# ivargr/kmer_mapper

Hardware: AMD Instinct MI355X
Metric: M k-mers mapped/sec (whole node), k=31 150bp reads (higher is better)
Workload: dtype u64

## Files before the change

### kmer_mapper_amd/csrc/kmm.hip

```cpp
#include <hip/hip_runtime.h>

#include <climits>
#include <cstdarg>
#include <cstdint>
#include <cstdio>
#include <cstdlib>
#include <chrono>
#include <cstring>
#include <memory>
#include <mutex>
#include <string>
#include <thread>
#include <type_traits>
#include <utility>
#include <vector>

#include "kmm.h"
#include "kmm_radix_plan.hpp"

namespace {

thread_local std::string g_err;

int fail(int code, const char *fmt, ...)
// ... 188 lines not shown
constexpr size_t RING_SLOT = (size_t)16 << 20;
#ifndef KMM_RING_SLOTS
#define KMM_RING_SLOTS 8
#endif
constexpr int RING_SLOTS = KMM_RING_SLOTS;


struct TimedEvent {
    Event start, stop;
    int kernel_id = 0;
};

struct BgzfStaged {
    std::vector<unsigned long long> m_off, o_rel;
    uint64_t p = 0;
    int chain_err = 0;
    uint32_t bad_isize = 0, bad_ms = 0;
    bool hit_cap = false;
    bool staged = false;
    double ms_scan_inside = 0;
};

struct IndexStreams {
    Stream stream;
    Stream copy_stream;
};

struct RxDir16 {
    DevPtr<uint16_t> rx_pstart16;
    DevPtr<uint32_t> rx_slice_e0;
    DevPtr<uint16_t> rx_slice_fmax;
};
struct RxSlotFilter {
    DevPtr<uint32_t> rx_slots;
};
struct RxArrays : RxDir16, RxSlotFilter {
    uint64_t rx_S = 0;
    DevPtr<uint32_t> rx_pstart;
    DevPtr<uint64_t> rx_pkeys;
    DevPtr<uint64_t> rx_pkeys_raw;
    DevPtr<uint16_t> rx_pfreq;
    DevPtr<uint32_t> rx_pnodes, rx_porig, rx_ecnt, rx_ecnt_acc;
    DevPtr<uint32_t> rx_norder, rx_nnode;
    DevPtr<uint32_t> rx_occ;
};

struct kmm_index : IndexStreams, RxArrays {
    int device = 0;
    Event copied;
    DevPtr<uint4> buckets;
    DevPtr<uint4> entries;
    DevPtr<uint32_t> occ;
    bool use_occ = true;
    int occ_shift = 0;
    uint32_t bloom_words = 0;
    bool wide = false;
    bool direct_deferred = false;
    size_t direct_bytes = 0;
    size_t occ_bytes_plan = 0;
    int rx_why_not = 0;
    uint32_t *counts = nullptr;
    DevPtr<uint32_t> own_counts_buf;
    DevPtr<uint8_t> lut_default;
    DevPtr<uint8_t> lut_codes;
    DevPtr<unsigned long long> first_bad;
    DevPtr<unsigned long long> stats;
    DevPtr<unsigned long long> queue;
    bool dynamic_schedule = true;
    int dyn_chunk = 16;
    uint64_t modulo = 0, magic = 0;
    int64_t n_entries = 0, max_node_id = 0;
    Stage stage[2];
    int cur = 0;
    int n_cu = 256;
    int path = 0;
    int grid_per_cu = 64;
    bool rx_ok = false;
    RxGeometry rx_geo;
    bool rx_no_mid = false;
    bool rx_flush_sorted = true;
    uint32_t rx_max_slice = 0;
    bool rx_fits_small = false, rx_fits_mid = false;
    int rx_grid_per_cu = 2;
    int64_t rx_min_units = 0;
    int64_t rx_sub_cap = RX_SUB_CAP_MAX;
    int64_t rx_sub_cap_eff = 0;
    int rx_sub_cap_eff_age = 0;
    int64_t rx_sub_cap_last = 0;
    const uint32_t *dbg_T1 = nullptr, *dbg_item_base = nullptr;
    const uint16_t *dbg_start1 = nullptr;
    uint32_t dbg_F1 = 0, dbg_NB = 0;
    int host_pack_threads = 0;
    std::unique_ptr<kmm_hostpack::Workers> pack_pool;
    PinnedBuf pack_pinned;
    PinnedBuf ring[RING_SLOTS];
    PinnedBuf pack_bits_pinned;
    int64_t host_packed_calls = 0, host_packed_record_calls = 0;
    int64_t host_pack_slice_kb = 0;
    DevBuf bgzf_comp[2], bgzf_raw[2], bgzf_meta[2], bgzf_tabs, bgzf_err, bgzf_carry, bgzf_crc, bgzf_status;
    Event bgzf_done[2];
    Event bgzf_slot_ev[RING_SLOTS];
    bool bgzf_used[2] = {false, false};
    int bgzf_cur = 0;
    int64_t bgzf_carry_len = 0;
    BgzfStaged bgzf_pre;
    bool bgzf_pre_valid = false;
    const uint8_t *bgzf_pre_from = nullptr, *bgzf_hint_ptr = nullptr;
    int64_t bgzf_pre_n = 0, bgzf_hint_n = 0;
    int bgzf_pre_buf = 0;
    int64_t bgzf_prestaged_calls = 0;
    int64_t bgzf_head_skip = 0;
    int64_t bgzf_tail_stop = -1;
    int64_t bgzf_calls = 0, bgzf_members = 0;
    DevBuf gz_comp, gz_raw, gz_carry, gz_window, gz_tabs, gz_meta, gz_res, gz_win, gz_gmaps, gz_gwin, gz_err;
    std::vector<DevBuf> gz_arena;
    kmm_gunzip::StreamState gz_state;
    int64_t gz_carry_len = 0;
    double gz_ratio = 4.0;
    int64_t gzip_calls = 0, gzip_members = 0, gzip_chunks = 0, gzip_false_starts = 0, gzip_continuations = 0, gzip_inflated = 0;
    int dbg_gzip_chunk_kb = 0;
    DevBuf bam_tiles[2], bam_bad, bam_base, bam_ctl, bam_out;
    int32_t bam_n_ref = -1;
    uint32_t bam_excl = 0;
    int64_t bam_calls = 0, bam_records = 0, bam_excluded = 0, bam_header_bytes = 0, bam_false_starts = 0, bam_continuations = 0;
    DevBuf rs_comp, rs_raw, rs_meta, rs_err, rs_status;
    int64_t bam_n_ref_param = -1;
    int64_t dbg_bam_resync_kb = 0;
    int64_t dbg_bgzf_call_cap_kb = 0;
    int64_t flat_uniform_batches = 0;
    DevBuf sam_tiles, sam_base, sam_ctl;
    int64_t sam_calls = 0, sam_records = 0, sam_excluded = 0, sam_header_lines = 0;
    uint32_t bam_incl = 0, bam_min_mapq = 0;
    int sel_n_regions = 0, sel_keep_unplaced = 0;
    std::vector<kmm_sel::Interval> sel_iv_id, sel_iv_name;
    std::vector<std::string> sel_names;
    DevBuf sel_buf;
    size_t sel_off_name_iv = 0, sel_off_name_off = 0, sel_off_names = 0;
    int dbg_bgzf_slot_kb = 0;
    int64_t dbg_rx_buf_limit = 0;
    int dbg_rec_copy_stream = 0;
    int dbg_rec_skip = 0;
    int min_base_quality = 0;
    int use_record_qual = 0;
    int original_strand = 0;
    int64_t dbg_rec_piece_kb = 0;
    int dbg_rec_grid = 0;
    bool rx_filter = true;
    bool rx_filter_slots = true;
    bool rx_p3_fp = true;
    uint32_t dbg_p2f_cap = P2F_SLOTS;
    bool rx_packed = true;
    bool ecnt_dirty = false;
    bool rx_unchecked = false;
    DevBuf rx_buf1, rx_buf2, rx_meta, rx_probe;
    int sticky_rc = KMM_OK;
    std::string sticky_msg;
    uint64_t map_calls = 0;
    int64_t read_hits_calls = 0;
    int record_hits = 0, rhq_mode = 0;
    DevBuf rhq_hits, rhq_win;
    int64_t rhq_head = 0, rhq_pending = 0, rhq_cap = 0;
    int record_keep = 0, rk_invert = 0, rk_min_permille = 0;
    int64_t rk_min_hits = 1;
    DevBuf rkq, rk_ctl, rk_tile, rk_super;
    int64_t rkq_bound = 0, rkq_cap = 0;
    uint64_t n_radix_batches = 0, n_direct_batches = 0;
    ncclComm_t comm = nullptr;
    int comm_rank = -1, comm_size = 0;
    int comm_slices = 8;
    int64_t comm_sliced_reduces = 0;
    Stream comm_stream;
    std::vector<Event> comm_events;
    std::vector<uint64_t> flush_cuts;
    bool timing = false;
    std::vector<TimedEvent> ev_used;
    std::vector<TimedEvent> ev_free;
    double ms_total[KMM_N_KERNELS] = {0};
    int64_t launches[KMM_N_KERNELS] = {0};
};

namespace {

IndexView view_of(const kmm_index *ix)
{
    IndexView v;
    v.buckets = ix->buckets;
    v.entries = ix->entries;
    v.occ = ix->use_occ ? ix->occ : nullptr;
    v.occ_shift = ix->occ_shift;
    v.bloom_words = ix->bloom_words;
    v.wide = ix->wide ? 1 : 0;
    v.counts = ix->counts;
    v.stats = ix->stats;
    v.modulo = ix->modulo;
    v.magic = ix->magic;
    return v;
}

struct ScopedTimer {
    kmm_index *ix;
    TimedEvent ev{};
    bool active = false;
    int begin(kmm_index *ix_, int kernel_id)
    {
        ix = ix_;
        if (!ix->timing)
            return KMM_OK;
        if (!ix->ev_free.empty()) {
            ev = std::move(ix->ev_free.back());
            ix->ev_free.pop_back();
        } else {
            HIPCHK(hipEventCreate(ev.start.put()));
            HIPCHK(hipEventCreate(ev.stop.put()));
        }
        ev.kernel_id = kernel_id;
        HIPCHK(hipEventRecord(ev.start, ix->stream));
        active = true;
        return KMM_OK;
    }
    int end()
    {
        if (!active)
            return KMM_OK;
        HIPCHK(hipEventRecord(ev.stop, ix->stream));
        ix->ev_used.push_back(std::move(ev));
        active = false;
        return KMM_OK;
    }
};

int rx_flush(kmm_index *ix);
int rx_build_slots(kmm_index *ix);
bool rx_slots_active(const kmm_index *ix);
int rx_check_conservation(kmm_index *ix);
int ensure_direct(kmm_index *ix);
constexpr size_t KMM_STAT_BYTES = (size_t)KMM_STAT_SHARDS * KMM_STAT_STRIDE * 8;

int drain(kmm_index *ix)
{
    KMMCHK(rx_flush(ix));
    HIPCHK(hipStreamSynchronize(ix->copy_stream));
    HIPCHK(hipStreamSynchronize(ix->stream));
    if (ix->sticky_rc != KMM_OK)
        return fail(ix->sticky_rc, "%s", ix->sticky_msg.c_str());
    KMMCHK(rx_check_conservation(ix));
    unsigned long long bad[3] = {NO_BAD, NO_BAD, NO_BAD};
    HIPCHK(hipMemcpy(bad, ix->first_bad, sizeof bad, hipMemcpyDeviceToHost));
    if (bad[0] != NO_BAD || bad[1] != NO_BAD || bad[2] != NO_BAD) {
        unsigned long long reset[3] = {NO_BAD, NO_BAD, NO_BAD};
        HIPCHK(hipMemcpy(ix->first_bad, reset, sizeof reset, hipMemcpyHostToDevice));
        char where[160];
        snprintf(where, sizeof where, " [one of the map calls since the last synchronising call; the latest was call "
                 "#%llu on this handle; counts are invalid until kmm_reset_counts]", (unsigned long long)ix->map_calls);
        int rc;
        if (bad[2] != NO_BAD)
            rc = fail(KMM_ERR_INVALID_ARG, "read_offsets of a mapped chunk is not non-decreasing at read %llu%s",
                      bad[2], where);
        else if (bad[1] != NO_BAD)
            rc = fail(KMM_ERR_MALFORMED,
                      "record structure violated at byte offset %llu of a mapped chunk (a record line "
                      "does not start with '@' / '+' / '>'%s): multi-line FASTA/FASTQ is not supported by "
                      "the GPU reader%s", bad[1],
                      ix->min_base_quality > 0 ? ", or a quality line that ends there is not as long as its sequence line "
                                                 "(checked with min_base_quality set)" : "", where);
        else
            rc = fail(KMM_ERR_INVALID_BASE,
                      "read byte at offset %llu of a mapped chunk is not a nucleotide under the "
                      "lookup table (the reference's DNA encoder raises here)%s", bad[0], where);
        ix->sticky_rc = rc;
        ix->sticky_msg = g_err;
        return rc;
    }
    return KMM_OK;
}

int grid_for(const kmm_index *ix, int64_t work_items, int per_cu)
{
    int64_t cap = (int64_t)ix->n_cu * per_cu;
    int64_t g = work_items < cap ? work_items : cap;
    return (int)(g < 1 ? 1 : g);
}

int grid_for_tiles(const kmm_index *ix, int64_t n_tiles)
{
    const int64_t slots = (int64_t)ix->n_cu * 8;
    const int64_t cap = (int64_t)ix->n_cu * ix->grid_per_cu;
    int64_t g = n_tiles <= slots ? n_tiles : n_tiles / 4;
    if (n_tiles > slots && g < slots)
        g = slots;
    if (g > cap)
        g = cap;
    return (int)(g < 1 ? 1 : g);
}

struct DirectSchedule {
    dim3 grid;
    unsigned long long *queue;
};

int direct_schedule(kmm_index *ix, int64_t n_units, DirectSchedule *sched)
{
    const int64_t slots = (int64_t)ix->n_cu * 8;
    const bool dynamic = ix->dynamic_schedule && n_units >= slots * 4 * ix->dyn_chunk;
    if (dynamic)
        HIPCHK(hipMemsetAsync(ix->queue, 0, 3 * sizeof(unsigned long long), ix->stream));
    sched->grid = dim3(dynamic ? (unsigned)slots : (unsigned)grid_for_tiles(ix, n_units));
    sched->queue = dynamic ? ix->queue : nullptr;
    return KMM_OK;
}

template <typename F>
void with_probe_flavour(const IndexView &iv, F &&f)
{
    if (iv.occ && iv.wide)
        f(std::integral_constant<int, PROBE_WIDE_FILTER>{});
    else if (iv.occ)
        f(std::integral_constant<int, PROBE_BITMAP>{});
    else if (iv.wide)
        f(std::integral_constant<int, PROBE_WIDE>{});
    else
        f(std::integral_constant<int, PROBE_NARROW>{});
}

template <typename TT>
int stage_in(kmm_index *ix, DevBuf &buf, const TT *src, size_t count, const TT **dev, bool *staged)
{
    if (count == 0) {
        KMMCHK(ensure(buf, 256));
        *dev = static_cast<const TT *>(buf.p);
        return KMM_OK;
    }
    if (is_device_ptr(src)) {
        *dev = src;
        return KMM_OK;
    }
    KMMCHK(ensure(buf, count * sizeof(TT)));
    HIPCHK(hipMemcpyAsync(buf.p, src, count * sizeof(TT), hipMemcpyHostToDevice, ix->copy_stream));
    *dev = static_cast<const TT *>(buf.p);
    *staged = true;
    return KMM_OK;
}

Stage &next_stage(kmm_index *ix)
{
    Stage &s = ix->stage[ix->cur];
    ix->cur ^= 1;
    return s;
}

int stage_acquire(kmm_index *ix, Stage &s)
{
    if (s.used)
        HIPCHK(hipStreamWaitEvent(ix->copy_stream, s.done, 0));
    return KMM_OK;
}

int stage_copies_done(kmm_index *ix)
{
    HIPCHK(hipEventRecord(ix->copied, ix->copy_stream));
    HIPCHK(hipStreamWaitEvent(ix->stream, ix->copied, 0));
    return KMM_OK;
}

int stage_release(kmm_index *ix, Stage &s, bool staged)
{
    HIPCHK(hipEventRecord(s.done, ix->stream));
    s.used = true;
    if (staged)
        HIPCHK(hipEventSynchronize(ix->copied));
    return KMM_OK;
}

int lut_has_break(const uint8_t *lut, bool *has_break)
{
    *has_break = false;
    if (!lut)
        return KMM_OK;
    uint8_t copy[256];
    if (is_device_ptr(lut)) {
        HIPCHK(hipMemcpy(copy, lut, 256, hipMemcpyDeviceToHost));
        lut = copy;
    }
    *has_break = memchr(lut, KMM_LUT_BREAK, 256) != nullptr;
    return KMM_OK;
// ... 540 lines not shown
    if (with_occ && N <= bloom_max_entries) {
        size_t bb = (size_t)N * 2;
        const size_t cap = N <= 13000000 ? KMM_BLOOM_MAX_BYTES : KMM_BLOOM_MAX_BYTES * 3 / 2;
        if (bb > cap) bb = cap;
        if (bb < 64) bb = 64;
        if (const char *env = getenv("KMM_BLOOM_BYTES"))
            bb = (size_t)strtoull(env, nullptr, 10);
        if (bb >= 4) {
            ix->bloom_words = (uint32_t)(bb / 4);
            occ_bytes = (size_t)ix->bloom_words * 4;
        }
    }
    ix->occ_shift = occ_shift;
    ix->wide = !with_occ;
    if (const char *env = getenv("KMM_WIDE_BUCKETS"))
        ix->wide = atoi(env) != 0;
    HIPCHK(hipMalloc(ix->own_counts_buf.put(), sizeof(uint32_t) * (size_t)(ix->max_node_id + 1)));
    ix->counts = ix->own_counts_buf;
    HIPCHK(hipMemsetAsync(ix->counts, 0, sizeof(uint32_t) * (size_t)(ix->max_node_id + 1), ix->stream));
    HIPCHK(hipMalloc(ix->lut_default.put(), 256));
    HIPCHK(hipMalloc(ix->first_bad.put(), 3 * sizeof(unsigned long long)));
    HIPCHK(hipMalloc(ix->queue.put(), 4 * sizeof(unsigned long long)));
    HIPCHK(hipMalloc(ix->stats.put(), KMM_STAT_BYTES));
    HIPCHK(hipMemset(ix->stats, 0, KMM_STAT_BYTES));
    uint8_t lut[256];
    default_lut(lut);
    HIPCHK(hipMemcpy(ix->lut_default, lut, 256, hipMemcpyHostToDevice));
    HIPCHK(hipMalloc(ix->lut_codes.put(), 256));
    memset(lut, 0xFF, sizeof lut);
    lut[0] = 0; lut[1] = 1; lut[2] = 2; lut[3] = 3;
    HIPCHK(hipMemcpy(ix->lut_codes, lut, 256, hipMemcpyHostToDevice));
    unsigned long long nb[3] = {NO_BAD, NO_BAD, NO_BAD};
    HIPCHK(hipMemcpy(ix->first_bad, nb, sizeof nb, hipMemcpyHostToDevice));
    {
        const int budget = kmm_hostpack::cpu_budget();
        ix->host_pack_threads = budget >= 8 ? (budget < 16 ? budget : 16) : 0;
        if (const char *env = getenv("KMM_HOST_PACK_THREADS")) {
            const int v = atoi(env);
            ix->host_pack_threads = v < 0 ? 0 : (v > 256 ? 256 : v);
        }
    }

    if (ix->host_pack_threads > 0 && (size_t)(ix->max_node_id + 1) * 4 >= ((size_t)64 << 20))
        (void)ensure_ring(ix);

    DevBuf d_h2i, d_nk, d_km, d_nd, d_fr, d_err;
    bool staged = false;
    const int32_t *p_h2i = nullptr, *p_nk = nullptr, *p_nd = nullptr;
    const uint64_t *p_km = nullptr;
    const uint16_t *p_fr = nullptr;
    int rc = KMM_OK;
    do {
        if ((rc = stage_in<int32_t>(ix, d_h2i, h2i, (size_t)M, &p_h2i, &staged))) break;
        if ((rc = stage_in<int32_t>(ix, d_nk, nk, (size_t)M, &p_nk, &staged))) break;
        if ((rc = stage_in<uint64_t>(ix, d_km, kmers, (size_t)N, &p_km, &staged))) break;
        if ((rc = stage_in<int32_t>(ix, d_nd, nodes, (size_t)N, &p_nd, &staged))) break;
        if ((rc = stage_in<uint16_t>(ix, d_fr, freqs, (size_t)N, &p_fr, &staged))) break;
        if ((rc = ensure(d_err, 4))) break;
    } while (0);
    if (rc == KMM_OK) {
        hipError_t e = hipMemsetAsync(d_err.p, 0, 4, ix->copy_stream);
        if (e == hipSuccess) e = hipStreamSynchronize(ix->copy_stream);
        if (e != hipSuccess)
            rc = fail(KMM_ERR_HIP, "index upload: %s", hipGetErrorString(e));
    }
    uint32_t err = 0;
    if (rc == KMM_OK) {
        hipLaunchKernelGGL(k_validate_index, dim3(grid_for(ix, (int64_t)((M + 255) / 256), 16)), dim3(256), 0, ix->stream,
                           p_h2i, p_nk, p_nd, M, N, ix->max_node_id, (uint32_t *)d_err.p);
        hipError_t e = hipGetLastError();
        if (e == hipSuccess) e = hipStreamSynchronize(ix->stream);
        if (e == hipSuccess) e = hipMemcpy(&err, d_err.p, 4, hipMemcpyDeviceToHost);
        if (e != hipSuccess)
            rc = fail(KMM_ERR_HIP, "index validation: %s", hipGetErrorString(e));
    }
    if (rc == KMM_OK && !err)
        rc = rx_build(ix, p_h2i, p_nk, p_km, p_nd, p_fr);
    size_t eager_max = (size_t)16 << 30;
    if (const char *env = getenv("KMM_DIRECT_EAGER_BYTES"))
        eager_max = (size_t)strtoull(env, nullptr, 10);
    ix->direct_bytes = sizeof(uint4) * ((size_t)M * (ix->wide ? 2 : 1) + (size_t)(N > 0 ? N : 1));
    if (rc == KMM_OK && !err) {
        ix->occ_bytes_plan = with_occ ? occ_bytes : 0;
        if (ix->rx_ok && ix->direct_bytes > eager_max) {
            ix->direct_deferred = true;
        } else {
            IdxRaw src;
            src.h2i = p_h2i; src.nk = p_nk; src.kmers = p_km; src.nodes = p_nd; src.freqs = p_fr;
            rc = direct_build(ix, src, N, with_occ ? occ_bytes : 0, (uint32_t *)d_err.p);
        }
    }
    if (rc != KMM_OK)
        return rc;
    if (err & 1u)
        return fail(KMM_ERR_INDEX, "index inconsistent: a non-empty bucket "
                    "(hashes_to_index[h], n_kmers[h]) reaches outside [0, n_entries=%lld)",
                    (long long)N);
    if (err & 2u)
        return fail(KMM_ERR_INDEX, "index inconsistent: a node id lies outside [0, max_node_id=%lld]",
                    (long long)ix->max_node_id);
    return KMM_OK;
}

int kmm_index_create(const int32_t *hashes_to_index, const int32_t *n_kmers, uint64_t modulo,
                     const uint64_t *kmers, const int32_t *nodes, const uint16_t *frequencies,
                     int64_t n_entries, int64_t max_node_id, int device, kmm_index_t **out)
{
    if (!out)
        return fail(KMM_ERR_INVALID_ARG, "out is NULL");
    *out = nullptr;
    if (!hashes_to_index || !n_kmers)
        return fail(KMM_ERR_INVALID_ARG, "hashes_to_index / n_kmers is NULL");
    if (modulo < 1)
        return fail(KMM_ERR_INVALID_ARG, "modulo must be >= 1");
    if (n_entries < 0 || max_node_id < 0)
        return fail(KMM_ERR_INVALID_ARG, "n_entries=%lld / max_node_id=%lld negative",
                    (long long)n_entries, (long long)max_node_id);
    if (n_entries > 0 && (!kmers || !nodes || !frequencies))
        return fail(KMM_ERR_INVALID_ARG, "kmers / nodes / frequencies is NULL");
    if (n_entries > 0x7FFFFFFFll)
        return fail(KMM_ERR_INVALID_ARG, "n_entries exceeds the int32 bucket offsets of the index format");
    int ndev = 0;
    hipError_t e = hipGetDeviceCount(&ndev);
    if (e != hipSuccess || ndev < 1) {
        (void)hipGetLastError();
        return fail(KMM_ERR_HIP, "no HIP device available (%s): libkmm has no CPU fallback",
                    e != hipSuccess ? hipGetErrorString(e) : "0 devices");
    }
    if (device < 0 || device >= ndev)
        return fail(KMM_ERR_INVALID_ARG, "device %d outside [0, %d)", device, ndev);
    kmm_index *ix = new kmm_index();
    ix->device = device;
    ix->modulo = modulo;
    ix->magic = magic_for(modulo);
    ix->n_entries = n_entries;
    ix->max_node_id = max_node_id;
    int rc = index_create_impl(ix, hashes_to_index, n_kmers, kmers, nodes, frequencies);
    if (rc != KMM_OK) {
        std::string keep = g_err;
        kmm_index_destroy(ix);
        g_err = keep;
        return rc;
    }
    *out = ix;
    return KMM_OK;
}

int kmm_reset_counts(kmm_index_t *ix)
{
    if (!ix)
        return fail(KMM_ERR_INVALID_ARG, "idx is NULL");
    HIPCHK(hipSetDevice(ix->device));
    HIPCHK(hipMemsetAsync(ix->counts, 0, sizeof(uint32_t) * (size_t)(ix->max_node_id + 1), ix->stream));
    if (ix->rx_ecnt && ix->ecnt_dirty)
        HIPCHK(hipMemsetAsync(ix->rx_ecnt, 0, sizeof(uint32_t) * (size_t)(ix->rx_S ? ix->rx_S : 1), ix->stream));
    if (ix->rx_ecnt_acc)
        HIPCHK(hipMemsetAsync(ix->rx_ecnt_acc, 0, sizeof(uint32_t) * (size_t)(ix->rx_S ? ix->rx_S : 1), ix->stream));
    ix->ecnt_dirty = false;
    ix->rhq_head = ix->rhq_pending = 0;
    if (ix->rk_ctl.p)
        HIPCHK(hipMemsetAsync(ix->rk_ctl.p, 0, 16, ix->stream));
    ix->rkq_bound = 0;
    HIPCHK(hipMemsetAsync(ix->first_bad, 0xFF, 3 * sizeof(unsigned long long), ix->stream));
    if (ix->sticky_rc != KMM_OK) {
        unsigned long long nb[3] = {NO_BAD, NO_BAD, NO_BAD};
        HIPCHK(hipStreamSynchronize(ix->stream));
        HIPCHK(hipMemcpy(ix->first_bad, nb, sizeof nb, hipMemcpyHostToDevice));
        if (ix->sticky_rc == KMM_ERR_INTERNAL)
            HIPCHK(hipMemset(ix->stats, 0, KMM_STAT_BYTES));
        ix->sticky_rc = KMM_OK;
        ix->sticky_msg.clear();
    }
    return KMM_OK;
}

int kmm_bind_counts(kmm_index_t *ix, uint32_t *device_counts)
{
    if (!ix)
        return fail(KMM_ERR_INVALID_ARG, "idx is NULL");
    HIPCHK(hipSetDevice(ix->device));
    KMMCHK(rx_flush(ix));
    HIPCHK(hipStreamSynchronize(ix->stream));
    if (!device_counts) {
        ix->counts = ix->own_counts_buf;
        return KMM_OK;
    }
    if (!is_device_ptr(device_counts))
        return fail(KMM_ERR_INVALID_ARG, "kmm_bind_counts needs a device pointer");
    ix->counts = device_counts;
    return KMM_OK;
}

int kmm_counts_device_ptr(kmm_index_t *ix, uint32_t **out)
{
    if (!ix || !out)
        return fail(KMM_ERR_INVALID_ARG, "NULL argument");
    *out = ix->counts;
    return KMM_OK;
}

int kmm_synchronize(kmm_index_t *ix)
{
    if (!ix)
        return fail(KMM_ERR_INVALID_ARG, "idx is NULL");
    HIPCHK(hipSetDevice(ix->device));
    return drain(ix);
}

static bool ensure_pack_pool(kmm_index_t *ix);
static bool ensure_pinned(PinnedBuf &b, size_t want);

static bool ensure_ring(kmm_index_t *ix)
{
    for (int i = 0; i < RING_SLOTS; ++i) {
        if (ix->ring[i].p)
            continue;
        size_t got = 0;
        uint8_t *p = g_shelf.take(RING_SLOT, &got);
        if (p && got != RING_SLOT) {
            g_shelf.give(p, got);
            p = nullptr;
        }
        if (!p && hipHostMalloc(reinterpret_cast<void **>(&p), RING_SLOT, hipHostMallocDefault) != hipSuccess) {
            (void)hipGetLastError();
            return false;
        }
        ix->ring[i].p = p;
        ix->ring[i].bytes = RING_SLOT;
    }
    for (int i = 0; i < RING_SLOTS; ++i)
        if (!ix->bgzf_slot_ev[i] && hipEventCreateWithFlags(ix->bgzf_slot_ev[i].put(), hipEventDisableTiming) != hipSuccess) {
            (void)hipGetLastError();
            return false;
        }
    return true;
}

static int fetch_to_pageable(kmm_index_t *ix, uint8_t *dst, const uint8_t *src, size_t bytes, bool *done)
{
    *done = false;
    constexpr size_t SLOT = RING_SLOT;
    constexpr int SLOTS = RING_SLOTS;
    if (bytes < 4 * SLOT || !ensure_pack_pool(ix) || !ensure_ring(ix))
        return KMM_OK;
    const size_t n_slots = (bytes + SLOT - 1) / SLOT;
    auto issue = [&](size_t c) -> int {
        const size_t b0 = c * SLOT, len = bytes - b0 < SLOT ? bytes - b0 : SLOT;
        HIPCHK(hipMemcpyAsync(ix->ring[c % SLOTS].p, src + b0, len, hipMemcpyDeviceToHost, ix->copy_stream));
        HIPCHK(hipEventRecord(ix->bgzf_slot_ev[c % SLOTS], ix->copy_stream));
        return KMM_OK;
    };
    for (size_t c = 0; c < n_slots && c < (size_t)SLOTS; ++c)
        KMMCHK(issue(c));
    const int T = ix->pack_pool->size();
    for (size_t c = 0; c < n_slots; ++c) {
        HIPCHK(hipEventSynchronize(ix->bgzf_slot_ev[c % SLOTS]));
        const size_t b0 = c * SLOT, len = bytes - b0 < SLOT ? bytes - b0 : SLOT;
        const uint8_t *from = ix->ring[c % SLOTS].p;
        const size_t per = ((len + (size_t)T - 1) / (size_t)T + 63) & ~(size_t)63;
        ix->pack_pool->start([=](int w) {
            const size_t a = (size_t)w * per;
            if (a < len)
                memcpy(dst + b0 + a, from + a, len - a < per ? len - a : per);
        });
        ix->pack_pool->wait();
        if (c + SLOTS < n_slots)
            KMMCHK(issue(c + SLOTS));
    }
    *done = true;
    return KMM_OK;
}

int kmm_get_node_counts(kmm_index_t *ix, uint32_t *out)
{
    if (!ix || !out)
        return fail(KMM_ERR_INVALID_ARG, "NULL argument");
    HIPCHK(hipSetDevice(ix->device));
    KMMCHK(drain(ix));
    const size_t bytes = sizeof(uint32_t) * (size_t)(ix->max_node_id + 1);
    hipPointerAttribute_t a;
    memset(&a, 0, sizeof a);
    const bool known = hipPointerGetAttributes(&a, out) == hipSuccess;
    if (!known)
        (void)hipGetLastError();
    const bool on_device = known && (a.type == hipMemoryTypeDevice || a.type == hipMemoryTypeManaged);
    const bool page_locked = known && a.type == hipMemoryTypeHost;
    if (!on_device && !page_locked) {
        bool done = false;
        KMMCHK(guarded("kmm_get_node_counts", [&] {
            return fetch_to_pageable(ix, reinterpret_cast<uint8_t *>(out), reinterpret_cast<const uint8_t *>(ix->counts), bytes, &done);
        }));
        if (done)
            return KMM_OK;
    }
    HIPCHK(hipMemcpy(out, ix->counts, bytes, on_device ? hipMemcpyDeviceToDevice : hipMemcpyDeviceToHost));
    return KMM_OK;
}

int kmm_comm_get_unique_id(uint8_t id[KMM_COMM_ID_BYTES])
{
    if (!id)
        return fail(KMM_ERR_INVALID_ARG, "id is NULL");
    static_assert(KMM_COMM_ID_BYTES == NCCL_UNIQUE_ID_BYTES, "kmm.h and rccl.h disagree on the id size");
    KMMCHK(rccl_load());
    ncclUniqueId u;
    RCCLCHK(g_rccl.GetUniqueId(&u));
    memcpy(id, u.internal, KMM_COMM_ID_BYTES);
    return KMM_OK;
}

int kmm_comm_init_rank(kmm_index_t *ix, const uint8_t id[KMM_COMM_ID_BYTES], int n_ranks, int rank)
{
    if (!ix || !id)
        return fail(KMM_ERR_INVALID_ARG, "NULL argument");
    if (n_ranks < 1 || rank < 0 || rank >= n_ranks)
        return fail(KMM_ERR_INVALID_ARG, "rank %d outside [0, %d)", rank, n_ranks);
    KMMCHK(rccl_load());
    HIPCHK(hipSetDevice(ix->device));
    if (ix->comm) {
        RCCLCHK(g_rccl.CommDestroy(ix->comm));
        ix->comm = nullptr;
    }
    ncclUniqueId u;
    memcpy(u.internal, id, KMM_COMM_ID_BYTES);
    RCCLCHK(g_rccl.CommInitRank(&ix->comm, n_ranks, u, rank));
    ix->comm_rank = rank;
    ix->comm_size = n_ranks;
    return KMM_OK;
}

int kmm_comm_reduce_counts(kmm_index_t *ix, int root)
{
    if (!ix)
        return fail(KMM_ERR_INVALID_ARG, "idx is NULL");
    if (!ix->comm)
        return fail(KMM_ERR_INVALID_ARG, "kmm_comm_init_rank has not been called on this handle");
    if (root < -1 || root >= ix->comm_size)
        return fail(KMM_ERR_INVALID_ARG, "root %d outside [-1, %d)", root, ix->comm_size);
    HIPCHK(hipSetDevice(ix->device));
    const size_t n = (size_t)ix->max_node_id + 1;
    auto reduce = [&](size_t first, size_t count, hipStream_t st) {
        return root < 0 ? g_rccl.AllReduce(ix->counts + first, ix->counts + first, count, ncclUint32, ncclSum, ix->comm, st)
                        : g_rccl.Reduce(ix->counts + first, ix->counts + first, count, ncclUint32, ncclSum, root, ix->comm, st);
    };
    const int S = ix->comm_slices;
    if (S > 1 && n >= (size_t)S * 1024) {
        const bool by_range = ix->rx_norder && !ix->rx_ecnt_acc && ix->rx_flush_sorted;
        ix->comm_sliced_reduces++;
        if (!ix->comm_stream)
            HIPCHK(hipStreamCreateWithFlags(ix->comm_stream.put(), hipStreamNonBlocking));
        while ((int)ix->comm_events.size() < S + 1) {
            Event e;
            HIPCHK(hipEventCreateWithFlags(e.put(), hipEventDisableTiming));
            ix->comm_events.push_back(std::move(e));
        }
        if (!by_range)
            KMMCHK(rx_flush(ix));
        if (by_range && (int)ix->flush_cuts.size() != S + 1) {
            std::vector<uint32_t> bounds(S + 1);
            for (int t = 0; t <= S; ++t)
                bounds[t] = (uint32_t)(n * (size_t)t / (size_t)S);
            DevBuf d_b, d_c;
            KMMCHK(ensure(d_b, (S + 1) * 4));
            KMMCHK(ensure(d_c, (S + 1) * 8));
            HIPCHK(hipMemcpyAsync(d_b.p, bounds.data(), (S + 1) * 4, hipMemcpyHostToDevice, ix->stream));
            hipLaunchKernelGGL(k_rx_node_cuts, dim3(1), dim3(64), 0, ix->stream, ix->rx_nnode, ix->rx_S, (const uint32_t *)d_b.p, S + 1,
                               (unsigned long long *)d_c.p);
            HIPCHK(hipGetLastError());
            ix->flush_cuts.assign(S + 1, 0);
            HIPCHK(hipMemcpyAsync(ix->flush_cuts.data(), d_c.p, (S + 1) * 8, hipMemcpyDeviceToHost, ix->stream));
            HIPCHK(hipStreamSynchronize(ix->stream));
            ix->flush_cuts[0] = 0;
            ix->flush_cuts[S] = ix->rx_S;
        }
        ScopedTimer tm;
        KMMCHK(tm.begin(ix, KMM_KERNEL_RX_FLUSH));
        for (int t = 0; t < S; ++t) {
            if (by_range && ix->ecnt_dirty) {
                const uint64_t j0 = ix->flush_cuts[t], j1 = ix->flush_cuts[t + 1];
                if (j1 > j0)
                    hipLaunchKernelGGL(k_rx_flush_sorted, dim3(grid_for(ix, (int64_t)((j1 - j0 + 1023) / 1024), 8)), dim3(256), 0, ix->stream,
                                       view_of(ix), ix->rx_ecnt, ix->rx_norder + j0, ix->rx_nnode + j0, j1 - j0);
                HIPCHK(hipGetLastError());
            }
            HIPCHK(hipEventRecord(ix->comm_events[t], ix->stream));
            HIPCHK(hipStreamWaitEvent(ix->comm_stream, ix->comm_events[t], 0));
            const size_t first = n * (size_t)t / (size_t)S, end = n * (size_t)(t + 1) / (size_t)S;
            RCCLCHK(reduce(first, end - first, ix->comm_stream));
        }
        if (by_range && ix->ecnt_dirty)
            HIPCHK(hipMemsetAsync(ix->rx_ecnt, 0, (size_t)ix->rx_S * 4, ix->stream));
        KMMCHK(tm.end());
        ix->ecnt_dirty = false;
        HIPCHK(hipEventRecord(ix->comm_events[S], ix->comm_stream));
        HIPCHK(hipStreamWaitEvent(ix->stream, ix->comm_events[S], 0));
        return drain(ix);
    }
    KMMCHK(rx_flush(ix));
    RCCLCHK(reduce(0, n, ix->stream));
    return drain(ix);
}

int kmm_comm_destroy(kmm_index_t *ix)
{
    if (!ix)
        return fail(KMM_ERR_INVALID_ARG, "idx is NULL");
    if (ix->comm) {
        HIPCHK(hipSetDevice(ix->device));
        HIPCHK(hipStreamSynchronize(ix->stream));
        RCCLCHK(g_rccl.CommDestroy(ix->comm));
        ix->comm = nullptr;
        ix->comm_rank = -1;
        ix->comm_size = 0;
    }
    return KMM_OK;
}

int kmm_reduce_counts(kmm_index_t **per_gpu, int n_gpus, int root)
{
    if (!per_gpu || n_gpus < 1)
        return fail(KMM_ERR_INVALID_ARG, "per_gpu is NULL or n_gpus < 1");
    if (root < -1 || root >= n_gpus)
        return fail(KMM_ERR_INVALID_ARG, "root %d outside [-1, %d)", root, n_gpus);
    std::vector<int> devs(n_gpus);
    for (int i = 0; i < n_gpus; ++i) {
        if (!per_gpu[i])
            return fail(KMM_ERR_INVALID_ARG, "per_gpu[%d] is NULL", i);
        if (per_gpu[i]->max_node_id != per_gpu[0]->max_node_id)
            return fail(KMM_ERR_INVALID_ARG, "handles disagree on max_node_id");
        devs[i] = per_gpu[i]->device;
        for (int j = 0; j < i; ++j)
            if (devs[j] == devs[i])
                return fail(KMM_ERR_INVALID_ARG, "handles %d and %d share device %d: one handle per GPU", j, i, devs[i]);
    }
    if (n_gpus == 1) {
        HIPCHK(hipSetDevice(per_gpu[0]->device));
        return drain(per_gpu[0]);
    }
    KMMCHK(rccl_load());
    std::vector<ncclComm_t> comms(n_gpus);
    RCCLCHK(g_rccl.CommInitAll(comms.data(), n_gpus, devs.data()));
    int rc = KMM_OK;
    const size_t n = (size_t)per_gpu[0]->max_node_id + 1;
    for (int i = 0; i < n_gpus && rc == KMM_OK; ++i) {
        if (hipSetDevice(devs[i]) != hipSuccess)
            rc = fail(KMM_ERR_HIP, "hipSetDevice(%d) failed", devs[i]);
        else
            rc = rx_flush(per_gpu[i]);
    }
    if (rc == KMM_OK) {
        ncclResult_t r = g_rccl.GroupStart();
        for (int i = 0; i < n_gpus && r == ncclSuccess; ++i) {
            kmm_index *ix = per_gpu[i];
            r = root < 0 ? g_rccl.AllReduce(ix->counts, ix->counts, n, ncclUint32, ncclSum, comms[i], ix->stream)
                         : g_rccl.Reduce(ix->counts, ix->counts, n, ncclUint32, ncclSum, root, comms[i], ix->stream);
        }
        const ncclResult_t r2 = g_rccl.GroupEnd();
        if (r == ncclSuccess)
            r = r2;
        if (r != ncclSuccess)
            rc = fail(KMM_ERR_HIP, "RCCL reduce of the node counts: %s", g_rccl.GetErrorString(r));
    }
    for (int i = 0; i < n_gpus; ++i) {
        (void)hipSetDevice(devs[i]);
        const int d = drain(per_gpu[i]);
        if (rc == KMM_OK)
            rc = d;
        (void)g_rccl.CommDestroy(comms[i]);
    }
    return rc;
}

int kmm_get_kmer_counts(kmm_index_t *ix, uint32_t *out)
{
    if (!ix || !out)
        return fail(KMM_ERR_INVALID_ARG, "NULL argument");
    if (!ix->rx_ecnt_acc)
        return fail(KMM_ERR_INVALID_ARG, "per-k-mer counts are only kept in count_kmers mode "
                    "(kmm_set_param(idx, \"count_kmers\", 1) before mapping)");
    HIPCHK(hipSetDevice(ix->device));
    KMMCHK(drain(ix));
    const size_t n = (size_t)ix->n_entries;
    if (n == 0)
        return KMM_OK;
    const bool out_dev = is_device_ptr(out);
    DevBuf tmp;
    uint32_t *d_out = out;
    if (!out_dev) {
        KMMCHK(ensure(tmp, n * 4));
        d_out = (uint32_t *)tmp.p;
    }
    hipError_t e = hipMemsetAsync(d_out, 0, n * 4, ix->stream);
    if (e == hipSuccess && ix->rx_S) {
        hipLaunchKernelGGL(k_rx_entry_counts, dim3(grid_for(ix, (int64_t)((ix->rx_S + 255) / 256), 16)), dim3(256), 0,
                           ix->stream, ix->rx_ecnt_acc, ix->rx_porig, ix->rx_S, d_out);
        e = hipGetLastError();
    }
    if (e == hipSuccess && !out_dev)
        e = hipMemcpyAsync(out, d_out, n * 4, hipMemcpyDeviceToHost, ix->stream);
    if (e == hipSuccess)
        e = hipStreamSynchronize(ix->stream);
    if (e != hipSuccess)
        return fail(KMM_ERR_HIP, "kmm_get_kmer_counts: %s", hipGetErrorString(e));
    return KMM_OK;
}

int kmm_map_kmers(kmm_index_t *ix, const uint64_t *kmers, int64_t n, int max_freq, int also_revcomp,
                  int k)
// ... 2476 lines not shown
                    "lookup table (the reference's DNA encoder raises here)", bad[0]);
    return KMM_OK;
}

int kmm_build_index(int device, const uint64_t *kmers, const int32_t *nodes, int64_t n, uint64_t modulo,
                    int32_t *hashes_to_index, int32_t *n_kmers, uint64_t *kmers_out, int32_t *nodes_out,
                    uint16_t *frequencies_out)
{
    if (n < 0 || modulo < 1)
        return fail(KMM_ERR_INVALID_ARG, "n negative or modulo < 1");
    if (n > 0x7FFFFFFFll || modulo > 0x7FFFFFFFull)
        return fail(KMM_ERR_INVALID_ARG, "n / modulo exceed the int32 arrays of the index format");
    if (!hashes_to_index || !n_kmers || (n > 0 && (!kmers || !nodes || !kmers_out || !nodes_out || !frequencies_out)))
        return fail(KMM_ERR_INVALID_ARG, "NULL argument");
    int ndev = 0;
    hipError_t e0 = hipGetDeviceCount(&ndev);
    if (e0 != hipSuccess || ndev < 1) {
        (void)hipGetLastError();
        return fail(KMM_ERR_HIP, "no HIP device available: libkmm has no CPU fallback");
    }
    HIPCHK(hipSetDevice(device));
    const uint64_t M = modulo;
    const uint64_t magic = magic_for(M);
    Stream st;
    DevBuf d_km, d_nd, d_nk, d_h2i, d_cur, d_src, d_ko, d_no, d_fo, d_list, d_ksort;
    std::vector<DevBuf> scratch(2 * SCAN_MAX_LEVELS);
    int rc = KMM_OK;
    hipError_t e = hipSuccess;
    HIPCHK(hipStreamCreateWithFlags(st.put(), hipStreamNonBlocking));
    auto up = [&](DevBuf &b, const void *src, size_t bytes, const void **dev) -> bool {
        if (bytes == 0 || is_device_ptr(src)) {
            *dev = src;
            return true;
        }
        if ((rc = ensure(b, bytes)))
            return false;
        if ((e = hipMemcpyAsync(b.p, src, bytes, hipMemcpyHostToDevice, st)))
            return false;
        *dev = b.p;
        return true;
    };
    auto down = [&](void *dst, const void *dev, size_t bytes) -> bool {
        if (bytes == 0 || dst == dev)
            return true;
        e = hipMemcpyAsync(dst, dev, bytes, is_device_ptr(dst) ? hipMemcpyDeviceToDevice : hipMemcpyDeviceToHost, st);
        if (e == hipSuccess)
            e = hipStreamSynchronize(st);
        return e == hipSuccess;
    };
    do {
        const void *p_km = nullptr, *p_nd = nullptr;
        if (!up(d_km, kmers, (size_t)n * 8, &p_km)) break;
        if (!up(d_nd, nodes, (size_t)n * 4, &p_nd)) break;
        uint32_t *w_nk = is_device_ptr(n_kmers) ? (uint32_t *)n_kmers : nullptr;
        uint32_t *w_h2i = is_device_ptr(hashes_to_index) ? (uint32_t *)hashes_to_index : nullptr;
        if (!w_nk) { if ((rc = ensure(d_nk, (size_t)M * 4))) break; w_nk = (uint32_t *)d_nk.p; }
        if (!w_h2i) { if ((rc = ensure(d_h2i, (size_t)M * 4))) break; w_h2i = (uint32_t *)d_h2i.p; }
        if ((rc = ensure(d_cur, (size_t)M * 4))) break;
        if ((e = hipMemsetAsync(w_nk, 0, (size_t)M * 4, st))) break;
        if ((e = hipMemsetAsync(d_cur.p, 0, (size_t)M * 4, st))) break;
        int64_t g = (n + 255) / 256;
        if (g > 65536) g = 65536;
        if (g < 1) g = 1;
        if (n > 0)
            hipLaunchKernelGGL(k_bi_hist, dim3((unsigned)g), dim3(256), 0, st, (const uint64_t *)p_km, n, M, magic, w_nk);
        if ((rc = scan_exclusive(w_nk, w_h2i, M, scratch, 0, st))) break;
        if (n > 0) {
            uint64_t *w_ko = is_device_ptr(kmers_out) ? kmers_out : nullptr;
            int32_t *w_no = is_device_ptr(nodes_out) ? nodes_out : nullptr;
            uint16_t *w_fo = is_device_ptr(frequencies_out) ? frequencies_out : nullptr;
            if (!w_ko) { if ((rc = ensure(d_ko, (size_t)n * 8))) break; w_ko = (uint64_t *)d_ko.p; }
            if (!w_no) { if ((rc = ensure(d_no, (size_t)n * 4))) break; w_no = (int32_t *)d_no.p; }
            if (!w_fo) { if ((rc = ensure(d_fo, (size_t)n * 2))) break; w_fo = (uint16_t *)d_fo.p; }
            if ((rc = ensure(d_src, (size_t)n * 4))) break;
            hipLaunchKernelGGL(k_bi_scatter, dim3((unsigned)g), dim3(256), 0, st, (const uint64_t *)p_km, n, M, magic,
                               w_h2i, (uint32_t *)d_cur.p, (uint32_t *)d_src.p);
            hipLaunchKernelGGL(k_bi_place, dim3((unsigned)g), dim3(256), 0, st, (const uint64_t *)p_km,
                               (const int32_t *)p_nd, n, M, magic, w_h2i, w_nk, (const uint32_t *)d_src.p, w_ko,
                               w_no, w_fo);
            const size_t list_cap = (size_t)n / BI_BIG + 2;
            if ((rc = ensure(d_list, (list_cap + 1) * 4))) break;
            if ((rc = ensure(d_ksort, (size_t)n * 8))) break;
            uint32_t *d_count = (uint32_t *)d_list.p + list_cap;
            if ((e = hipMemsetAsync(d_count, 0, 4, st))) break;
            {
                uint64_t gm = (M + 255) / 256;
                if (gm > 65536) gm = 65536;
                hipLaunchKernelGGL(k_bi_list_big, dim3((unsigned)gm), dim3(256), 0, st, w_nk, M, (uint32_t *)d_list.p, d_count);
            }
            hipLaunchKernelGGL(k_bi_big, dim3(1024), dim3(1024), 0, st, (const uint64_t *)p_km, (const int32_t *)p_nd, w_h2i,
                               w_nk, (const uint32_t *)d_list.p, d_count, (uint32_t *)d_src.p, (uint64_t *)d_ksort.p, w_ko,
                               w_no, w_fo);
            if ((e = hipGetLastError())) break;
            if ((e = hipStreamSynchronize(st))) break;
            if (!down(kmers_out, w_ko, (size_t)n * 8)) break;
            if (!down(nodes_out, w_no, (size_t)n * 4)) break;
            if (!down(frequencies_out, w_fo, (size_t)n * 2)) break;
        }
        {
            uint64_t gm = (M + 255) / 256;
            if (gm > 65536) gm = 65536;
            hipLaunchKernelGGL(k_bi_zero_empty, dim3((unsigned)gm), dim3(256), 0, st, w_h2i, w_nk, M);
        }
        if ((e = hipGetLastError())) break;
        if ((e = hipStreamSynchronize(st))) break;
        if (!down(n_kmers, w_nk, (size_t)M * 4)) break;
        if (!down(hashes_to_index, w_h2i, (size_t)M * 4)) break;
    } while (0);
    (void)hipStreamSynchronize(st);
    if (rc != KMM_OK)
        return rc;
    if (e != hipSuccess)
        return fail(KMM_ERR_HIP, "kmm_build_index: %s", hipGetErrorString(e));
    return KMM_OK;
}

int kmm_get_stats(kmm_index_t *ix, int reset, uint64_t *n_lookups, uint64_t *n_hits)
{
    if (!ix)
        return fail(KMM_ERR_INVALID_ARG, "idx is NULL");
    HIPCHK(hipSetDevice(ix->device));
    KMMCHK(drain(ix));
    std::vector<unsigned long long> st(KMM_STAT_BYTES / 8);
    HIPCHK(hipMemcpy(st.data(), ix->stats, KMM_STAT_BYTES, hipMemcpyDeviceToHost));
    unsigned long long tot[2] = {0, 0};
    for (int i = 0; i < KMM_STAT_SHARDS; ++i) {
        tot[0] += st[(size_t)i * KMM_STAT_STRIDE];
        tot[1] += st[(size_t)i * KMM_STAT_STRIDE + 1];
    }
    if (n_lookups)
        *n_lookups = tot[0];
    if (n_hits)
        *n_hits = tot[1];
    if (reset)
        HIPCHK(hipMemset(ix->stats, 0, KMM_STAT_BYTES));
    return KMM_OK;
}

int kmm_set_timing(kmm_index_t *ix, int enabled)
{
    if (!ix)
        return fail(KMM_ERR_INVALID_ARG, "idx is NULL");
    ix->timing = enabled != 0;
    return KMM_OK;
}

int kmm_get_timing(kmm_index_t *ix, int kernel_id, double *kernel_ms, int64_t *n_launches)
{
    if (!ix)
        return fail(KMM_ERR_INVALID_ARG, "idx is NULL");
    if (kernel_id < 0 || kernel_id >= KMM_N_KERNELS)
        return fail(KMM_ERR_INVALID_ARG, "kernel_id %d outside [0, %d)", kernel_id, KMM_N_KERNELS);
    HIPCHK(hipSetDevice(ix->device));
    HIPCHK(hipStreamSynchronize(ix->stream));
    for (auto &ev : ix->ev_used) {
        float ms = 0.f;
        HIPCHK(hipEventElapsedTime(&ms, ev.start, ev.stop));
        ix->ms_total[ev.kernel_id] += ms;
        ix->launches[ev.kernel_id] += 1;
        ix->ev_free.push_back(std::move(ev));
    }
    ix->ev_used.clear();
    if (kernel_ms)
        *kernel_ms = ix->ms_total[kernel_id];
    if (n_launches)
        *n_launches = ix->launches[kernel_id];
    ix->ms_total[kernel_id] = 0.0;
    ix->launches[kernel_id] = 0;
    return KMM_OK;
}

int kmm_set_record_regions(kmm_index_t *ix, const kmm_region_t *regions, int n_regions, int keep_unplaced)
{
    return guarded("kmm_set_record_regions", [&]() -> int {
        if (!ix || n_regions < 0 || (n_regions > 0 && !regions))
            return fail(KMM_ERR_INVALID_ARG, "kmm_set_record_regions: NULL argument or n_regions negative");
        if (n_regions > KMM_MAX_RECORD_REGIONS)
            return fail(KMM_ERR_INVALID_ARG, "kmm_set_record_regions: %d regions, at most %d are taken", n_regions, KMM_MAX_RECORD_REGIONS);
        std::vector<kmm_sel::Interval> by_id, by_name;
        std::vector<std::string> names;
        bool ids = true, named = true;
        for (int i = 0; i < n_regions; ++i) {
            const kmm_region_t &r = regions[i];
            if (r.beg < 0 || r.end <= r.beg)
                return fail(KMM_ERR_INVALID_ARG, "kmm_set_record_regions: region %d is [%lld, %lld): beg < 0 or end <= beg", i,
                            (long long)r.beg, (long long)r.end);
            if (r.ref_name && (r.ref_name[0] == 0 || strlen(r.ref_name) > (size_t)KMM_MAX_REGION_NAME_BYTES || !strcmp(r.ref_name, "*")))
                return fail(KMM_ERR_INVALID_ARG, "kmm_set_record_regions: region %d: ref_name is empty, \"*\" or longer than %d bytes", i,
                            KMM_MAX_REGION_NAME_BYTES);
            ids = ids && r.ref_id >= 0;
            named = named && r.ref_name != nullptr;
            if (r.ref_name)
                names.push_back(r.ref_name);
        }
        if (n_regions > 0 && !ids && !named)
            return fail(KMM_ERR_INVALID_ARG, "kmm_set_record_regions: every region needs a ref_id (>= 0; BAM) or every region a ref_name (SAM)");
        std::sort(names.begin(), names.end());
        names.erase(std::unique(names.begin(), names.end()), names.end());
        if (!named)
            names.clear();
        for (int i = 0; i < n_regions; ++i) {
            const kmm_region_t &r = regions[i];
            if (ids)
                by_id.push_back(kmm_sel::Interval{(int64_t)r.ref_id, r.beg, r.end});
            if (named)
                by_name.push_back(kmm_sel::Interval{(int64_t)(std::lower_bound(names.begin(), names.end(), std::string(r.ref_name)) - names.begin()),
                                                    r.beg, r.end});
        }
        kmm_sel::merge_intervals(by_id);
        kmm_sel::merge_intervals(by_name);
        std::vector<int64_t> refs;
        for (const kmm_sel::Interval &v : by_id)
            if (refs.empty() || refs.back() != v.ref)
                refs.push_back(v.ref);
        if (refs.size() > (size_t)KMM_MAX_REGION_REFERENCES || names.size() > (size_t)KMM_MAX_REGION_REFERENCES)
            return fail(KMM_ERR_INVALID_ARG, "kmm_set_record_regions: regions on %zu distinct references, at most %d are taken",
                        std::max(refs.size(), names.size()), KMM_MAX_REGION_REFERENCES);
        const size_t off_name_iv = by_id.size() * sizeof(kmm_sel::Interval), off_name_off = off_name_iv + by_name.size() * sizeof(kmm_sel::Interval),
                     off_names = off_name_off + (names.size() + 1) * 4;
        std::vector<uint8_t> h(off_names);
        if (!by_id.empty())
            memcpy(h.data(), by_id.data(), off_name_iv);
        if (!by_name.empty())
            memcpy(h.data() + off_name_iv, by_name.data(), off_name_off - off_name_iv);
        uint32_t at = 0;
        for (size_t i = 0; i <= names.size(); ++i) {
            memcpy(h.data() + off_name_off + 4 * i, &at, 4);
            if (i < names.size()) {
                h.insert(h.end(), names[i].begin(), names[i].end());
                at += (uint32_t)names[i].size();
            }
        }
        HIPCHK(hipSetDevice(ix->device));
        HIPCHK(hipStreamSynchronize(ix->stream));
        if (n_regions > 0) {
            KMMCHK(ensure(ix->sel_buf, h.size() + 64));
            HIPCHK(hipMemcpy(ix->sel_buf.p, h.data(), h.size(), hipMemcpyHostToDevice));
        }
        ix->sel_n_regions = n_regions;
        ix->sel_keep_unplaced = n_regions > 0 && keep_unplaced ? 1 : 0;
        ix->sel_iv_id.swap(by_id);
        ix->sel_iv_name.swap(by_name);
        ix->sel_names.swap(names);
        ix->sel_off_name_iv = off_name_iv;
        ix->sel_off_name_off = off_name_off;
        ix->sel_off_names = off_names;
        return KMM_OK;
    });
}

int kmm_set_param(kmm_index_t *ix, const char *name, int64_t value)
{
    if (!ix || !name)
        return fail(KMM_ERR_INVALID_ARG, "NULL argument");
    HIPCHK(hipSetDevice(ix->device));
    if (strncmp(name, "debug_records_", 14) != 0)
        HIPCHK(hipStreamSynchronize(ix->stream));
    if (!strcmp(name, "path")) {
        if (value < 0 || value > 2)
            return fail(KMM_ERR_INVALID_ARG, "path must be 0 (auto), 1 (direct) or 2 (radix)");
        if (value == 2 && !ix->rx_ok)
            return fail(KMM_ERR_INVALID_ARG, "the radix path is not available for this index (modulo %llu: needs modulo < 2^31 "
                        "and slices whose entries fit LDS)", (unsigned long long)ix->modulo);
        ix->path = (int)value;
    } else if (!strcmp(name, "part_shift")) {
        const int rc = rx_reconfigure(ix, (int)value, -1, true);
        if (rc == RX_REFUSED)
            return fail(KMM_ERR_INVALID_ARG, "part_shift %lld: needs 0 <= shift <= 13, at most 512 x 512 fine partitions "
                        "and 2^shift small enough for the quotient of a 64-bit k-mer by the modulo to fit beside "
                        "the hash bits", (long long)value);
        KMMCHK(rc);
    } else if (!strcmp(name, "radix_packed_tiles")) {
        ix->rx_packed = value != 0;
    } else if (!strcmp(name, "radix_filter")) {
        ix->rx_filter = value != 0;
        if (ix->rx_pstart) {
            const int rc = rx_reconfigure(ix, ix->rx_geo.w, -1, false);
            if (rc != RX_REFUSED)
                KMMCHK(rc);
        }
    } else if (!strcmp(name, "radix_filter_slots")) {
        ix->rx_filter_slots = value != 0;
        if (ix->rx_pstart && ix->rx_ok)
            KMMCHK(rx_build_slots(ix));
    } else if (!strcmp(name, "radix_p3_fingerprints")) {
        ix->rx_p3_fp = value != 0;
    } else if (!strcmp(name, "debug_p2f_round_slots")) {
        if (value < 512 || value > P2F_SLOTS || (value & 1))
            return fail(KMM_ERR_INVALID_ARG, "debug_p2f_round_slots must be even and in [512, %d]", P2F_SLOTS);
        ix->dbg_p2f_cap = (uint32_t)value;
    } else if (!strcmp(name, "fine_bits")) {
        const int rc = value < 0 || value > 9 ? RX_REFUSED : rx_reconfigure(ix, ix->rx_geo.w, (int)value, true);
        if (rc == RX_REFUSED)
            return fail(KMM_ERR_INVALID_ARG, "fine_bits %lld: both fan-outs must stay within 512", (long long)value);
        KMMCHK(rc);
    } else if (!strcmp(name, "radix_min_units")) {
        ix->rx_min_units = value;
    } else if (!strcmp(name, "radix_sub_batch_kmers")) {
        if (value < 4 * RX_B || value > ((int64_t)1 << 32) - 2 * RX_B)
            return fail(KMM_ERR_INVALID_ARG, "radix_sub_batch_kmers outside [%d, 2^32 - %d]", 4 * RX_B, 2 * RX_B);
        ix->rx_sub_cap = value;
        ix->rx_sub_cap_eff = 0;
    } else if (!strcmp(name, "comm_overlap_slices")) {
        if (value < 1 || value > 64)
            return fail(KMM_ERR_INVALID_ARG, "comm_overlap_slices outside [1, 64]");
        ix->comm_slices = (int)value;
        ix->flush_cuts.clear();
    } else if (!strcmp(name, "radix_sorted_flush")) {
        ix->rx_flush_sorted = value != 0;
    } else if (!strcmp(name, "radix_grid_per_cu")) {
        if (value < 1 || value > 2)
            return fail(KMM_ERR_INVALID_ARG, "radix_grid_per_cu must be 1 or 2");
        ix->rx_grid_per_cu = (int)value;
    } else if (!strcmp(name, "count_kmers")) {
        if (value && !ix->rx_ok)
            return fail(KMM_ERR_INVALID_ARG, "count_kmers needs the radix path, which is not available for this index");
        KMMCHK(rx_flush(ix));
        HIPCHK(hipStreamSynchronize(ix->stream));
        if (value && !ix->rx_ecnt_acc) {
            const size_t S = ix->rx_S ? ix->rx_S : 1;
            HIPCHK(hipMalloc(ix->rx_ecnt_acc.put(), S * 4));
            HIPCHK(hipMemset(ix->rx_ecnt_acc, 0, S * 4));
        } else if (!value && ix->rx_ecnt_acc) {
            HIPCHK(ix->rx_ecnt_acc.reset());
        }
    } else if (!strcmp(name, "grid_per_cu")) {
        if (value < 1 || value > 1024)
            return fail(KMM_ERR_INVALID_ARG, "grid_per_cu outside [1, 1024]");
        ix->grid_per_cu = (int)value;
    } else if (!strcmp(name, "dynamic_schedule")) {
        ix->dynamic_schedule = value != 0;
    } else if (!strcmp(name, "dyn_chunk")) {
        if (value < 1 || value > 4096)
            return fail(KMM_ERR_INVALID_ARG, "dyn_chunk outside [1, 4096]");
        ix->dyn_chunk = (int)value;
    } else if (!strcmp(name, "occupancy_filter")) {
        ix->use_occ = value != 0;
    } else if (!strcmp(name, "debug_records_copy_stream")) {
        ix->dbg_rec_copy_stream = value != 0;
    } else if (!strcmp(name, "host_pack_threads")) {
        if (value < 0 || value > 256)
            return fail(KMM_ERR_INVALID_ARG, "host_pack_threads outside [0, 256]");
        ix->host_pack_threads = (int)value;
    } else if (!strcmp(name, "host_pack_slice_kb")) {
        if (value < 0 || value > 65536)
            return fail(KMM_ERR_INVALID_ARG, "host_pack_slice_kb outside [0, 65536]");
        ix->host_pack_slice_kb = value;
    } else if (!strcmp(name, "bgzf_head_skip")) {
        if (value < 0)
            return fail(KMM_ERR_INVALID_ARG, "bgzf_head_skip negative");
        ix->bgzf_head_skip = value;
    } else if (!strcmp(name, "bgzf_tail_stop")) {
        ix->bgzf_tail_stop = value < 0 ? -1 : value;
    } else if (!strcmp(name, "debug_bgzf_ring_slot_kb") || !strcmp(name, "debug_ring_slot_kb")) {
        if (value != 0 && (value < 4 || value > (1 << 20) || (value & (value - 1))))
            return fail(KMM_ERR_INVALID_ARG, "debug_ring_slot_kb: 0 or a power of two in [4, 2^20]");
        ix->dbg_bgzf_slot_kb = (int)value;
    } else if (!strcmp(name, "bam_exclude_flags")) {
        if (value < 0 || value > 0xFFFF)
            return fail(KMM_ERR_INVALID_ARG, "bam_exclude_flags outside [0, 0xFFFF]");
        ix->bam_excl = (uint32_t)value;
    } else if (!strcmp(name, "bam_include_flags")) {
        if (value < 0 || value > 0xFFFF)
            return fail(KMM_ERR_INVALID_ARG, "bam_include_flags outside [0, 0xFFFF]");
        ix->bam_incl = (uint32_t)value;
    } else if (!strcmp(name, "bam_min_mapq")) {
        if (value < 0 || value > 255)
            return fail(KMM_ERR_INVALID_ARG, "bam_min_mapq outside [0, 255]");
        ix->bam_min_mapq = (uint32_t)value;
    } else if (!strcmp(name, "bam_n_ref")) {
        if (value < -1 || value > 0x7FFFFFFFll)
            return fail(KMM_ERR_INVALID_ARG, "bam_n_ref outside [-1, 2^31)");
        ix->bam_n_ref_param = value;
    } else if (!strcmp(name, "debug_bam_resync_kb")) {
        if (value < 0 || value > (1ll << 32))
            return fail(KMM_ERR_INVALID_ARG, "debug_bam_resync_kb outside [0, 2^32]");
        ix->dbg_bam_resync_kb = value;
    } else if (!strcmp(name, "debug_bgzf_call_cap_kb")) {
        if (value < 0 || value > (7ll << 19))
            return fail(KMM_ERR_INVALID_ARG, "debug_bgzf_call_cap_kb outside [0, 3.5 GiB / 1 KiB]");
        ix->dbg_bgzf_call_cap_kb = value;
    } else if (!strcmp(name, "debug_gzip_chunk_kb")) {
        if (value < 0 || value > (1 << 20))
            return fail(KMM_ERR_INVALID_ARG, "debug_gzip_chunk_kb outside [0, 2^20]");
        ix->dbg_gzip_chunk_kb = (int)value;
    } else if (!strcmp(name, "debug_rx_buffer_limit")) {
        ix->dbg_rx_buf_limit = value;
    } else if (!strcmp(name, "debug_records_skip")) {
        ix->dbg_rec_skip = (int)value;
    } else if (!strcmp(name, "min_base_quality")) {
        if (value < 0 || value > 93)
            return fail(KMM_ERR_INVALID_ARG, "min_base_quality outside [0, 93]");
        ix->min_base_quality = (int)value;
    } else if (!strcmp(name, "record_hits")) {
        if (value < 0 || value > 2)
            return fail(KMM_ERR_INVALID_ARG, "record_hits takes 0 (off), 1 (hits) or 2 (hits and windows)");
        if (value != 0 && ix->rhq_pending > 0 && ix->rhq_mode != (int)value)
            return fail(KMM_ERR_INVALID_ARG, "record_hits %lld with %lld entries of mode %d pending: take them (kmm_take_record_hits) "
                        "or empty the queue (kmm_reset_counts) first", (long long)value, (long long)ix->rhq_pending, ix->rhq_mode);
        ix->record_hits = (int)value;
        if (value != 0)
            ix->rhq_mode = (int)value;
    } else if (!strcmp(name, "record_keep")) {
        if (value != 0 && value != 1)
            return fail(KMM_ERR_INVALID_ARG, "record_keep takes 0 or 1");
        ix->record_keep = (int)value;
    } else if (!strcmp(name, "record_keep_min_hits")) {
        if (value < 0 || value > 0xFFFFFFFFll)
            return fail(KMM_ERR_INVALID_ARG, "record_keep_min_hits outside [0, 2^32 - 1]");
        ix->rk_min_hits = value;
    } else if (!strcmp(name, "record_keep_min_permille")) {
        if (value < 0 || value > 1000)
            return fail(KMM_ERR_INVALID_ARG, "record_keep_min_permille outside [0, 1000]");
        ix->rk_min_permille = (int)value;
    } else if (!strcmp(name, "record_keep_invert")) {
        if (value != 0 && value != 1)
            return fail(KMM_ERR_INVALID_ARG, "record_keep_invert takes 0 or 1");
        ix->rk_invert = (int)value;
    } else if (!strcmp(name, "record_keep_pending_bytes") || !strcmp(name, "record_keep_pending_records")) {
        return fail(KMM_ERR_INVALID_ARG, "%s is read-only", name);
    } else if (!strcmp(name, "use_record_qual")) {
        if (value != 0 && value != 1)
            return fail(KMM_ERR_INVALID_ARG, "use_record_qual takes 0 or 1");
        ix->use_record_qual = (int)value;
    } else if (!strcmp(name, "original_strand")) {
        if (value != 0 && value != 1)
            return fail(KMM_ERR_INVALID_ARG, "original_strand takes 0 or 1");
        ix->original_strand = (int)value;
    } else if (!strcmp(name, "debug_records_piece_kb")) {
        if (value < 0 || value > (1 << 20))
            return fail(KMM_ERR_INVALID_ARG, "debug_records_piece_kb outside [0, 2^20]");
        ix->dbg_rec_piece_kb = value;
    } else if (!strcmp(name, "debug_records_grid")) {
        if (value < 0 || value > 65536)
            return fail(KMM_ERR_INVALID_ARG, "debug_records_grid outside [0, 65536]");
        ix->dbg_rec_grid = (int)value;
    } else if (!strcmp(name, "debug_skew_p2_counter")) {
        unsigned long long v = 0;
        HIPCHK(hipMemcpy(&v, ix->stats + 2, 8, hipMemcpyDeviceToHost));
// ... 32 lines not shown
    else if (!strcmp(name, "gzip_calls"))
        *value = ix->gzip_calls;
    else if (!strcmp(name, "gzip_members"))
        *value = ix->gzip_members;
    else if (!strcmp(name, "gzip_chunks"))
        *value = ix->gzip_chunks;
    else if (!strcmp(name, "gzip_false_starts"))
        *value = ix->gzip_false_starts;
    else if (!strcmp(name, "gzip_continuations"))
        *value = ix->gzip_continuations;
    else if (!strcmp(name, "gzip_inflated_bytes"))
        *value = ix->gzip_inflated;
    else if (!strcmp(name, "debug_gzip_chunk_kb"))
        *value = ix->dbg_gzip_chunk_kb;
    else if (!strcmp(name, "min_base_quality"))
        *value = ix->min_base_quality;
    else if (!strcmp(name, "use_record_qual"))
        *value = ix->use_record_qual;
    else if (!strcmp(name, "original_strand"))
        *value = ix->original_strand;
    else if (!strcmp(name, "debug_records_piece_kb"))
        *value = ix->dbg_rec_piece_kb;
    else if (!strcmp(name, "debug_records_grid"))
        *value = ix->dbg_rec_grid;
    else if (!strcmp(name, "record_hits"))
        *value = ix->record_hits;
    else if (!strcmp(name, "record_hits_pending"))
        *value = ix->rhq_pending;
    else if (!strcmp(name, "record_hits_pending_mode"))
        *value = ix->rhq_mode;
    else if (!strcmp(name, "record_keep"))
        *value = ix->record_keep;
    else if (!strcmp(name, "record_keep_min_hits"))
        *value = ix->rk_min_hits;
    else if (!strcmp(name, "record_keep_min_permille"))
        *value = ix->rk_min_permille;
    else if (!strcmp(name, "record_keep_invert"))
        *value = ix->rk_invert;
    else if (!strcmp(name, "record_keep_pending_bytes") || !strcmp(name, "record_keep_pending_records")) {
        HIPCHK(hipSetDevice(ix->device));
        KMMCHK(drain(ix));
        unsigned long long tail[2];
        KMMCHK(rkq_tail(ix, tail));
        *value = (int64_t)tail[name[20] == 'b' ? 0 : 1];
    } else if (!strcmp(name, "read_hits_calls"))
        *value = ix->read_hits_calls;
    else if (!strcmp(name, "bam_calls"))
        *value = ix->bam_calls;
    else if (!strcmp(name, "bam_records"))
        *value = ix->bam_records;
    else if (!strcmp(name, "bam_records_excluded"))
        *value = ix->bam_excluded;
    else if (!strcmp(name, "bam_header_bytes"))
        *value = ix->bam_header_bytes;
    else if (!strcmp(name, "bam_false_starts"))
        *value = ix->bam_false_starts;
    else if (!strcmp(name, "bam_continuations"))
        *value = ix->bam_continuations;
    else if (!strcmp(name, "bam_exclude_flags"))
        *value = ix->bam_excl;
    else if (!strcmp(name, "bam_include_flags"))
        *value = ix->bam_incl;
    else if (!strcmp(name, "bam_min_mapq"))
        *value = ix->bam_min_mapq;
    else if (!strcmp(name, "record_regions"))
        *value = (int64_t)(ix->sel_iv_id.empty() ? ix->sel_iv_name.size() : ix->sel_iv_id.size());
    else if (!strcmp(name, "sam_calls"))
        *value = ix->sam_calls;
    else if (!strcmp(name, "sam_records"))
        *value = ix->sam_records;
    else if (!strcmp(name, "sam_records_excluded"))
        *value = ix->sam_excluded;
    else if (!strcmp(name, "sam_header_lines"))
        *value = ix->sam_header_lines;
    else if (!strcmp(name, "debug_bgzf_call_cap_kb"))
        *value = ix->dbg_bgzf_call_cap_kb;
    else if (!strcmp(name, "bam_n_ref"))
        *value = ix->bam_n_ref_param;
    else if (!strcmp(name, "debug_bam_resync_kb"))
        *value = ix->dbg_bam_resync_kb;
    else if (!strcmp(name, "flat_uniform_batches"))
        *value = ix->flat_uniform_batches;
    else if (!strcmp(name, "bgzf_members"))
        *value = ix->bgzf_members;
    else if (!strcmp(name, "bgzf_carry_bytes"))
        *value = ix->bgzf_carry_len;
    else if (!strcmp(name, "host_cpu_budget"))
        *value = kmm_hostpack::cpu_budget();
    else if (!strcmp(name, "radix_sub_batch_kmers"))
        *value = ix->rx_sub_cap;
    else if (!strcmp(name, "radix_sub_batch_kmers_effective"))
        *value = ix->rx_sub_cap_last;
    else if (!strcmp(name, "comm_overlap_slices"))
        *value = ix->comm_slices;
    else if (!strcmp(name, "comm_sliced_reduces"))
        *value = ix->comm_sliced_reduces;
    else if (!strcmp(name, "debug_rx_t1_sum") || !strcmp(name, "debug_rx_start1_sum") || !strcmp(name, "debug_rx_items")) {
        HIPCHK(hipSetDevice(ix->device));
        HIPCHK(hipStreamSynchronize(ix->copy_stream));
        HIPCHK(hipStreamSynchronize(ix->stream));
        if (!ix->dbg_T1)
            return fail(KMM_ERR_INVALID_ARG, "no radix batch has run on this handle");
        uint64_t sum = 0;
        if (name[9] == 't') {
            std::vector<uint32_t> t(ix->dbg_F1);
            HIPCHK(hipMemcpy(t.data(), ix->dbg_T1, t.size() * 4, hipMemcpyDeviceToHost));
            for (uint32_t v : t)
                sum += v;
        } else if (name[9] == 'i') {
            uint32_t v = 0;
            HIPCHK(hipMemcpy(&v, ix->dbg_item_base + ix->dbg_F1, 4, hipMemcpyDeviceToHost));
            sum = v;
        } else {
            const size_t ld = (size_t)ix->dbg_F1 + 1;
            std::vector<uint16_t> r((size_t)ix->dbg_NB * ld);
            HIPCHK(hipMemcpy(r.data(), ix->dbg_start1, r.size() * 2, hipMemcpyDeviceToHost));
            for (size_t b = 0; b < ix->dbg_NB; ++b)
                sum += r[b * ld + ld - 1];
        }
        *value = (int64_t)sum;
    }
    else if (!strcmp(name, "radix_sorted_flush"))
        *value = (ix->rx_flush_sorted && ix->rx_norder) ? 1 : 0;
    else if (!strcmp(name, "radix_available"))
        *value = ix->rx_ok ? 1 : 0;
    else if (!strcmp(name, "radix_batches"))
        *value = (int64_t)ix->n_radix_batches;
    else if (!strcmp(name, "direct_batches"))
        *value = (int64_t)ix->n_direct_batches;
    else if (!strcmp(name, "radix_unavailable_reason"))
        *value = ix->rx_ok ? 0 : ix->rx_why_not;
    else if (!strcmp(name, "direct_view_resident"))
        *value = ix->buckets ? 1 : 0;
    else if (!strcmp(name, "direct_view_bytes"))
        *value = (int64_t)ix->direct_bytes;
    else if (!strcmp(name, "radix_view_bytes"))
        *value = ix->rx_pstart ? (int64_t)rx_view_bytes(ix->modulo, ix->rx_S, ix->rx_norder != nullptr) : 0;
    else if (!strcmp(name, "radix_filter"))
        *value = (ix->rx_ok && rx_filter_active(ix)) ? 1 : 0;
    else if (!strcmp(name, "radix_p3_keys_in_lds"))
        *value = ix->rx_ok ? rx_p3_shape(rx_p3_variant(ix)).keys_in_lds : 0;
    else if (!strcmp(name, "radix_filter_buckets_per_bit"))
        *value = (ix->rx_ok && rx_filter_active(ix)) ? (1 << ix->rx_geo.occ_shift) : 0;
    else if (!strcmp(name, "radix_filter_slots"))
        *value = (ix->rx_ok && rx_slots_active(ix)) ? 1 : 0;
    else if (!strcmp(name, "radix_p3_fingerprints"))
        *value = (ix->rx_ok && rx_p3_fp_active(ix)) ? 1 : 0;
    else if (!strcmp(name, "radix_filter_bits_per_partition"))
        *value = !(ix->rx_ok && rx_filter_active(ix)) ? 0
                 : rx_slots_active(ix)                ? (int64_t)P2F_SLOT_WORDS * 32
                                                      : (int64_t)1 << (ix->rx_geo.w + ix->rx_geo.f2 - ix->rx_geo.occ_shift);
    else if (!strcmp(name, "debug_p2f_round_slots"))
        *value = ix->dbg_p2f_cap;
    else if (!strcmp(name, "radix_packed_tiles"))
        *value = ix->rx_packed ? 1 : 0;
    else if (!strcmp(name, "n_fine_per_coarse"))
        *value = ix->rx_ok ? ix->rx_geo.F2 : 0;
    else if (!strcmp(name, "count_kmers"))
        *value = ix->rx_ecnt_acc ? 1 : 0;
    else if (!strcmp(name, "n_coarse_partitions"))
        *value = ix->rx_ok ? ix->rx_geo.F1 : 0;
    else if (!strcmp(name, "radix_p2_kmers") || !strcmp(name, "radix_p3_kmers") || !strcmp(name, "radix_p2_dropped") ||
             !strcmp(name, "radix_p2_multi_round_items") || !strcmp(name, "quality_masked_bases") ||
             !strcmp(name, "records_without_qual") || !strcmp(name, "records_reversed") ||
             !strcmp(name, "debug_p3_key_reads") || !strncmp(name, "stats_slot_", 11)) {
        HIPCHK(hipSetDevice(ix->device));
        KMMCHK(drain(ix));
        std::vector<unsigned long long> st(KMM_STAT_BYTES / 8);
        HIPCHK(hipMemcpy(st.data(), ix->stats, KMM_STAT_BYTES, hipMemcpyDeviceToHost));
        const int slot = name[0] == 's' ? atoi(name + 11) : name[0] == 'q' ? KMM_STAT_QUAL_MASKED
                                                          : !strcmp(name, "records_without_qual") ? KMM_STAT_REC_NO_QUAL
                                                          : !strcmp(name, "records_reversed") ? KMM_STAT_REC_REVERSED
                                                          : name[0] == 'd' ? KMM_STAT_RX_P3_KEYS
                                                          : !strcmp(name, "radix_p2_dropped") ? KMM_STAT_RX_DROPPED
                                                          : !strcmp(name, "radix_p2_multi_round_items") ? KMM_STAT_RX_MULTI
                                                          : name[7] == '2' ? 2 : 3;
        if (slot < 0 || slot >= KMM_STAT_STRIDE)
            return fail(KMM_ERR_INVALID_ARG, "unknown parameter '%s'", name);
        unsigned long long t = 0;
        for (int i = 0; i < KMM_STAT_SHARDS; ++i)
            t += st[(size_t)i * KMM_STAT_STRIDE + slot];
        *value = (int64_t)t;
    }
    else if (!strcmp(name, "grid_per_cu"))
        *value = ix->grid_per_cu;
    else if (!strcmp(name, "dynamic_schedule"))
        *value = ix->dynamic_schedule ? 1 : 0;
    else if (!strcmp(name, "occupancy_filter"))
        *value = (ix->use_occ && ix->occ) ? 1 : 0;
    else if (!strcmp(name, "bloom_filter_bytes"))
        *value = (ix->use_occ && ix->occ) ? (int64_t)ix->bloom_words * 4 : 0;
    else if (!strcmp(name, "occupancy_bits_per_bucket"))
        *value = (ix->use_occ && ix->occ && !ix->bloom_words) ? (1 << ix->occ_shift) : 0;
    else if (!strcmp(name, "wide_buckets"))
        *value = ix->wide ? 1 : 0;
    else if (!strcmp(name, "n_partitions"))
        *value = ix->rx_ok ? ix->rx_geo.PF : 0;
    else
        return fail(KMM_ERR_INVALID_ARG, "unknown parameter '%s'", name);
    return KMM_OK;
}

}
```

### kmer_mapper_amd/csrc/kmm_radix.hpp

```cpp
#pragma once
#include <type_traits>
#include "kmm_radix_plan.hpp"

constexpr int RX_NT = 512;
constexpr int RX_KPT = RX_B / RX_NT;
#ifndef RX_LPR2V
#define RX_LPR2V 16
#endif
constexpr int RX_LPR = RX_LPR2V;
constexpr int RX_NG = RX_NT / RX_LPR;
#ifndef RX_RB1
#define RX_RB1 4
#endif
#ifndef RX_RB2
#define RX_RB2 8
#endif
constexpr int RX_SUBCAP = 1024;
#ifndef RX_SUBCAP3V
#define RX_SUBCAP3V 3072
#endif
constexpr int RX_SUBCAP3 = RX_SUBCAP3V;
#ifndef RX_LPR3
#define RX_LPR3 16
#endif
constexpr bool RX_P3_LINECUT = false;
constexpr int RX_LPR_P3 = RX_LPR3;
constexpr int RX_NG3 = RX_NT / RX_LPR_P3;
#ifndef RX_U3
#define RX_U3 8
#endif
constexpr int RX_U = RX_U3;
#ifndef RX_P3_GROUP
#define RX_P3_GROUP 4
#endif
constexpr int RX_G3 = RX_P3_GROUP;
#ifndef RX_U2V
#define RX_U2V 8
#endif
constexpr int RX_U2 = RX_U2V;
#ifdef RX_NT_LOADS
#define RX_LOAD2(p) __builtin_nontemporal_load(p)
#define RX_LOAD3(p) __builtin_nontemporal_load(p)
#else
#define RX_LOAD2(p) (*(p))
#define RX_LOAD3(p) (*(p))
#endif
constexpr int RX_WMAX = 4096;
constexpr int RX_WMAX_BIG = 8192;
constexpr uint32_t RX_FILTERED = 0x80000000u;
enum { MODE_KMERS = 3 };

struct RxView {
    const uint16_t *pstart16;
    const uint32_t *slice_e0;
    const uint16_t *slice_fmax;
    const uint32_t *pstart;
    const uint64_t *pkeys;
    const uint16_t *pfreq;
    uint32_t *ecnt;
    const uint32_t *occ;
    const uint32_t *slots;
    uint32_t p2f_cap;
    uint32_t p2f_k;
    int w, f2;
    int occ_shift;
    uint32_t PF, F1, F2;
    uint32_t NB;
    uint32_t max_items;
    uint64_t *buf1, *buf2;
    uint16_t *start1;
    uint32_t *P1T;
    uint16_t *S1T;
    uint32_t *csum;
    uint32_t *T1;
    uint32_t *item_base;
    uint32_t *work_base;
    uint2 *item_desc;
    uint16_t *start2;
    uint16_t *start2T;
    uint32_t *ctrl;
    unsigned long long *queue;
    uint64_t *probe;
};

#ifndef RX_PROBE_P1W
#define RX_PROBE_P1W 0
#endif
#ifndef RX_PROBE_P2R
#define RX_PROBE_P2R 0
#endif
#ifndef RX_PROBE_P2W
#define RX_PROBE_P2W 0
#endif
#ifndef RX_PROBE_P3R
#define RX_PROBE_P3R 0
#endif
#define RX_PROBE_ANY (RX_PROBE_P1W || RX_PROBE_P2R || RX_PROBE_P2W || RX_PROBE_P3R)

__device__ __forceinline__ uint64_t rx_pack(const IndexView &iv, int sh, uint64_t q, uint32_t *coarse)
{
    uint32_t h;
    const uint64_t quo = fastdiv_m31(q, (uint32_t)iv.modulo, iv.magic, &h);
    *coarse = h >> sh;
    return (quo << sh) | (uint64_t)(h & ((1u << sh) - 1u));
}

__device__ __forceinline__ uint2 rx_pair(const uint32_t *s_in, int c0, int n)
{
    const uint2 p = *reinterpret_cast<const uint2 *>(s_in + c0);
    return make_uint2(c0 < n ? p.x : 0u, c0 + 1 < n ? p.y : 0u);
}

template <bool ONEBAR>
__device__ __forceinline__ uint32_t rx_scan256(const uint32_t *s_in, uint32_t *s_out, int n, uint32_t *s_wave, const int tid)
{
    if (ONEBAR) {
    (void)s_wave;
    const int lane = tid & 63;
    const int wave = __builtin_amdgcn_readfirstlane(tid >> 6);
    if (wave < 4) {
        const uint32_t v = tid < n ? s_in[tid] : 0u;
        const uint32_t inc = wave_scan_incl(v);
        uint32_t before = 0;
        for (int x = 0; x < wave; ++x) {
            const uint32_t t = x * 64 + lane < n ? s_in[x * 64 + lane] : 0u;
            before += (uint32_t)__builtin_amdgcn_readlane((int)wave_scan_incl(t), 63);
        }
        if (tid < n)
            s_out[tid] = before + inc - v;
        if (tid == 255)
            s_out[n] = before + inc;
    }
    __syncthreads();
    return s_out[n];
    }
    const int lane = tid & 63, wave = tid >> 6;
    const uint32_t v = tid < n ? s_in[tid] : 0u;
    const uint32_t inc = wave_scan_incl(v);
    if (wave < 4 && lane == 63)
        s_wave[wave] = inc;
    __syncthreads();
    const uint32_t total = s_wave[0] + s_wave[1] + s_wave[2] + s_wave[3];
    if (tid < n) {
        uint32_t base = 0;
        for (int x = 0; x < wave; ++x)
            base += s_wave[x];
        s_out[tid] = base + inc - v;
    }
    if (tid == 0)
        s_out[n] = total;
    __syncthreads();
    return total;
}

template <bool ONEBAR>
__device__ __forceinline__ uint32_t rx_scan512(const uint32_t *s_in, uint32_t *s_out, int n, uint32_t *s_wave, const int tid)
{
    const int lane = tid & 63;
    const int wave = __builtin_amdgcn_readfirstlane(tid >> 6);
    if (ONEBAR) {
    (void)s_wave;
    if (wave < 4) {
        const int c0 = wave * 128 + lane * 2;
        const uint2 p = rx_pair(s_in, c0, n);
        const uint32_t v = p.x + p.y;
        const uint32_t inc = wave_scan_incl(v);
        uint32_t before = 0;
        for (int x = 0; x < wave; ++x) {
            const uint2 t = rx_pair(s_in, x * 128 + lane * 2, n);
            before += (uint32_t)__builtin_amdgcn_readlane((int)wave_scan_incl(t.x + t.y), 63);
        }
        const uint32_t ex = before + inc - v;
        if (c0 < n)
            s_out[c0] = ex;
        if (c0 + 1 < n)
            s_out[c0 + 1] = ex + p.x;
        if (tid == 255)
            s_out[n] = before + inc;
    }
    __syncthreads();
    return s_out[n];
    }
    uint2 p = make_uint2(0u, 0u);
    uint32_t v = 0, inc = 0;
    const int c0 = wave * 128 + lane * 2;
    if (wave < 4) {
        p = rx_pair(s_in, c0, n);
        v = p.x + p.y;
        inc = wave_scan_incl(v);
        if (lane == 63)
            s_wave[wave] = inc;
    }
    __syncthreads();
    const uint32_t total = s_wave[0] + s_wave[1] + s_wave[2] + s_wave[3];
    if (wave < 4) {
        uint32_t base = 0;
        for (int x = 0; x < wave; ++x)
            base += s_wave[x];
        const uint32_t ex = base + inc - v;
// ... 473 lines not shown
                            "v_addc_co_u32 %0, vcc, %0, %4, vcc\n\t"
                            "v_addc_co_u32 %1, vcc, %1, %5, vcc"
                            : "=&v"(nlo), "=&v"(nhi)
                            : "v"(qlo), "v"(qhi), "v"(e.y), "v"(e.z), "s"(M32), "v"(r2)
                            : "vcc");
                        qlo = nlo;
                        qhi = nhi;
                        rem = r2 - M32 < r2 ? r2 - M32 : r2;
                    }
                    q[i] = ((((uint64_t)qhi << 32) | qlo) << sh) | (uint64_t)(rem & ((1u << sh) - 1u));
                    return ((valid >> i) & 1u) ? rem >> sh : spare;
                } else {
                    uint32_t c;
                    q[i] = rx_pack(iv, sh, q[i], &c);
                    return ((valid >> i) & 1u) ? c : spare;
                }
            };
            auto post = [&]() {
                if constexpr (STAGE_EARLY) {
                    if (sb + sb_step < sb_end)
                        tile_packed_stage<C2>(rv, tile_begin + ((int64_t)(sb + sb_step) * 2 + half), sm[half], ltid, pw[0]);
                }
            };
            rx_sort_emit<RX_RB1, MODE == MODE_KMERS, true, RX_NT, true, decltype(fwd), RxNoHook, 0, true, decltype(post)>(
                q, fwd, F1, sbuf, s_cnt, s_base, s_wave, rx.buf1 + (size_t)sb * RX_B,
                rx.start1 + (size_t)sb * (size_t)(F1 + 1) RX_PT_ARG2, RxNoHook(), RX_KPT, wave_s, post,
                RX_PROBE_P1W ? rx.probe + (size_t)sb * RX_B : nullptr, RX_PROBE_P1W);
        }
    }
#ifdef RX_PT_P1
    RX_PT_END(iv, 10);
#endif
    rx_stat_add(iv, 0, lookups);
    rx_stat_add(iv, KMM_STAT_RX_P1, lookups);
}

__global__ void __launch_bounds__(256) k_rx_colsum(RxView rx)
{
    const uint32_t F1 = rx.F1;
    const uint32_t b0 = blockIdx.x * RX_CH;
    const uint32_t b1 = b0 + RX_CH < rx.NB ? b0 + RX_CH : rx.NB;
    const size_t ld = F1 + 1;
    for (uint32_t c = threadIdx.x; c < F1; c += 256) {
        const uint16_t *p = rx.start1 + (size_t)b0 * ld + c;
        uint32_t sum = 0, b = b0;
        for (; b + 8 <= b1; b += 8, p += 8 * ld) {
            uint32_t lo[8], hi[8];
#pragma unroll
            for (int u = 0; u < 8; ++u) {
                lo[u] = p[u * ld];
                hi[u] = p[u * ld + 1];
            }
#pragma unroll
            for (int u = 0; u < 8; ++u)
                sum += hi[u] - lo[u];
        }
        for (; b < b1; ++b, p += ld)
            sum += (uint32_t)p[1] - (uint32_t)p[0];
        rx.csum[(size_t)blockIdx.x * F1 + c] = sum;
    }
}

__device__ __forceinline__ uint32_t scan256_excl(uint32_t v, uint32_t *s_wave4, uint32_t *total)
{
    const int lane = threadIdx.x & 63, wave = threadIdx.x >> 6;
    const uint32_t inc = wave_scan_incl(v);
    __syncthreads();
    if (lane == 63)
        s_wave4[wave] = inc;
    __syncthreads();
    uint32_t base = 0;
    for (int x = 0; x < wave; ++x)
        base += s_wave4[x];
    *total = s_wave4[0] + s_wave4[1] + s_wave4[2] + s_wave4[3];
    return base + inc - v;
}

template <bool WITH_P>
__global__ void __launch_bounds__(256) k_rx_chunkscan(RxView rx, uint32_t n_chunks)
{
    __shared__ uint32_t s_wave4[4];
    const uint32_t c = blockIdx.x, F1 = rx.F1;
    uint32_t carry = 0;
    for (uint32_t base = 0; base < n_chunks; base += 256) {
        const uint32_t ch = base + threadIdx.x;
        const uint32_t v = ch < n_chunks ? rx.csum[(size_t)ch * F1 + c] : 0u;
        uint32_t tot;
        const uint32_t ex = scan256_excl(v, s_wave4, &tot);
        if (ch < n_chunks)
            rx.csum[(size_t)ch * F1 + c] = carry + ex;
        carry += tot;
    }
    if (threadIdx.x == 0) {
        rx.T1[c] = carry;
        if constexpr (WITH_P)
            rx.P1T[(size_t)c * (rx.NB + 1) + rx.NB] = carry;
    }
}

__device__ __forceinline__ uint32_t scan512_excl(uint32_t v, uint32_t *s_wave8, uint32_t *total)
{
    const int lane = threadIdx.x & 63, wave = threadIdx.x >> 6;
    const uint32_t inc = wave_scan_incl(v);
    __syncthreads();
    if (lane == 63)
        s_wave8[wave] = inc;
    __syncthreads();
    uint32_t base = 0, tot = 0;
    for (int x = 0; x < 8; ++x) {
        base += x < wave ? s_wave8[x] : 0u;
        tot += s_wave8[x];
    }
    *total = tot;
    return base + inc - v;
}

__global__ void __launch_bounds__(512) k_rx_tables(RxView rx)
{
    static_assert(RX_MAXF <= 512, "one thread per coarse partition");
    __shared__ uint32_t s_wave8[8];
    const uint32_t c = threadIdx.x, F1 = rx.F1;
    const uint32_t run = c < F1 ? rx.T1[c] : 0u;
    const uint32_t n_items = c < F1 ? (run + RX_B - 1) / RX_B : 0u;
    const uint32_t rows = (n_items + RX_IC - 1) / RX_IC;
    uint32_t tot_items, tot_rows;
    const uint32_t ib = scan512_excl(n_items, s_wave8, &tot_items);
    const uint32_t wb = scan512_excl(rows, s_wave8, &tot_rows);
    uint32_t jmax = n_items;
#pragma unroll
    for (int d = 32; d > 0; d >>= 1) {
        const uint32_t o = __shfl_xor(jmax, d);
        jmax = o > jmax ? o : jmax;
    }
    __syncthreads();
    if ((threadIdx.x & 63) == 0)
        s_wave8[threadIdx.x >> 6] = jmax;
    __syncthreads();
    if (c < F1) {
        rx.item_base[c] = ib;
        rx.work_base[c] = wb;
    }
    if (c == 0) {
        uint32_t m = s_wave8[0];
        for (int x = 1; x < 8; ++x)
            m = s_wave8[x] > m ? s_wave8[x] : m;
        rx.item_base[F1] = tot_items;
        rx.work_base[F1] = tot_rows;
        rx.ctrl[0] = tot_items;
        rx.ctrl[1] = tot_rows;
        rx.ctrl[2] = m;
    }
}

template <bool WITH_P>
__global__ void __launch_bounds__(256) k_rx_colscan(RxView rx)
{
    constexpr int RB = 32;
    constexpr int TB = WITH_P ? 32 : 64, CW = 256;
    static_assert(RX_CH % TB == 0 && TB % RB == 0, "a chunk is whole tiles, a tile whole register rounds");
    __shared__ uint32_t tP[WITH_P ? CW : 1][TB + 1];
    __shared__ uint16_t tS[CW][TB + 2];
    const uint32_t F1 = rx.F1, NB = rx.NB;
    const uint32_t b0 = blockIdx.x * RX_CH;
    const uint32_t b1 = b0 + RX_CH < NB ? b0 + RX_CH : NB;
    const size_t ld = F1 + 1;
    const uint32_t lane = threadIdx.x & 63, wave = threadIdx.x >> 6;
    {
    const uint32_t cb = blockIdx.y * CW;
    const uint32_t c = cb + threadIdx.x;
    const uint32_t nc = F1 - cb < (uint32_t)CW ? F1 - cb : (uint32_t)CW;
    uint32_t run = c < F1 ? rx.csum[(size_t)blockIdx.x * F1 + c] : 0u;
    const uint32_t ib = c < F1 ? rx.item_base[c] : 0u;
    for (uint32_t t0 = b0; t0 < b1; t0 += TB) {
        const uint32_t nb = b1 - t0 < (uint32_t)TB ? b1 - t0 : (uint32_t)TB;
        if (c < F1) {
#pragma unroll 1
            for (uint32_t r0 = 0; r0 < (uint32_t)TB; r0 += RB) {
                const uint16_t *p = rx.start1 + (size_t)(t0 + r0) * ld + c;
                uint32_t lo[RB], hi[RB];
#pragma unroll
                for (int u = 0; u < RB; ++u) {
                    lo[u] = r0 + (uint32_t)u < nb ? p[u * ld] : 0u;
                    hi[u] = r0 + (uint32_t)u < nb ? p[u * ld + 1] : 0u;
                }
#pragma unroll
                for (int u = 0; u < RB; ++u) {
                    const uint32_t cnt = hi[u] - lo[u];
                    if constexpr (WITH_P)
                        tP[threadIdx.x][r0 + u] = run;
                    tS[threadIdx.x][r0 + u] = (uint16_t)lo[u];
                    if (cnt) {
                        uint32_t m = (run + RX_B - 1) / RX_B;
                        while ((uint64_t)m * RX_B < (uint64_t)run + cnt) {
                            rx.item_desc[ib + m] = make_uint2(t0 + r0 + u, WITH_P ? c : run);
                            ++m;
                        }
                    }
                    run += cnt;
                }
            }
        }
        __syncthreads();
        if constexpr (WITH_P) {
            const uint32_t bi = lane & 31;
            for (uint32_t cc = wave * 2 + (lane >> 5); cc < nc; cc += 8) {
                if (bi < nb) {
                    rx.P1T[(size_t)(cb + cc) * (NB + 1) + t0 + bi] = tP[cc][bi];
                    rx.S1T[(size_t)(cb + cc) * NB + t0 + bi] = tS[cc][bi];
                }
            }
        } else {
            for (uint32_t cc = wave; cc < nc; cc += 4) {
                if (lane < nb)
                    rx.S1T[(size_t)(cb + cc) * NB + t0 + lane] = tS[cc][lane];
            }
        }
        __syncthreads();
    }
    }
}

constexpr int RX_TR2 = 32;
__global__ void __launch_bounds__(256) k_rx_tr2(RxView rx)
{
    __shared__ uint16_t tile[RX_TR2][RX_MAXF + 2];
    const uint32_t n_items = rx.ctrl[0], cols = rx.F2 + 1;
    const uint32_t i0 = blockIdx.x * RX_TR2;
    if (i0 >= n_items)
        return;
    const uint32_t ni = n_items - i0 < (uint32_t)RX_TR2 ? n_items - i0 : (uint32_t)RX_TR2;
    for (uint32_t e = threadIdx.x; e < ni * cols; e += 256)
        tile[e / cols][e % cols] = rx.start2[(size_t)i0 * cols + e];
    __syncthreads();
    const uint32_t it = threadIdx.x % RX_TR2, c0 = threadIdx.x / RX_TR2;
    if (it < ni)
        for (uint32_t col = c0; col < cols; col += 256 / RX_TR2)
            rx.start2T[(size_t)col * rx.max_items + i0 + it] = tile[it][col];
}

__global__ void __launch_bounds__(RX_NT, 4) k_rx_p2(IndexView iv, RxView rx)
{
    __shared__ uint64_t sbuf[RX_B];
    __shared__ uint32_t sub_src[RX_SUBCAP];
    __shared__ uint32_t sub_meta[RX_SUBCAP], s_wave8[2][RX_NT / 64];
    __shared__ __attribute__((aligned(8))) uint32_t s_cnt[RX_MAXF + 2 + 64];
    __shared__ uint32_t s_base[RX_MAXF + 1], s_wave[4];
    __shared__ uint32_t s_idx;
    const int tid = threadIdx.x, grp = tid / RX_LPR, lg = tid % RX_LPR;
    const uint32_t NB = rx.NB;
    uint32_t gathered = 0;
    uint32_t scan_flip = 0;
    const uint32_t spare = rx_spare_key();
    const int F2 = (int)rx.F2;
    const uint32_t cs = (rx.F1 + 7u) / 8u, limit = rx.ctrl[2] * cs;
    const uint32_t home = rx_xcc_id();
    if (tid <= F2)
        s_cnt[tid] = 0;
    if (tid == 0)
        s_cnt[RX_NT] = 0;
    struct Item {
        uint32_t valid, c, item, b0, lo, hi;
    };
    struct RunDesc {
        uint32_t vs, ve, st;
    };
    auto describe = [&](uint32_t sub, uint32_t idx) {
        Item d;
        d.valid = 0; d.c = 0; d.item = 0; d.b0 = 0; d.lo = 0; d.hi = 0;
        if (idx >= limit)
            return d;
        const uint32_t cj = idx / cs, cc = sub * cs + idx % cs;
        if (cc >= rx.F1)
            return d;
        const uint32_t ib = rx.item_base[cc];
        if (cj >= rx.item_base[cc + 1] - ib)
            return d;
        d.valid = 1;
        d.c = cc;
        d.item = ib + cj;
        d.b0 = rx.item_desc[d.item].x;
        d.lo = cj * RX_B;
        const uint32_t Tc = rx.T1[cc];
        d.hi = Tc - d.lo < (uint32_t)RX_B ? Tc : d.lo + RX_B;
        return d;
    };
    auto run_desc = [&](const Item &d, uint32_t bb) {
        RunDesc r;
        r.vs = 0xFFFFFFFFu; r.ve = 0xFFFFFFFFu; r.st = 0;
        const uint32_t b = bb + tid;
        if (d.valid && b < NB) {
            const uint32_t *P = rx.P1T + (size_t)d.c * (NB + 1);
            r.vs = P[b];
            r.ve = P[b + 1];
            r.st = rx.S1T[(size_t)d.c * NB + b];
        }
        return r;
    };
    RX_PT_DECL;
    for (uint32_t turn = 0; turn < 8u; ++turn) {
    const uint32_t sub = (home + turn) & 7u;
    uint32_t nxt = limit;
    if (tid == 0)
        nxt = rx_pop(rx.queue, sub, limit);
    if (tid == 0)
        s_idx = nxt;
    __syncthreads();
// ... 327 lines not shown
                len_max = 0;
            }
            }
            for (uint32_t stp = len_max ? 1u << (31 - __builtin_clz(len_max)) : 0u; stp >= 1u; stp >>= 1) {
#pragma unroll
                for (int u = 0; u < P2F_KPT; ++u) {
                    const uint32_t cand = pos[u] + stp;
                    const uint32_t t = t_vs[cand <= A[u + 1] ? cand : A[u + 1]];
                    pos[u] = (cand <= A[u + 1] && t <= v[u]) ? cand : pos[u];
                }
            }
            const uint32_t bbs = (uint32_t)__builtin_amdgcn_readfirstlane((int)bb);
            const char *base = reinterpret_cast<const char *>(rx.buf1 + (size_t)bbs * RX_B);
            const size_t left = (size_t)NB * RX_B - (size_t)bbs * RX_B;
            const uint32_t lim = left > 0x1FFFFFFFull ? 0x1FFFFFFFu : (uint32_t)left - 1u;
#pragma unroll
            for (int u = 0; u < P2F_KPT; ++u) {
                uint32_t el = t_off[pos[u]] + v[u];
                el = el < lim ? el : lim;
                const uint64_t y = RX_LOAD2(reinterpret_cast<const uint64_t *>(base + (el << 3)));
                x[u] = (!MERGE || ((vmask >> u) & 1u)) ? y : x[u];
#if RX_PROBE_P2R
                if (u % RX_PROBE_P2R == 0) {
                    const size_t all = (size_t)NB * RX_B, far = ((size_t)bbs * RX_B + el + all / 2) % all;
                    const uint64_t z = RX_LOAD2(rx.buf1 + far);
                    asm volatile("" ::"v"(z));
                }
#endif
            }
            return vmask;
        };

        uint32_t cover = 0, b0 = 0;
        RunDesc rd;
        rd.a = 0; rd.b = 0;
        auto more_rounds = [&](uint32_t j, uint64_t (&x)[P2F_KPT], uint32_t &vm) {
            const uint32_t lo = item_lo(j), n = item_n(j), hi = lo + n;
            uint32_t bb = b0 + P2F_NT;
            while (cover < hi && bb < NB) {
                RunDesc r2 = load_desc(bb);
                prescan(r2, 2u);
                __syncthreads();
                put_table(r2, cover, 2u, lo, hi);
                __syncthreads();
                const uint32_t cover2 = t_vs[P2F_NT];
                vm |= fill(std::true_type(), bb, lo, n, cover, cover2, x);
                cover = cover2;
                bb += P2F_NT;
            }
            __syncthreads();
        };
        auto process = [&](uint32_t j, uint64_t (&xa)[P2F_KPT], uint32_t vma, uint64_t (&xb)[P2F_KPT], uint32_t &vmb) {
            const uint32_t item = ib + j0 + j;
            RX_PT(0);
            uint32_t keys[P2F_KPT], n_ok = 0;
            if (nofilt) {
#pragma unroll
                for (int u = 0; u < P2F_KPT; ++u) {
                    const uint32_t ok = (vma >> u) & 1u;
                    n_ok += ok;
                    keys[u] = ok ? __builtin_amdgcn_ubfe((uint32_t)xa[u], (uint32_t)w, (uint32_t)rx.f2) : spare;
                }
            } else {
#pragma unroll
                for (int u = 0; u < P2F_KPT; ++u) {
                    const uint32_t xl = (uint32_t)xa[u];
                    const uint32_t bit = SLOT ? rx_filter_slot(xl & bmask, xa[u] >> P2F_LOGBITS)
                                              : (xl & bmask) >> gs;
                    const uint32_t ok = (s_bits[bit >> 5] >> (bit & 31u)) & (vma >> u) & 1u;
                    n_ok += ok;
                    keys[u] = ok ? __builtin_amdgcn_ubfe(xl, (uint32_t)w, (uint32_t)rx.f2) : spare;
                }
            }
            gathered += (uint32_t)__popc(vma);
            dropped += (uint32_t)__popc(vma) - n_ok;
            RX_PT(5);
            if (j + 2u < n_it)
                prescan(rd, j & 1u);
            if (j + 1u < n_it) {
                const uint32_t lo1 = item_lo(j + 1u), n1 = item_n(j + 1u);
                b0 = s_b0[j + 1u];
                cover = t_vs[P2F_NT];
                vmb = fill(std::false_type(), b0, lo1, n1, lo1, cover, xb, (int)((j + 1u) & 1u));
                if (cover < lo1 + n1)
                    more_rounds(j + 1u, xb, vmb);
            }
            RX_PT(1);
            auto fine = [&](int i) { return keys[i]; };
            auto mid = [&]() {
                if (j + 2u < n_it) {
                    put_table(rd, s_v0[j + 2u], j & 1u, item_lo(j + 2u), item_lo(j + 2u) + item_n(j + 2u), (int)(j & 1u));
                    if (j + 3u < n_it)
                        rd = load_desc(s_b0[j + 3u]);
                }
            };
            rx_sort_emit<P2F_KPT, false, true, P2F_NT, false, decltype(fine), decltype(mid), (FSMALL ? 2 : 1), false, RxNoHook, CAPMAX>(
                xa, fine, F2, sbuf, s_cnt2[j & 1u], s_base, s_wave, rx.buf2 + (size_t)item * RX_B,
                rx.start2 + (size_t)item * (F2 + 1) RX_PT_ARG2, mid, P2F_KPT, -1, RxNoHook(),
                RX_PROBE_P2W ? rx.probe + (size_t)item * RX_B : nullptr, RX_PROBE_P2W, SLOT ? rx.p2f_cap : (uint32_t)RX_B,
                SLOT ? multi_stat : nullptr);
            if (tid < RX_B / 32)
                t_sbits[(j + 1u) & 1u][tid] = 0u;
            if (tid == 0)
                t_empty[(j + 1u) & 1u] = 0u;
        };

        uint64_t x0[P2F_KPT], x1[P2F_KPT];
        uint32_t vm0 = 0, vm1 = 0;
        b0 = s_b0[0];
        rd = load_desc(b0);
        prescan(rd, 0u);
        __syncthreads();
        put_table(rd, s_v0[0], 0u, item_lo(0), item_lo(0) + item_n(0), 0);
        if (n_it > 1u) {
            rd = load_desc(s_b0[1]);
            prescan(rd, 1u);
        }
        __syncthreads();
        cover = t_vs[P2F_NT];
        vm0 = fill(std::false_type(), b0, item_lo(0), item_n(0), item_lo(0), cover, x0, 0);
        __syncthreads();
        if (cover < item_lo(0) + item_n(0))
            more_rounds(0, x0, vm0);
        if (tid < RX_B / 32)
            t_sbits[0][tid] = 0u;
        if (tid == 0)
            t_empty[0] = 0u;
        if (n_it > 1u) {
            put_table(rd, s_v0[1], 1u, item_lo(1), item_lo(1) + item_n(1), 1);
            if (n_it > 2u)
                rd = load_desc(s_b0[2]);
        }
        __syncthreads();
        for (uint32_t j = 0; j < n_it; j += 2u) {
            process(j, x0, vm0, x1, vm1);
            if (j + 1u < n_it)
                process(j + 1u, x1, vm1, x0, vm0);
        }
    }
    }
#ifndef RX_PT_P1
    RX_PT_END(iv, 10);
#endif
    rx_stat_add(iv, 2, gathered);
    rx_stat_add(iv, KMM_STAT_RX_DROPPED, dropped);
}

#ifdef RX_P3_FP_STATS
#define RX_P3_KEY_READ(cond) key_reads += (cond) ? 1u : 0u
#else
#define RX_P3_KEY_READ(cond)
#endif
template <int WMAX, int ECAP, int WPS, typename DirT, int SUBCAP = RX_SUBCAP3, bool P16 = false, bool FP = false>
__global__ void __launch_bounds__(RX_NT, WPS) k_rx_p3(IndexView iv, RxView rx, int max_freq)
{
    static_assert(!P16 || sizeof(DirT) == 2, "the 16-bit directory is copied as it is");
    __shared__ uint32_t sfp[FP ? (ECAP + 8) / 4 : 1];
    __shared__ __attribute__((aligned(4))) DirT sdir[WMAX + 2];
    __shared__ uint64_t skeys[ECAP];
    __shared__ uint32_t scnt[ECAP];
    __shared__ uint32_t sub_list[SUBCAP];
    __shared__ uint32_t s_wb[RX_MAXF + 1], s_wave8[2][RX_NT / 64];
    __shared__ uint32_t s_idx;
    const int tid = threadIdx.x, grp = tid / RX_LPR_P3, lg = tid % RX_LPR_P3;
    const uint32_t n_rows = rx.ctrl[1], F1 = rx.F1, F2 = rx.F2;
    const uint32_t W = 1u << rx.w;
    const uint64_t M = iv.modulo;
    for (uint32_t i = tid; i <= F1; i += RX_NT)
        s_wb[i] = rx.work_base[i];
    const uint32_t gs = (F2 + 7u) / 8u, limit = n_rows * gs;
    unsigned long long *counters = rx.queue + 128;
    const uint32_t home = rx_xcc_id();
    uint32_t hits = 0, probed = 0, scan_flip = 0;
#ifdef RX_P3_FP_STATS
    uint32_t key_reads = 0;
#endif
    const int sh = rx.w + rx.f2;
    __syncthreads();
    struct Slice {
        uint32_t valid, g, e0, ne, it0, n_it, over, tot, fmax;
        uint64_t h0;
    };
    auto describe = [&](uint32_t sub, uint32_t idx) {
        Slice d;
        d.valid = 0; d.g = 0; d.e0 = 0; d.ne = 0; d.it0 = 0; d.n_it = 0; d.h0 = 0; d.over = 0; d.tot = 0; d.fmax = 0xFFFFu;
        if (idx >= limit)
            return d;
        const uint32_t row = idx / gs, g = sub * gs + idx % gs;
        uint32_t c_lo = 0, c_hi = F1;
        while (c_hi - c_lo > 1) {
            const uint32_t mid = (c_lo + c_hi) >> 1;
            if (s_wb[mid] <= row)
                c_lo = mid;
            else
                c_hi = mid;
        }
        const uint32_t c = c_lo;
        const uint32_t f2c = rx.PF - c * F2 < F2 ? rx.PF - c * F2 : F2;
        if (g >= f2c)
            return d;
        const uint32_t chunk = row - s_wb[c];
        d.valid = 1;
        d.g = g;
        d.h0 = (uint64_t)(c * F2 + g) << rx.w;
        uint32_t e1;
        if (P16) {
            d.e0 = rx.slice_e0[c * F2 + g];
            e1 = rx.slice_e0[c * F2 + g + 1u];
            d.fmax = rx.slice_fmax ? (uint32_t)rx.slice_fmax[c * F2 + g] : 0xFFFFu;
        } else {
            d.e0 = rx.pstart[d.h0];
            e1 = rx.pstart[d.h0 + W < M ? d.h0 + W : M];
        }
        d.tot = e1 - d.e0;
        d.ne = e1 - d.e0 < (uint32_t)ECAP ? e1 - d.e0 : (uint32_t)ECAP;
        d.over = e1 - d.e0 > (uint32_t)ECAP ? 1u : 0u;
        d.it0 = rx.item_base[c] + chunk * RX_IC;
        const uint32_t it_end = rx.item_base[c + 1];
        d.n_it = it_end - d.it0 < (uint32_t)RX_IC ? it_end - d.it0 : (uint32_t)RX_IC;
        return d;
    };
    RX_PT_DECL;
    for (uint32_t turn = 0; turn < 8u; ++turn) {
    const uint32_t sub = (home + turn) & 7u;
    uint32_t nxt = limit;
    if (tid == 0)
        nxt = rx_pop(counters, sub, limit);
    if (tid == 0)
        s_idx = nxt;
    __syncthreads();
    const uint32_t idx_first = s_idx;
    __syncthreads();
    if (idx_first >= limit)
        continue;
    if (tid == 0)
        nxt = rx_pop(counters, sub, limit);
    Slice sl = describe(sub, idx_first);
    for (;;) {
        RX_PT(0);
        const uint32_t g = sl.g, e0 = sl.e0, ne = sl.ne, it0 = sl.it0, n_it = sl.n_it;
        const uint64_t h0 = sl.h0;
        uint32_t rf[RX_IC / RX_NT], rt[RX_IC / RX_NT];
#pragma unroll
        for (int j = 0; j < RX_IC / RX_NT; ++j)
            rf[j] = rt[j] = 0;
        if (sl.valid) {
        uint32_t dv[WMAX / RX_NT + 1];
        uint64_t kv[ECAP / RX_NT];
        uint32_t fv[ECAP / RX_NT];
#ifndef RX_P3_FMAX
#define RX_P3_FMAX 1
#endif
        const bool need_f = RX_P3_FMAX == 0 || (int)sl.fmax > max_freq;
        if (P16) {
            const uint32_t *p32 = reinterpret_cast<const uint32_t *>(rx.pstart16 + h0);
#pragma unroll
            for (int j = 0; j < WMAX / 2 / RX_NT; ++j) {
                const uint32_t i = tid + j * RX_NT;
                dv[j] = i < W / 2u ? p32[i] : 0u;
            }
            if (W < 2u)
                dv[0] = tid == 0 ? (uint32_t)rx.pstart16[h0] : 0u;
        } else {
#pragma unroll
            for (int j = 0; j <= WMAX / RX_NT; ++j) {
                const uint32_t i = tid + j * RX_NT;
                dv[j] = i <= W ? rx.pstart[h0 + i < M ? h0 + i : M] : 0u;
            }
        }
#pragma unroll
        for (int j = 0; j < ECAP / RX_NT; ++j) {
            const uint32_t i = tid + j * RX_NT;
            kv[j] = i < ne ? rx.pkeys[(size_t)e0 + i] : 0ull;
            fv[j] = i < ne && need_f ? rx.pfreq[(size_t)e0 + i] : 0u;
        }
        const uint16_t *rfp = rx.start2T + (size_t)g * rx.max_items + it0;
        const uint16_t *rtp = rfp + rx.max_items;
#pragma unroll
        for (int j = 0; j < RX_IC / RX_NT; ++j) {
            const uint32_t i = tid + j * RX_NT;
            rf[j] = i < n_it ? rfp[i] : 0u;
            rt[j] = i < n_it ? rtp[i] : 0u;
        }
        if (P16) {
            uint32_t *sd32 = reinterpret_cast<uint32_t *>(sdir);
#pragma unroll
            for (int j = 0; j < WMAX / 2 / RX_NT; ++j) {
                const uint32_t i = tid + j * RX_NT;
                if (i < W / 2u)
                    sd32[i] = dv[j];
            }
            if (W < 2u && tid == 0)
                sdir[0] = (DirT)dv[0];
            if (tid == 0)
                sdir[W] = (DirT)sl.tot;
        } else {
#pragma unroll
            for (int j = 0; j <= WMAX / RX_NT; ++j) {
                const uint32_t i = tid + j * RX_NT;
                if (i <= W)
                    sdir[i] = (DirT)(dv[j] - e0);
            }
        }
#pragma unroll
        for (int j = 0; j < ECAP / RX_NT; ++j) {
            const uint32_t i = tid + j * RX_NT;
            if (i < ne) {
                skeys[i] = kv[j];
                if constexpr (FP)
                    reinterpret_cast<uint8_t *>(sfp)[i] = (uint8_t)rx_p3_fp(kv[j] >> sh);
                scnt[i] = (int)fv[j] <= max_freq ? 0u : RX_FILTERED;
            }
        }
        }
        RX_PT(1);
        if (tid == 0)
            s_idx = nxt;
        __syncthreads();
        const uint32_t idx_n = s_idx;
        if (tid == 0 && idx_n < limit)
            nxt = rx_pop(counters, sub, limit);
        const Slice sl_n = describe(sub, idx_n);
        auto probe_bucket_hbm = [&](uint64_t q, uint32_t st, uint32_t cn) {
            for (uint32_t j = 0; j < cn; ++j) {
                const size_t e = (size_t)e0 + st + j;
                if (rx.pkeys[e] == q && (int)rx.pfreq[e] <= max_freq) {
                    atomicAdd(&rx.ecnt[e], 1u);
                    ++hits;
                }
            }
        };
        if (sl.valid) {
        {
            constexpr int NR = RX_IC / RX_NT;
            uint32_t len[NR], np[NR], np_sum = 0, src[NR];
#pragma unroll
            for (int j = 0; j < NR; ++j) {
                len[j] = rt[j] - rf[j];
                src[j] = (uint32_t)(tid + j * RX_NT) * (uint32_t)RX_B + rf[j];
                np[j] = (len[j] + (uint32_t)RX_LPR_P3 - 1u) / (uint32_t)RX_LPR_P3;
                np_sum += np[j];
            }
            const char *wbase = reinterpret_cast<const char *>(rx.buf2 + (size_t)__builtin_amdgcn_readfirstlane((int)it0) * RX_B);
            uint32_t n_sub;
            const uint32_t pre = rx_scan_threads(np_sum, s_wave8, scan_flip, &n_sub);
            for (uint32_t win = 0; win < n_sub; win += SUBCAP) {
                uint32_t first = pre;
#pragma unroll
                for (int j = 0; j < NR; ++j) {
                    const uint32_t j0 = first > win ? first : win;
                    const uint32_t j1 = first + np[j] < win + (uint32_t)SUBCAP ? first + np[j] : win + (uint32_t)SUBCAP;
                    for (uint32_t q = j0; q < j1; ++q) {
                        const uint32_t done = (q - first) * (uint32_t)RX_LPR_P3;
                        const uint32_t n = len[j] - done < (uint32_t)RX_LPR_P3 ? len[j] - done : (uint32_t)RX_LPR_P3;
                        sub_list[q - win] = ((src[j] + done) << 5) | n;
                    }
                    first += np[j];
                }
                const uint32_t nw = n_sub - win < (uint32_t)SUBCAP ? n_sub - win : (uint32_t)SUBCAP;
                constexpr uint32_t STEP = RX_NG3 * RX_U;
                static_assert(SUBCAP % STEP == 0, "a padded list must fit the window");
                const uint32_t n_bat = (nw + STEP - 1u) / STEP;
                for (uint32_t i = nw + tid; i < n_bat * STEP; i += RX_NT)
                    sub_list[i] = 0u;
                __syncthreads();
                RX_PT(2);
                auto request = [&](uint32_t j0, uint64_t (&x)[RX_U]) {
                    uint32_t e[RX_U], act = 0;
#pragma unroll
                    for (int u = 0; u < RX_U; ++u)
                        e[u] = sub_list[j0 + u * RX_NG3];
#pragma unroll
                    for (int u = 0; u < RX_U; ++u) {
                        const bool in = (uint32_t)lg < (e[u] & 31u);
                        x[u] = RX_LOAD3(reinterpret_cast<const uint64_t *>(wbase + (((e[u] >> 5) + (in ? (uint32_t)lg : 0u)) << 3)));
                        act |= (in ? 1u : 0u) << u;
#if RX_PROBE_P3R
                        if (u % RX_PROBE_P3R == 0) {
                            const size_t far = ((size_t)it0 * RX_B + (e[u] >> 5) + (uint32_t)lg) % ((size_t)rx.NB * RX_B);
                            const uint64_t z = RX_LOAD3(rx.buf1 + far);
                            asm volatile("" ::"v"(z));
                        }
#endif
                    }
                    return act;
                };
                auto probe = [&](auto over_tag, const uint64_t (&x)[RX_U], uint32_t actm) {
                    constexpr bool OVER = decltype(over_tag)::value;
#pragma unroll
                    for (int g0 = 0; g0 < RX_U; g0 += RX_G3) {
                        uint32_t st[RX_G3], cn[RX_G3];
#pragma unroll
                        for (int i = 0; i < RX_G3; ++i) {
                            const uint32_t hb = (uint32_t)x[g0 + i] & (W - 1u);
                            st[i] = sdir[hb];
                            cn[i] = sdir[hb + 1];
                        }
                        uint32_t mx = 0;
#pragma unroll
                        for (int i = 0; i < RX_G3; ++i) {
                            const bool act = (actm >> (g0 + i)) & 1u;
                            probed += act ? 1u : 0u;
                            cn[i] = act ? cn[i] - st[i] : 0u;
                            if constexpr (OVER) {
                                if (cn[i] && st[i] + cn[i] > ne) {
                                    probe_bucket_hbm(x[g0 + i], st[i], cn[i]);
                                    cn[i] = 0;
                                }
                            }
                            mx = cn[i] > mx ? cn[i] : mx;
                        }
                        if constexpr (FP) {
                            uint32_t f0[RX_G3], f1[RX_G3], fp4[RX_G3], cm[RX_G3], any = 0;
#pragma unroll
                            for (int i = 0; i < RX_G3; ++i) {
                                const uint32_t wi = (OVER && !cn[i] ? 0u : st[i]) >> 2;
                                f0[i] = sfp[wi];
                                f1[i] = sfp[wi + 1u];
                            }
#pragma unroll
                            for (int i = 0; i < RX_G3; ++i) {
                                fp4[i] = rx_p3_fp4(x[g0 + i] >> sh);
                                const uint32_t lo = __builtin_amdgcn_alignbit(f1[i], f0[i], 8u * st[i]);
                                cm[i] = rx_p3_match4(lo, fp4[i], cn[i]);
                                any |= cm[i];
                            }
                            while (any) {
                                uint64_t key[RX_G3];
                                uint32_t e8[RX_G3];
#pragma unroll
                                for (int i = 0; i < RX_G3; ++i) {
                                    e8[i] = cm[i] ? 8u * st[i] + (uint32_t)__builtin_ctz(cm[i]) : 0u;
                                    key[i] = *reinterpret_cast<const uint64_t *>(reinterpret_cast<const char *>(skeys) + e8[i]);
                                    RX_P3_KEY_READ(cm[i] != 0u);
                                }
                                any = 0;
#pragma unroll
                                for (int i = 0; i < RX_G3; ++i) {
                                    if (cm[i] && key[i] == x[g0 + i])
                                        atomicAdd(reinterpret_cast<uint32_t *>(reinterpret_cast<char *>(scnt) + (e8[i] >> 1)), 1u);
                                    cm[i] &= cm[i] - 1u;
                                    any |= cm[i];
                                }
                            }
                            if (mx >= (uint32_t)RX_P3_FP_ENTRIES) {
#pragma unroll
                                for (int i = 0; i < RX_G3; ++i) {
                                    if (rx_p3_match_entry4(f1[i] >> (8u * (st[i] & 3u)), fp4[i], cn[i])) {
                                        RX_P3_KEY_READ(true);
                                        if (skeys[st[i] + 4u] == x[g0 + i])
                                            atomicAdd(&scnt[st[i] + 4u], 1u);
                                    }
                                }
                            }
                        }
                        for (uint32_t j = FP ? RX_P3_FP_ENTRIES : 0; j < mx; ++j) {
                            uint64_t key[RX_G3];
#pragma unroll
                            for (int i = 0; i < RX_G3; ++i) {
                                key[i] = skeys[j < cn[i] ? st[i] + j : 0u];
                                RX_P3_KEY_READ(j < cn[i]);
                            }
#pragma unroll
                            for (int i = 0; i < RX_G3; ++i)
                                if (j < cn[i] && key[i] == x[g0 + i])
                                    atomicAdd(&scnt[st[i] + j], 1u);
                        }
                    }
                };
                auto stream = [&](auto over_tag) {
                    for (uint32_t bi = 0; bi < n_bat; ++bi) {
                        uint64_t x[RX_U];
                        const uint32_t m = request(grp + bi * STEP, x);
                        probe(over_tag, x, m);
                    }
                };
                if (sl.over)
                    stream(std::true_type());
                else
                    stream(std::false_type());
                __syncthreads();
                RX_PT(3);
            }
        }
        for (uint32_t i = tid; i < ne; i += RX_NT) {
            const uint32_t cn = scnt[i];
            if (cn - 1u < RX_FILTERED - 1u) {
                atomicAdd(&rx.ecnt[(size_t)e0 + i], cn);
                hits += cn;
            }
        }
        }
        RX_PT(4);
        __syncthreads();
        if (idx_n >= limit)
            break;
        sl = sl_n;
    }
    }
    RX_PT_END(iv, 4);
    rx_stat_add(iv, 1, hits);
    rx_stat_add(iv, 3, probed);
#ifdef RX_P3_FP_STATS
    rx_stat_add(iv, KMM_STAT_RX_P3_KEYS, key_reads);
#endif
}

__global__ void __launch_bounds__(256) k_rx_flush(IndexView iv, uint32_t *__restrict__ ecnt,
                                                  const uint32_t *__restrict__ pnodes, uint64_t n,
                                                  uint32_t *__restrict__ ecnt_acc)
{
    __shared__ NodeAgg agg;
    agg_init(agg);
    __syncthreads();
    auto one = [&](uint64_t e, uint32_t cn, uint32_t node) {
        if (cn) {
            if (ecnt_acc)
                ecnt_acc[e] += cn;
            agg_add_n(iv, agg, node, cn);
        }
    };
    const uint64_t n4 = n / 4, gid = (uint64_t)blockIdx.x * 256 + threadIdx.x, stride = (uint64_t)gridDim.x * 256;
    uint4 *c4 = reinterpret_cast<uint4 *>(ecnt);
    const uint4 *n4p = reinterpret_cast<const uint4 *>(pnodes);
    for (uint64_t i = gid; i < n4; i += stride) {
        const uint4 c = c4[i];
        const uint4 nd = n4p[i];
        if (c.x | c.y | c.z | c.w) {
            c4[i] = make_uint4(0u, 0u, 0u, 0u);
            one(4 * i, c.x, nd.x);
            one(4 * i + 1, c.y, nd.y);
            one(4 * i + 2, c.z, nd.z);
            one(4 * i + 3, c.w, nd.w);
        }
    }
    for (uint64_t e = n4 * 4 + gid; e < n; e += stride) {
        const uint32_t cn = ecnt[e];
        if (cn) {
            ecnt[e] = 0;
            one(e, cn, pnodes[e]);
        }
    }
    __syncthreads();
    agg_flush_counts(iv, agg);
}

__global__ void __launch_bounds__(256) k_rx_node_hist(const uint32_t *__restrict__ pnodes, uint64_t n, uint32_t *__restrict__ hist)
{
    for (uint64_t e = (uint64_t)blockIdx.x * 256 + threadIdx.x; e < n; e += (uint64_t)gridDim.x * 256)
        atomicAdd(&hist[pnodes[e]], 1u);
}

__global__ void __launch_bounds__(256) k_rx_node_scatter(const uint32_t *__restrict__ pnodes, uint64_t n,
                                                         uint32_t *__restrict__ cursor, uint32_t *__restrict__ norder,
                                                         uint32_t *__restrict__ nnode)
{
    for (uint64_t e = (uint64_t)blockIdx.x * 256 + threadIdx.x; e < n; e += (uint64_t)gridDim.x * 256) {
        const uint32_t nd = pnodes[e];
        const uint32_t j = atomicAdd(&cursor[nd], 1u);
        norder[j] = (uint32_t)e;
        nnode[j] = nd;
    }
}

__global__ void __launch_bounds__(256) k_rx_flush_sorted(IndexView iv, const uint32_t *__restrict__ ecnt,
                                                         const uint32_t *__restrict__ norder,
                                                         const uint32_t *__restrict__ nnode, uint64_t n)
{
    constexpr int U = 4;
    const int lane = threadIdx.x & 63;
    const uint64_t n_round = (n + 255) / 256 * 256;
    for (uint64_t j0 = ((uint64_t)blockIdx.x * U) * 256 + threadIdx.x; j0 < n_round; j0 += (uint64_t)gridDim.x * U * 256) {
        uint32_t nd[U], c[U];
#pragma unroll
        for (int u = 0; u < U; ++u) {
            const uint64_t j = j0 + (uint64_t)u * 256;
            nd[u] = j < n ? nnode[j] : 0xFFFFFFFFu;
            c[u] = j < n ? ecnt[norder[j]] : 0u;
        }
#pragma unroll
        for (int u = 0; u < U; ++u) {
            uint32_t sum = c[u];
#pragma unroll
            for (int d = 1; d < 64; d <<= 1) {
                const uint32_t os = __shfl_up(sum, d), on = __shfl_up(nd[u], d);
                if (lane >= d && on == nd[u])
                    sum += os;
            }
            const uint32_t next = __shfl_down(nd[u], 1);
            if ((lane == 63 || next != nd[u]) && sum)
                atomicAdd(&iv.counts[nd[u]], sum);
        }
    }
}

__global__ void k_rx_node_cuts(const uint32_t *__restrict__ nnode, uint64_t n, const uint32_t *__restrict__ bounds, int n_bounds,
                               unsigned long long *__restrict__ cuts)
{
    for (int t = threadIdx.x; t < n_bounds; t += blockDim.x) {
        const uint32_t b = bounds[t];
        uint64_t lo = 0, hi = n;
        while (lo < hi) {
            const uint64_t mid = lo + (hi - lo) / 2;
            if (nnode[mid] < b)
                lo = mid + 1;
            else
                hi = mid;
        }
        cuts[t] = lo;
    }
}

__global__ void __launch_bounds__(256) k_rx_max_slice(const uint32_t *__restrict__ pstart, uint64_t modulo, int w,
                                                      uint32_t PF, unsigned long long *out)
{
    uint32_t m = 0, over = 0, over_mid = 0;
    for (uint64_t f = (uint64_t)blockIdx.x * 256 + threadIdx.x; f < PF; f += (uint64_t)gridDim.x * 256) {
        const uint64_t h0 = f << w, h1 = h0 + (1ull << w) < modulo ? h0 + (1ull << w) : modulo;
        const uint32_t c = pstart[h1] - pstart[h0];
        m = c > m ? c : m;
        over += c > (uint32_t)RX_ECAP ? 1u : 0u;
        over_mid += c > (uint32_t)RX_ECAP_MID ? 1u : 0u;
    }
#pragma unroll
    for (int d = 32; d > 0; d >>= 1) {
        const uint32_t o = __shfl_xor(m, d);
        m = o > m ? o : m;
        over += __shfl_xor(over, d);
        over_mid += __shfl_xor(over_mid, d);
    }
    if ((threadIdx.x & 63) == 0) {
        if (m)
            atomicMax(out, (unsigned long long)m);
        if (over)
            atomicAdd(out + 1, (unsigned long long)over);
        if (over_mid)
// ... 130 lines not shown
```

### kmer_mapper_amd/csrc/kmm_radix_host.hpp

```cpp
#pragma once

int rx_check_conservation(kmm_index *ix)
{
    if (!ix->rx_unchecked)
        return KMM_OK;
    ix->rx_unchecked = false;
    static thread_local std::vector<unsigned long long> st;
    st.resize(KMM_STAT_BYTES / 8);
    HIPCHK(hipMemcpy(st.data(), ix->stats, KMM_STAT_BYTES, hipMemcpyDeviceToHost));
    unsigned long long p1 = 0, p2 = 0, p3 = 0, dropped = 0;
    for (int i = 0; i < KMM_STAT_SHARDS; ++i) {
        const unsigned long long *sh = st.data() + (size_t)i * KMM_STAT_STRIDE;
        p1 += sh[KMM_STAT_RX_P1];
        p2 += sh[2];
        p3 += sh[3];
        dropped += sh[KMM_STAT_RX_DROPPED];
    }
    if (p1 == p2 && p2 == p3 + dropped)
        return KMM_OK;
    const int rc = fail(KMM_ERR_INTERNAL, "radix path self-check failed: pass 1 emitted %llu k-mers, pass 2 gathered %llu, "
                        "pass 3 probed %llu (+ %llu dropped as absent) since the counters were last reset: the node counts "
                        "are invalid until kmm_reset_counts [latest map call #%llu on this handle]",
                        p1, p2, p3, dropped, (unsigned long long)ix->map_calls);
    ix->sticky_rc = rc;
    ix->sticky_msg = g_err;
    return rc;
}

bool rx_filter_active(const kmm_index *ix)
{
    const RxGeometry &g = ix->rx_geo;
    return ix->rx_filter && ix->rx_occ && g.w + g.f2 - g.occ_shift >= 5 && g.occ_shift <= 2;
}

bool rx_slots_active(const kmm_index *ix)
{
    return rx_filter_active(ix) && ix->rx_geo.slot_filter && ix->rx_filter_slots && ix->rx_slots;
}

bool use_radix(const kmm_index *ix, int64_t units)
{
    if (!ix->rx_ok || ix->path == 1)
        return false;
    return ix->path == 2 || ix->rx_ecnt_acc || units >= ix->rx_min_units;
}

RxP3Variant rx_p3_variant(const kmm_index *ix)
{
    return rx_choose_p3(ix->rx_geo.w, ix->rx_fits_small, ix->rx_fits_mid, ix->rx_pstart16 != nullptr, ix->rx_max_slice,
                        ix->rx_no_mid);
}

bool rx_p3_fp_active(const kmm_index *ix)
{
    return ix->rx_p3_fp && rx_p3_shape(rx_p3_variant(ix)).fingerprints;
}

RxView rx_view_of(const kmm_index *ix, const RxScratch &sc, uint32_t NB)
{
    const RxGeometry &g = ix->rx_geo;
    RxView rx;
    memset(&rx, 0, sizeof rx);
    rx.pstart = ix->rx_pstart; rx.pkeys = ix->rx_pkeys; rx.pfreq = ix->rx_pfreq; rx.ecnt = ix->rx_ecnt;
    rx.pstart16 = ix->rx_pstart16; rx.slice_e0 = ix->rx_slice_e0; rx.slice_fmax = ix->rx_slice_fmax;
    rx.occ = ix->rx_occ;
    rx.slots = rx_slots_active(ix) ? (const uint32_t *)ix->rx_slots : nullptr;
    rx.p2f_cap = ix->dbg_p2f_cap;
    rx.occ_shift = rx_filter_active(ix) ? g.occ_shift : 3;
    rx.p2f_k = NB / 2048u < 4u ? 4u : (NB / 2048u > (uint32_t)P2F_KMAX ? (uint32_t)P2F_KMAX : NB / 2048u);
    rx.w = g.w; rx.f2 = g.f2; rx.PF = g.PF; rx.F1 = g.F1; rx.F2 = g.F2;
    rx.NB = NB; rx.max_items = (uint32_t)sc.max_items;
    uint8_t *m = (uint8_t *)ix->rx_meta.p;
    rx.start1 = (uint16_t *)(m + sc.start1); rx.P1T = (uint32_t *)(m + sc.P1T); rx.S1T = (uint16_t *)(m + sc.S1T);
    rx.csum = (uint32_t *)(m + sc.csum); rx.T1 = (uint32_t *)(m + sc.T1); rx.item_base = (uint32_t *)(m + sc.item_base);
    rx.work_base = (uint32_t *)(m + sc.work_base); rx.item_desc = (uint2 *)(m + sc.item_desc);
    rx.start2 = (uint16_t *)(m + sc.start2); rx.start2T = (uint16_t *)(m + sc.start2T);
    rx.ctrl = (uint32_t *)(m + sc.ctrl);
    rx.queue = (unsigned long long *)(m + sc.queue);
    rx.buf1 = (uint64_t *)ix->rx_buf1.p;
    rx.buf2 = (uint64_t *)ix->rx_buf2.p;
#if RX_PROBE_ANY
    rx.probe = (uint64_t *)ix->rx_probe.p;
#endif
    return rx;
}

template <int MODE>
int rx_launch_p1(kmm_index *ix, const ReadsView &rv, const uint64_t *src_kmers, int64_t n_kmers, const IndexView &iv,
                 const RxView &rx, int k, int64_t tile0, uint32_t n_src, int also_rc)
{
    static const int p1_per_cu = getenv("KMM_RX_P1_GRID_PER_CU") ? atoi(getenv("KMM_RX_P1_GRID_PER_CU")) : 8;
    const int64_t g1cap = (int64_t)ix->n_cu * (p1_per_cu > 0 ? p1_per_cu : 8);
    const dim3 g1((unsigned)(n_src < g1cap ? n_src : g1cap));
    constexpr bool CAN_C2 = MODE == MODE_PACKED || MODE == MODE_UNIFORM || MODE == MODE_GENERAL;
    if (rv.codes2 && !CAN_C2)
        return fail(KMM_ERR_INTERNAL, "2-bit code input reaches pass 1 through the flat-read modes only");
    auto go = [&](auto kern) {
        hipLaunchKernelGGL(kern, g1, dim3(RX_NT), 0, ix->stream, rv, src_kmers, n_kmers, iv, rx, k, tile0, n_src);
    };
    if constexpr (CAN_C2) {
        if (rv.codes2) {
            if (also_rc)
                go(k_rx_p1<MODE, true, true>);
            else
                go(k_rx_p1<MODE, false, true>);
            return KMM_OK;
        }
    }
    if (also_rc)
        go(k_rx_p1<MODE, true>);
    else
        go(k_rx_p1<MODE, false>);
    return KMM_OK;
}

void rx_launch_p2(kmm_index *ix, const IndexView &iv, const RxView &rx)
{
    if (!ix->rx_filter) {
        hipLaunchKernelGGL(k_rx_p2, dim3(ix->n_cu * ix->rx_grid_per_cu), dim3(RX_NT), 0, ix->stream, iv, rx);
        return;
    }
    const bool flt = rx_filter_active(ix), small = rx.F2 <= 128;
    auto kern = rx.slots ? (small ? k_rx_p2f<P2F_SLOT, true> : k_rx_p2f<P2F_SLOT, false>)
                : flt    ? (small ? k_rx_p2f<P2F_BITMAP, true> : k_rx_p2f<P2F_BITMAP, false>)
                         : (small ? k_rx_p2f<P2F_NONE, true> : k_rx_p2f<P2F_NONE, false>);
    hipLaunchKernelGGL(kern, dim3(ix->n_cu), dim3(P2F_NT), 0, ix->stream, iv, rx);
}

void rx_launch_p3(kmm_index *ix, const IndexView &iv, const RxView &rx, int max_freq)
{
    const RxP3Variant v = rx_p3_variant(ix);
    const dim3 grid(ix->n_cu * (rx_p3_shape(v).wg_per_cu > 1 ? ix->rx_grid_per_cu : 1));
    auto go = [&](auto kern) { hipLaunchKernelGGL(kern, grid, dim3(RX_NT), 0, ix->stream, iv, rx, max_freq); };
    static_assert(rx_p3_shape(RxP3Variant::W12_DIR16).fingerprints && rx_p3_fp_shapes() == 1,
                  "RX_P3_SHAPES promises the fingerprint form exactly where an instantiation is named below");
    switch (v) {
    case RxP3Variant::W12_DIR16:
        if (rx_p3_fp_active(ix))
            go(k_rx_p3<RX_WMAX, RX_ECAP, 4, uint16_t, RX_SUBCAP3, true, true>);
        else
            go(k_rx_p3<RX_WMAX, RX_ECAP, 4, uint16_t, RX_SUBCAP3, true>);
        break;
    case RxP3Variant::W12:             go(k_rx_p3<RX_WMAX, RX_ECAP, 4, uint32_t>); break;
    case RxP3Variant::W13_SMALL_DIR16: go(k_rx_p3<RX_WMAX_BIG, RX_ECAP, 4, uint16_t, RX_SUBCAP3, true>); break;
    case RxP3Variant::W13_SMALL:       go(k_rx_p3<RX_WMAX_BIG, RX_ECAP, 4, uint16_t>); break;
    case RxP3Variant::W13_MID_DIR16:   go(k_rx_p3<RX_WMAX_BIG, RX_ECAP_MID, 4, uint16_t, 1024, true>); break;
    case RxP3Variant::W13_MID:         go(k_rx_p3<RX_WMAX_BIG, RX_ECAP_MID, 4, uint16_t, 1024>); break;
    case RxP3Variant::W13_BIG:         go(k_rx_p3<RX_WMAX_BIG, RX_ECAP_BIG, 2, uint32_t>); break;
    }
}

template <int MODE>
int launch_rx(kmm_index *ix, const ReadsView &rv, const uint64_t *kmers_in, int64_t n_in, int k, int max_freq,
              int also_rc)
{
    const IndexView iv = view_of(ix);
    const int64_t units = MODE == MODE_KMERS ? n_in : rv.total;
    const int64_t n_src_total = MODE == MODE_PACKED ? (rv.n_reads + 2 * (int64_t)rv.pk_rpt - 1) / (2 * (int64_t)rv.pk_rpt)
                                                    : (units + RX_B - 1) / RX_B;
    const uint32_t X = also_rc ? 2u : 1u;
    const uint32_t F1 = ix->rx_geo.F1, F2 = ix->rx_geo.F2;
    RxSplit split;
    static const bool verbose = getenv("KMM_VERBOSE") != nullptr;
    const auto t_0 = std::chrono::steady_clock::now();
    if (ix->rx_sub_cap_eff > 0 && ++ix->rx_sub_cap_eff_age >= RX_SUB_CAP_AGE)
        ix->rx_sub_cap_eff = 0;
    int64_t cap = ix->rx_sub_cap_eff > 0 && ix->rx_sub_cap_eff < ix->rx_sub_cap ? ix->rx_sub_cap_eff : ix->rx_sub_cap;
    for (;;) {
        split = rx_split(n_src_total, X, cap);
        const RxScratch sm = rx_scratch((uint32_t)(split.max_src * X), F1, F2);
        int rc = ix->dbg_rx_buf_limit && sm.buf1_bytes > (size_t)ix->dbg_rx_buf_limit ? (int)KMM_ERR_NOMEM
                                                                                      : ensure(ix->rx_meta, sm.meta_bytes);
        if (rc == KMM_OK)
            rc = ensure(ix->rx_buf1, sm.buf1_bytes);
        if (rc == KMM_OK)
            rc = ensure(ix->rx_buf2, sm.buf2_bytes);
#if RX_PROBE_ANY
        if (rc == KMM_OK)
            rc = ensure(ix->rx_probe, sm.buf2_bytes);
#endif
        if (rc == KMM_OK)
            break;
        if (rc != KMM_ERR_NOMEM || cap <= RX_SUB_CAP_FLOOR || n_src_total <= 1)
            return rc;
        (void)hipGetLastError();
        (void)ix->rx_buf1.reset();
        (void)ix->rx_buf2.reset();
        cap = rx_next_smaller_cap(n_src_total, X, split.n_sub);
        ix->rx_sub_cap_eff = cap;
        ix->rx_sub_cap_eff_age = 0;
    }
    ix->rx_sub_cap_last = cap;
    const double ms_buffers = ms_since(t_0);
    const int64_t max_src = split.max_src;
    for (int64_t s0 = 0; s0 < n_src_total; s0 += max_src) {
        const uint32_t n_src = (uint32_t)(n_src_total - s0 < max_src ? n_src_total - s0 : max_src);
        const uint32_t NB = n_src * X;
        const RxScratch sc = rx_scratch(NB, F1, F2);
        bool grew = sc.meta_bytes > ix->rx_meta.cap || sc.buf1_bytes > ix->rx_buf1.cap || sc.buf2_bytes > ix->rx_buf2.cap;
#if RX_PROBE_ANY
        grew = grew || sc.buf2_bytes > ix->rx_probe.cap;
#endif
        if (grew)
            return fail(KMM_ERR_INTERNAL, "radix path: a sub-batch of %u blocks needs more scratch than the largest one was given", NB);
        const RxView rx = rx_view_of(ix, sc, NB);
        ix->dbg_T1 = rx.T1; ix->dbg_item_base = rx.item_base; ix->dbg_start1 = rx.start1; ix->dbg_F1 = F1; ix->dbg_NB = NB;
        HIPCHK(hipMemsetAsync(rx.ctrl, 0, sc.meta_bytes - sc.ctrl, ix->stream));
        ScopedTimer tm;
        KMMCHK(tm.begin(ix, KMM_KERNEL_RX_P1));
        const int64_t tile0 = s0 * (RX_B / (MODE == MODE_RECORDS ? 1024 : 4096));
        KMMCHK(rx_launch_p1<MODE>(ix, rv, kmers_in ? kmers_in + s0 * RX_B : nullptr, n_in - s0 * RX_B, iv, rx, k, tile0, n_src,
                                  also_rc));
        HIPCHK(hipGetLastError());
        KMMCHK(tm.end());
        KMMCHK(tm.begin(ix, KMM_KERNEL_RX_SCAN));
        const bool with_p = !ix->rx_filter;
        auto chunkscan = with_p ? k_rx_chunkscan<true> : k_rx_chunkscan<false>;
        auto colscan = with_p ? k_rx_colscan<true> : k_rx_colscan<false>;
        hipLaunchKernelGGL(k_rx_colsum, dim3(sc.chunks), dim3(256), 0, ix->stream, rx);
        hipLaunchKernelGGL(chunkscan, dim3(F1), dim3(256), 0, ix->stream, rx, sc.chunks);
        hipLaunchKernelGGL(k_rx_tables, dim3(1), dim3(512), 0, ix->stream, rx);
        hipLaunchKernelGGL(colscan, dim3(sc.chunks, (F1 + 255) / 256), dim3(256), 0, ix->stream, rx);
        HIPCHK(hipGetLastError());
        KMMCHK(tm.end());
        KMMCHK(tm.begin(ix, KMM_KERNEL_RX_P2));
        rx_launch_p2(ix, iv, rx);
        HIPCHK(hipGetLastError());
        KMMCHK(tm.end());
        KMMCHK(tm.begin(ix, KMM_KERNEL_RX_SCAN));
        hipLaunchKernelGGL(k_rx_tr2, dim3((unsigned)((sc.max_items + RX_TR2 - 1) / RX_TR2)), dim3(256), 0, ix->stream, rx);
        HIPCHK(hipGetLastError());
        KMMCHK(tm.end());
        KMMCHK(tm.begin(ix, KMM_KERNEL_RX_P3));
        rx_launch_p3(ix, iv, rx, max_freq);
        HIPCHK(hipGetLastError());
        KMMCHK(tm.end());
        ix->ecnt_dirty = true;
        ix->rx_unchecked = true;
    }
    ix->n_radix_batches++;
    if (verbose && ms_since(t_0) > 20.0)
        fprintf(stderr, "libkmm: radix passes of %lld positions: %.2f ms for the batch buffers (%zu + %zu + %zu bytes), %.2f ms to issue %lld "
                "sub-batch(es)\n", (long long)units, ms_buffers, ix->rx_meta.cap, ix->rx_buf1.cap, ix->rx_buf2.cap, ms_since(t_0) - ms_buffers,
                (long long)split.n_sub);
    return KMM_OK;
}

int rx_flush(kmm_index *ix)
{
    if (!ix->ecnt_dirty)
        return KMM_OK;
    ScopedTimer tm;
    KMMCHK(tm.begin(ix, KMM_KERNEL_RX_FLUSH));
    if (ix->rx_norder && !ix->rx_ecnt_acc && ix->rx_flush_sorted) {
        hipLaunchKernelGGL(k_rx_flush_sorted, dim3(ix->n_cu * 8), dim3(256), 0, ix->stream, view_of(ix), ix->rx_ecnt,
                           ix->rx_norder, ix->rx_nnode, ix->rx_S);
        HIPCHK(hipMemsetAsync(ix->rx_ecnt, 0, (size_t)ix->rx_S * 4, ix->stream));
    } else {
        hipLaunchKernelGGL(k_rx_flush, dim3(ix->n_cu * 8), dim3(256), 0, ix->stream, view_of(ix), ix->rx_ecnt,
                           ix->rx_pnodes, ix->rx_S, ix->rx_ecnt_acc);
    }
    HIPCHK(hipGetLastError());
    KMMCHK(tm.end());
    ix->ecnt_dirty = false;
    return KMM_OK;
}

int rx_build_slots(kmm_index *ix)
{
    static_cast<RxSlotFilter &>(*ix) = RxSlotFilter();
    if (!ix->rx_filter || !ix->rx_geo.slot_filter || !ix->rx_filter_slots || !ix->rx_occ)
        return KMM_OK;
    const size_t bytes = (size_t)ix->rx_geo.F1 * P2F_SLOT_WORDS * 4;
    if (hipMalloc(ix->rx_slots.put(), bytes) != hipSuccess) {
        (void)hipGetLastError();
        static_cast<RxSlotFilter &>(*ix) = RxSlotFilter();
        return KMM_OK;
    }
    HIPCHK(hipMemsetAsync(ix->rx_slots, 0, bytes, ix->stream));
    hipLaunchKernelGGL(k_rx_build_slots, dim3(grid_for(ix, (int64_t)((ix->modulo + 255) / 256), 16)), dim3(256), 0, ix->stream,
                       ix->rx_pstart, ix->rx_pkeys, ix->modulo, ix->rx_geo.w + ix->rx_geo.f2, ix->rx_slots);
    HIPCHK(hipGetLastError());
    HIPCHK(hipStreamSynchronize(ix->stream));
    return KMM_OK;
}

int rx_repack_keys(kmm_index *ix)
{
    if (ix->rx_S)
        hipLaunchKernelGGL(k_rx_pack_keys, dim3(grid_for(ix, (int64_t)((ix->rx_S + 255) / 256), 16)), dim3(256), 0,
                           ix->stream, ix->rx_pkeys_raw, ix->rx_S, view_of(ix), ix->rx_geo.w + ix->rx_geo.f2, ix->rx_pkeys);
    HIPCHK(hipGetLastError());
    HIPCHK(hipMemsetAsync(ix->queue, 0, 3 * sizeof(unsigned long long), ix->stream));
    hipLaunchKernelGGL(k_rx_max_slice, dim3(grid_for(ix, (int64_t)((ix->rx_geo.PF + 255) / 256), 16)), dim3(256), 0, ix->stream,
                       ix->rx_pstart, ix->modulo, ix->rx_geo.w, ix->rx_geo.PF, ix->queue);
    HIPCHK(hipGetLastError());
    unsigned long long mx[3] = {0, 0, 0};
    HIPCHK(hipMemcpyAsync(mx, ix->queue, sizeof mx, hipMemcpyDeviceToHost, ix->stream));
    HIPCHK(hipStreamSynchronize(ix->stream));
    ix->rx_max_slice = (uint32_t)mx[0];
    const unsigned long long odd = ix->rx_geo.PF / 1000 > 1 ? ix->rx_geo.PF / 1000 : 1;
    ix->rx_fits_small = mx[1] <= odd;
    ix->rx_fits_mid = mx[2] <= odd;
    static_cast<RxDir16 &>(*ix) = RxDir16();
    if (ix->rx_max_slice <= 65535u && !getenv("KMM_RX_NO_P16")) {
        const size_t n16 = ((size_t)ix->rx_geo.PF << ix->rx_geo.w) + 8;
        if (hipMalloc(ix->rx_pstart16.put(), n16 * 2) == hipSuccess &&
            hipMalloc(ix->rx_slice_e0.put(), ((size_t)ix->rx_geo.PF + 2) * 4) == hipSuccess &&
            hipMalloc(ix->rx_slice_fmax.put(), ((size_t)ix->rx_geo.PF + 2) * 2) == hipSuccess) {
            hipLaunchKernelGGL(k_rx_pstart16, dim3(grid_for(ix, (int64_t)((n16 + 255) / 256), 16)), dim3(256), 0, ix->stream,
                               ix->rx_pstart, ix->modulo, ix->rx_geo.w, ix->rx_geo.PF, ix->rx_pstart16, ix->rx_slice_e0);
            HIPCHK(hipGetLastError());
            hipLaunchKernelGGL(k_rx_slice_fmax, dim3(grid_for(ix, (int64_t)((ix->rx_geo.PF + 3) / 4), 16)), dim3(256), 0, ix->stream,
                               ix->rx_slice_e0, ix->rx_pfreq, ix->rx_geo.PF, ix->rx_slice_fmax);
            HIPCHK(hipGetLastError());
            HIPCHK(hipStreamSynchronize(ix->stream));
        } else {
            (void)hipGetLastError();
            static_cast<RxDir16 &>(*ix) = RxDir16();
        }
    }
    return rx_build_slots(ix);
}

int rx_build(kmm_index *ix, const int32_t *h2i, const int32_t *nk, const uint64_t *kmers, const int32_t *nodes,
             const uint16_t *freqs)
{
    const uint64_t M = ix->modulo;
    if (const char *env = getenv("KMM_RX_FILTER"))
        ix->rx_filter = atoi(env) != 0;
    if (const char *env = getenv("KMM_RX_FILTER_SLOTS"))
        ix->rx_filter_slots = atoi(env) != 0;
    if (const char *env = getenv("KMM_RX_P3_FP"))
        ix->rx_p3_fp = atoi(env) != 0;
    ix->rx_why_not = 1;
    if (M >= (1ull << 31))
        return KMM_OK;
    DevBuf sizes;
    std::vector<DevBuf> scratch(2 * SCAN_MAX_LEVELS);
    int rc = KMM_OK;
    hipError_t e = hipSuccess;
    bool overlap = false;
    do {
        if ((rc = ensure(sizes, (size_t)(M + 1) * 4))) break;
        if ((e = hipMalloc(ix->rx_pstart.put(), (size_t)(M + 1) * RxViewBytes::pstart))) break;
        hipLaunchKernelGGL(k_rx_bucket_sizes, dim3(grid_for(ix, (int64_t)((M + 256) / 256), 16)), dim3(256), 0,
                           ix->stream, h2i, nk, M, ix->n_entries, (uint32_t *)sizes.p);
        unsigned long long sum64 = 0;
        if ((e = hipMemsetAsync(ix->queue, 0, sizeof(unsigned long long), ix->stream))) break;
        hipLaunchKernelGGL(k_sum_u32, dim3(grid_for(ix, (int64_t)((M + 256) / 256), 8)), dim3(256), 0, ix->stream,
                           (const uint32_t *)sizes.p, M + 1, ix->queue);
        if ((e = hipMemcpyAsync(&sum64, ix->queue, 8, hipMemcpyDeviceToHost, ix->stream))) break;
        if ((e = hipStreamSynchronize(ix->stream))) break;
        if (sum64 > (unsigned long long)ix->n_entries) {
            overlap = true;
            break;
        }
        if ((rc = scan_exclusive((const uint32_t *)sizes.p, ix->rx_pstart, M + 1, scratch, 0, ix->stream))) break;
        uint32_t total = 0;
        if ((e = hipMemcpyAsync(&total, ix->rx_pstart + M, 4, hipMemcpyDeviceToHost, ix->stream))) break;
        if ((e = hipStreamSynchronize(ix->stream))) break;
        ix->rx_S = total;
        {
            const size_t occ_words = (size_t)((M + 31) / 32) + ((size_t)1 << (P2F_LOGBITS + 2 - 5));
            if (hipMalloc(ix->rx_occ.put(), occ_words * 4) == hipSuccess) {
                if ((e = hipMemsetAsync(ix->rx_occ, 0, occ_words * 4, ix->stream))) break;
                hipLaunchKernelGGL(k_rx_build_occ, dim3(grid_for(ix, (int64_t)((M / 32 + 256) / 256), 16)), dim3(256), 0, ix->stream,
                                   ix->rx_pstart, M, ix->rx_occ);
            } else {
                (void)hipGetLastError();
            }
        }
        const size_t S = total ? total : 1;
        if ((e = hipMalloc(ix->rx_pkeys.put(), S * RxViewBytes::pkeys))) break;
        if ((e = hipMalloc(ix->rx_pkeys_raw.put(), S * RxViewBytes::pkeys_raw))) break;
        if ((e = hipMalloc(ix->rx_pfreq.put(), S * RxViewBytes::pfreq))) break;
        if ((e = hipMalloc(ix->rx_pnodes.put(), S * RxViewBytes::pnodes))) break;
        if ((e = hipMalloc(ix->rx_porig.put(), S * RxViewBytes::porig))) break;
        if ((e = hipMalloc(ix->rx_ecnt.put(), S * RxViewBytes::ecnt))) break;
        if ((e = hipMemsetAsync(ix->rx_ecnt, 0, S * RxViewBytes::ecnt, ix->stream))) break;
        hipLaunchKernelGGL(k_rx_pack, dim3(grid_for(ix, (int64_t)((M + 255) / 256), 16)), dim3(256), 0, ix->stream, h2i,
                           kmers, nodes, freqs, M, ix->max_node_id, ix->rx_pstart, ix->rx_pkeys_raw, ix->rx_pfreq,
                           ix->rx_pnodes, ix->rx_porig);
        if ((e = hipGetLastError())) break;
        if ((e = hipStreamSynchronize(ix->stream))) break;
        if (total) {
            const uint64_t n_nodes = (uint64_t)ix->max_node_id + 1;
            DevBuf hist, cursor;
            if (n_nodes + 1 < 0xFFFFFFFFull && (uint64_t)total / n_nodes < 8 && ensure(hist, (size_t)(n_nodes + 1) * 4) == KMM_OK &&
                ensure(cursor, (size_t)(n_nodes + 1) * 4) == KMM_OK &&
                hipMalloc(ix->rx_norder.put(), S * RxViewBytes::norder) == hipSuccess &&
                hipMalloc(ix->rx_nnode.put(), S * RxViewBytes::nnode) == hipSuccess) {
                bool ok = hipMemsetAsync(hist.p, 0, (size_t)(n_nodes + 1) * 4, ix->stream) == hipSuccess;
                hipLaunchKernelGGL(k_rx_node_hist, dim3(grid_for(ix, (int64_t)((S + 255) / 256), 16)), dim3(256), 0,
                                   ix->stream, ix->rx_pnodes, (uint64_t)total, (uint32_t *)hist.p);
                ok = ok && scan_exclusive((const uint32_t *)hist.p, (uint32_t *)cursor.p, n_nodes + 1, scratch, 0,
                                          ix->stream) == KMM_OK;
                hipLaunchKernelGGL(k_rx_node_scatter, dim3(grid_for(ix, (int64_t)((S + 255) / 256), 16)), dim3(256), 0,
                                   ix->stream, ix->rx_pnodes, (uint64_t)total, (uint32_t *)cursor.p, ix->rx_norder,
                                   ix->rx_nnode);
                ok = ok && hipGetLastError() == hipSuccess && hipStreamSynchronize(ix->stream) == hipSuccess;
                if (!ok) {
                    (void)ix->rx_norder.reset();
                    (void)ix->rx_nnode.reset();
                }
            } else {
                (void)hipGetLastError();
                (void)ix->rx_norder.reset();
                (void)ix->rx_nnode.reset();
            }
        }
    } while (0);
    (void)sizes.reset();
    scratch.clear();
    if (rc != KMM_OK || e != hipSuccess || overlap) {
        const bool nomem = rc == KMM_ERR_NOMEM || e == hipErrorOutOfMemory;
        (void)hipGetLastError();
        static_cast<RxArrays &>(*ix) = RxArrays();
        ix->rx_ok = false;
        if (overlap || nomem) {
            ix->rx_why_not = overlap ? 4 : 3;
            if (getenv("KMM_VERBOSE"))
                fprintf(stderr, "libkmm: radix view not built (%s): every batch takes the direct path\n",
                        overlap ? "the buckets of the index overlap" : "out of HBM");
            return KMM_OK;
        }
        if (rc != KMM_OK)
            return rc;
        return fail(KMM_ERR_HIP, "radix index build: %s", hipGetErrorString(e));
    }
    std::optional<int> w_force;
    if (const char *env = getenv("KMM_RX_W"))
        w_force = atoi(env);
    const int f2_force = getenv("KMM_RX_F2") ? atoi(getenv("KMM_RX_F2")) : -1;
    ix->rx_no_mid = getenv("KMM_RX_NO_MID") != nullptr;
    const std::optional<RxGeometry> geo = rx_choose_geometry(M, ix->rx_S, ix->rx_filter, w_force, f2_force);
    ix->rx_ok = geo.has_value();
    if (geo)
        ix->rx_geo = *geo;
    ix->rx_why_not = ix->rx_ok ? 0 : 2;
    if (getenv("KMM_VERBOSE"))
        fprintf(stderr, "libkmm: modulo %llu, %llu entries: radix path %s (2^%d buckets per slice, %u x %u partitions)\n",
                (unsigned long long)M, (unsigned long long)ix->rx_S, ix->rx_ok ? "available" : "NOT available: slices too "
                "dense for LDS or more than 512 x 512 of them", ix->rx_geo.w, ix->rx_geo.F1, ix->rx_geo.F2);
    if (ix->rx_ok)
        KMMCHK(rx_repack_keys(ix));
    ix->rx_min_units = rx_min_units(M, ix->rx_S);
    if (const char *env = getenv("KMM_RX_MIN_UNITS"))
        ix->rx_min_units = strtoll(env, nullptr, 10);
    return KMM_OK;
}

constexpr int RX_REFUSED = 1;
int rx_reconfigure(kmm_index *ix, int w, int f2_force, bool set_ok)
{
    const std::optional<RxGeometry> geo = rx_geometry(ix->modulo, ix->rx_S, ix->rx_filter, w, RX_MAXF, f2_force);
    if (!geo)
        return RX_REFUSED;
    ix->rx_geo = *geo;
    if (set_ok)
        ix->rx_ok = ix->rx_pstart != nullptr;
    if (ix->rx_pstart) {
        KMMCHK(rx_flush(ix));
        KMMCHK(rx_repack_keys(ix));
    }
    return KMM_OK;
}
```

### kmer_mapper_amd/csrc/kmm_radix_plan.hpp

```cpp
#pragma once
#include <cstddef>
#include <cstdint>
#include <optional>

constexpr int RX_B = 8192;
constexpr int RX_MAXF = 512;
#ifndef RX_CHV
#define RX_CHV 256
#endif
constexpr int RX_CH = RX_CHV;
constexpr int RX_IC = 1024;
constexpr int RX_ECAP = 4096;
constexpr int RX_ECAP_BIG = 8192;
constexpr int RX_ECAP_MID = 4608;
constexpr int P2F_KMAX = 64;
constexpr int P2F_LOGBITS = 19;
constexpr int P2F_SLOT_WORDS = 3 << (P2F_LOGBITS - 6);
constexpr int P2F_SLOTS = 5888;

constexpr uint32_t rx_filter_slot(uint32_t b, uint64_t quot)
{
    const uint32_t v = ((uint32_t)quot ^ (uint32_t)(quot >> 24) ^ (uint32_t)(quot >> 48)) + (b << 23);
    const uint32_t h16 = ((v & 0xFFFFFFu) * 0x9E3779u) >> 16;
    return 3u * (b >> 1) + ((h16 * 3u) >> 16);
// ... 73 lines not shown
        }
    }
    if (f2_force >= 0)
        f2 = f2_force;
    const uint64_t max_quo = ~0ull / modulo;
    auto fits = [&](int sh) { return sh == 0 || (sh < 64 && (max_quo >> (64 - sh)) == 0); };
    while (f2 > 0 && !fits(w + f2))
        --f2;
    if (!fits(w + f2))
        return std::nullopt;
    const uint64_t F2 = 1ull << f2, F1 = (PF + F2 - 1) / F2;
    if (F2 > (uint64_t)maxf || F1 > (uint64_t)(for_filter ? RX_MAXF : maxf))
        return std::nullopt;
    RxGeometry g;
    g.w = w;
    g.f2 = f2;
    g.occ_shift = w + f2 > P2F_LOGBITS ? w + f2 - P2F_LOGBITS : 0;
    g.slot_filter = w + f2 == P2F_LOGBITS;
    g.PF = (uint32_t)PF;
    g.F1 = (uint32_t)F1;
    g.F2 = (uint32_t)F2;
    return g;
}

inline std::optional<RxGeometry> rx_choose_geometry(uint64_t modulo, uint64_t S, bool filter, std::optional<int> w_force = std::nullopt,
                                                    int f2_force = -1)
{
    const bool w_forced = w_force.has_value();
    const double load = (double)S / (double)modulo;
    int w = 12;
    if (w_forced)
        w = *w_force;
    else
        while (w > 0 && (load * (double)(1u << w) * 1.3 + 64.0 > (double)RX_ECAP || (1ull << w) > modulo))
            --w;
    const bool fits13_small = load * 8192.0 * 1.3 + 64.0 <= (double)RX_ECAP;
    const bool fits13 = load * 8192.0 * 1.3 + 64.0 <= (double)RX_ECAP_BIG;
    auto conf = [&](int w_, int maxf) { return rx_geometry(modulo, S, filter, w_, maxf); };
    std::optional<RxGeometry> g = rx_geometry(modulo, S, filter, w, f2_force >= 0 ? RX_MAXF : 256, f2_force);
    if (!g && w == 12 && !w_forced) {
        if (fits13_small)
            g = conf(13, 256);
        if (!g)
            g = conf(12, RX_MAXF);
        if (!g && fits13 && !(g = conf(13, 256)))
            g = conf(13, RX_MAXF);
    } else if (!g) {
        g = conf(w, RX_MAXF);
    }
    return g;
}

struct RxScratch {
    uint32_t chunks;
    size_t max_items;
    size_t start1, P1T, S1T, csum, T1, item_base, work_base, item_desc, start2, start2T, ctrl, queue;
    size_t meta_bytes;
    size_t buf1_bytes, buf2_bytes;
};

constexpr size_t rx_align256(size_t x) { return (x + 255) & ~(size_t)255; }

inline RxScratch rx_scratch(uint32_t NB, uint32_t F1, uint32_t F2)
{
    RxScratch s;
    s.chunks = (NB + RX_CH - 1) / RX_CH;
    s.max_items = (size_t)NB + F1 + 1;
    size_t off = 0;
    auto carve = [&](size_t bytes) { const size_t o = off; off += rx_align256(bytes); return o; };
    s.start1 = carve((size_t)NB * (F1 + 1) * 2);
    s.P1T = carve((size_t)F1 * ((size_t)NB + 1) * 4);
    s.S1T = carve((size_t)F1 * NB * 2);
    s.csum = carve((size_t)s.chunks * F1 * 4);
    s.T1 = carve((size_t)F1 * 4);
    s.item_base = carve((size_t)(F1 + 1) * 4);
    s.work_base = carve((size_t)(F1 + 1) * 4);
    s.item_desc = carve(s.max_items * 8);
    s.start2 = carve(s.max_items * (F2 + 1) * 2);
    s.start2T = carve(s.max_items * (F2 + 1) * 2 + 256);
    s.ctrl = carve(64);
    s.queue = carve(2048);
    s.meta_bytes = off;
    s.buf1_bytes = (size_t)NB * RX_B * 8;
    s.buf2_bytes = s.max_items * RX_B * 8;
    return s;
}

constexpr int64_t RX_SUB_CAP_MAX = ((int64_t)1 << 32) - 2 * RX_B;
constexpr int64_t RX_SUB_CAP_FLOOR = (int64_t)1 << 28;
constexpr int RX_SUB_CAP_AGE = 16;

struct RxSplit {
    int64_t n_sub, max_src;
};

inline RxSplit rx_split(int64_t n_src_total, uint32_t X, int64_t cap)
{
    const int64_t cap_src = (cap / RX_B) / X > 0 ? (cap / RX_B) / X : 1;
    RxSplit s;
    s.n_sub = (n_src_total + cap_src - 1) / cap_src;
    s.max_src = s.n_sub ? (n_src_total + s.n_sub - 1) / s.n_sub : cap_src;
    return s;
}

inline int64_t rx_next_smaller_cap(int64_t n_src_total, uint32_t X, int64_t n_sub)
{
    const int64_t next_src = (n_src_total + n_sub) / (n_sub + 1);
    const int64_t cap = next_src * RX_B * X;
    return cap < RX_SUB_CAP_FLOOR ? RX_SUB_CAP_FLOOR : cap;
}

enum class RxP3Variant {
    W12_DIR16,
    W12,
    W13_SMALL_DIR16,
    W13_SMALL,
    W13_MID_DIR16,
    W13_MID,
    W13_BIG,
};
struct RxP3Shape {
    int keys_in_lds;
    int wg_per_cu;
    bool dir16;
    bool fingerprints = false;
};
constexpr RxP3Shape RX_P3_SHAPES[] = {
    {RX_ECAP, 2, true, true}, {RX_ECAP, 2, false},
    {RX_ECAP, 2, true}, {RX_ECAP, 2, false},
    {RX_ECAP_MID, 2, true}, {RX_ECAP_MID, 2, false},
    {RX_ECAP_BIG, 1, false},
};
constexpr const RxP3Shape &rx_p3_shape(RxP3Variant v) { return RX_P3_SHAPES[(int)v]; }
constexpr int rx_p3_fp_shapes()
{
    int n = 0;
    for (const RxP3Shape &s : RX_P3_SHAPES)
        n += s.fingerprints ? 1 : 0;
    return n;
}

inline RxP3Variant rx_choose_p3(int w, bool fits_small, bool fits_mid, bool p16, uint32_t max_slice, bool no_mid)
{
    if (w <= 12)
        return p16 ? RxP3Variant::W12_DIR16 : RxP3Variant::W12;
    const bool lds16 = p16 || max_slice <= 65535u;
    if (fits_small && lds16)
        return p16 ? RxP3Variant::W13_SMALL_DIR16 : RxP3Variant::W13_SMALL;
    if (fits_mid && lds16 && !no_mid)
        return p16 ? RxP3Variant::W13_MID_DIR16 : RxP3Variant::W13_MID;
    return RxP3Variant::W13_BIG;
}

struct RxViewBytes {
    enum : size_t { pstart = 4, pkeys = 8, pkeys_raw = 8, pfreq = 2, pnodes = 4, porig = 4, ecnt = 4, norder = 4, nnode = 4 };
};
constexpr size_t rx_view_bytes(uint64_t modulo, uint64_t S, bool node_order)
{
    return (size_t)(modulo + 1) * RxViewBytes::pstart +
           (size_t)(S ? S : 1) * (RxViewBytes::pkeys + RxViewBytes::pkeys_raw + RxViewBytes::pfreq + RxViewBytes::pnodes +
                                  RxViewBytes::porig + RxViewBytes::ecnt + (node_order ? RxViewBytes::norder + RxViewBytes::nnode : 0));
}

inline int64_t rx_min_units(uint64_t modulo, uint64_t S)
{
    const double bytes = (double)modulo * 4.0 + (double)S * 14.0;
    const double fixed = 50e-6 + bytes / 2.6e12;
    const double per_kmer_radix = 6.5e-12 * (1.0 + bytes / 40e9);
    const double per_kmer_direct = 1.0 / (bytes < 1e9 ? 60e9 : 38e9);
    const int64_t units = (int64_t)(1.25 * fixed / (per_kmer_direct - per_kmer_radix));
    return units < ((int64_t)1 << 22) ? (int64_t)1 << 22 : units;
}
```

Measured before the change: 178,600.

## Defer radix phase-3 across sub-batches and batch them into one launch

Result: no change. 180,000, median of 6 (+0.8%).

```diff
diff --git a/kmer_mapper_amd/csrc/kmm.hip b/kmer_mapper_amd/csrc/kmm.hip
--- a/kmer_mapper_amd/csrc/kmm.hip
+++ b/kmer_mapper_amd/csrc/kmm.hip
@@ -364,7 +364,16 @@
     bool rx_packed = true;
     bool ecnt_dirty = false;
     bool rx_unchecked = false;
-    DevBuf rx_buf1, rx_buf2, rx_meta, rx_probe;
+    DevBuf rx_buf1, rx_probe;
+    DevBuf rx_buf2[RX_P3_MAX_SLOTS], rx_meta[RX_P3_MAX_SLOTS], rx_p3_ctl, rx_p3_rowtab;
+    int rx_p3_defer = 2;
+    int rx_n_slots = 0;
+    RxP3Slot rx_pend[RX_P3_MAX_SLOTS] = {};
+    int rx_n_pend = 0;
+    int rx_pend_max_freq = 0;
+    int64_t rx_p3_launches = 0;
+    uint32_t dbg_p3_chunk_items = RX_IC;
+    uint32_t dbg_p3_row_chunks = RX_P3_ROW_CHUNKS;
     int sticky_rc = KMM_OK;
     std::string sticky_msg;
     uint64_t map_calls = 0;
@@ -442,6 +451,8 @@
 };
 
 int rx_flush(kmm_index *ix);
+int rx_settle(kmm_index *ix);
+int rx_drop_pending(kmm_index *ix);
 int rx_build_slots(kmm_index *ix);
 bool rx_slots_active(const kmm_index *ix);
 int rx_check_conservation(kmm_index *ix);
@@ -1288,6 +1299,7 @@
         return fail(KMM_ERR_INVALID_ARG, "idx is NULL");
     HIPCHK(hipSetDevice(ix->device));
     HIPCHK(hipMemsetAsync(ix->counts, 0, sizeof(uint32_t) * (size_t)(ix->max_node_id + 1), ix->stream));
+    KMMCHK(rx_drop_pending(ix));
     if (ix->rx_ecnt && ix->ecnt_dirty)
         HIPCHK(hipMemsetAsync(ix->rx_ecnt, 0, sizeof(uint32_t) * (size_t)(ix->rx_S ? ix->rx_S : 1), ix->stream));
     if (ix->rx_ecnt_acc)
@@ -1490,6 +1502,7 @@
             HIPCHK(hipEventCreateWithFlags(e.put(), hipEventDisableTiming));
             ix->comm_events.push_back(std::move(e));
         }
+        KMMCHK(rx_settle(ix));
         if (!by_range)
             KMMCHK(rx_flush(ix));
         if (by_range && (int)ix->flush_cuts.size() != S + 1) {
@@ -4272,6 +4285,7 @@
     if (kernel_id < 0 || kernel_id >= KMM_N_KERNELS)
         return fail(KMM_ERR_INVALID_ARG, "kernel_id %d outside [0, %d)", kernel_id, KMM_N_KERNELS);
     HIPCHK(hipSetDevice(ix->device));
+    KMMCHK(rx_settle(ix));
     HIPCHK(hipStreamSynchronize(ix->stream));
     for (auto &ev : ix->ev_used) {
         float ms = 0.f;
@@ -4376,6 +4390,10 @@
     HIPCHK(hipSetDevice(ix->device));
     if (strncmp(name, "debug_records_", 14) != 0)
         HIPCHK(hipStreamSynchronize(ix->stream));
+    for (const char *touches : {"part_shift", "fine_bits", "radix_filter", "radix_filter_slots", "radix_p3_fingerprints",
+                                "radix_grid_per_cu", "radix_p3_defer", "debug_p3_chunk_items", "debug_p3_row_chunks", "count_kmers"})
+        if (!strcmp(name, touches))
+            KMMCHK(rx_settle(ix));
     if (!strcmp(name, "path")) {
         if (value < 0 || value > 2)
             return fail(KMM_ERR_INVALID_ARG, "path must be 0 (auto), 1 (direct) or 2 (radix)");
@@ -4405,6 +4423,22 @@
             KMMCHK(rx_build_slots(ix));
     } else if (!strcmp(name, "radix_p3_fingerprints")) {
         ix->rx_p3_fp = value != 0;
+    } else if (!strcmp(name, "radix_p3_defer")) {
+        if (value < 1 || value > RX_P3_MAX_SLOTS)
+            return fail(KMM_ERR_INVALID_ARG, "radix_p3_defer outside [1, %d]", RX_P3_MAX_SLOTS);
+        ix->rx_p3_defer = (int)value;
+        ix->rx_n_slots = 0;
+    } else if (!strcmp(name, "debug_p3_chunk_items")) {
+        if (value < 1 || value > RX_IC)
+            return fail(KMM_ERR_INVALID_ARG, "debug_p3_chunk_items outside [1, %d]", RX_IC);
+        ix->dbg_p3_chunk_items = (uint32_t)value;
+    } else if (!strcmp(name, "debug_p3_row_chunks")) {
+        if (value < 1 || value > RX_P3_ROW_CHUNKS)
+            return fail(KMM_ERR_INVALID_ARG, "debug_p3_row_chunks outside [1, %d]", RX_P3_ROW_CHUNKS);
+        ix->dbg_p3_row_chunks = (uint32_t)value;
+    } else if (!strcmp(name, "radix_p3_launches") || !strcmp(name, "radix_pending_batches") ||
+               !strcmp(name, "radix_p3_defer_effective")) {
+        return fail(KMM_ERR_INVALID_ARG, "%s is read-only", name);
     } else if (!strcmp(name, "debug_p2f_round_slots")) {
         if (value < 512 || value > P2F_SLOTS || (value & 1))
             return fail(KMM_ERR_INVALID_ARG, "debug_p2f_round_slots must be even and in [512, %d]", P2F_SLOTS);
@@ -4743,6 +4777,18 @@
                                                       : (int64_t)1 << (ix->rx_geo.w + ix->rx_geo.f2 - ix->rx_geo.occ_shift);
     else if (!strcmp(name, "debug_p2f_round_slots"))
         *value = ix->dbg_p2f_cap;
+    else if (!strcmp(name, "radix_p3_defer"))
+        *value = ix->rx_p3_defer;
+    else if (!strcmp(name, "radix_p3_defer_effective"))
+        *value = ix->rx_n_slots;
+    else if (!strcmp(name, "radix_pending_batches"))
+        *value = ix->rx_n_pend;
+    else if (!strcmp(name, "radix_p3_launches"))
+        *value = ix->rx_p3_launches;
+    else if (!strcmp(name, "debug_p3_chunk_items"))
+        *value = ix->dbg_p3_chunk_items;
+    else if (!strcmp(name, "debug_p3_row_chunks"))
+        *value = ix->dbg_p3_row_chunks;
     else if (!strcmp(name, "radix_packed_tiles"))
         *value = ix->rx_packed ? 1 : 0;
     else if (!strcmp(name, "n_fine_per_coarse"))
diff --git a/kmer_mapper_amd/csrc/kmm_radix.hpp b/kmer_mapper_amd/csrc/kmm_radix.hpp
--- a/kmer_mapper_amd/csrc/kmm_radix.hpp
+++ b/kmer_mapper_amd/csrc/kmm_radix.hpp
@@ -45,6 +45,7 @@
 #define RX_LOAD2(p) (*(p))
 #define RX_LOAD3(p) (*(p))
 #endif
+#define RX_GLOBAL_PTR(T, p) ((const __attribute__((address_space(1))) T *)(p))
 constexpr int RX_WMAX = 4096;
 constexpr int RX_WMAX_BIG = 8192;
 constexpr uint32_t RX_FILTERED = 0x80000000u;
@@ -824,6 +825,58 @@
     }
 }
 
+__global__ void __launch_bounds__(512) k_rx_p3_rows(RxView rx, RxP3Slots ps, RxP3RowSeg *tab, uint32_t row_cap)
+{
+    static_assert(RX_MAXF <= 512, "one thread per coarse partition");
+    __shared__ uint32_t s_wave8[8];
+    const uint32_t c = threadIdx.x, F1 = rx.F1;
+    uint32_t n_items[RX_P3_MAX_SLOTS], first[RX_P3_MAX_SLOTS];
+#pragma unroll
+    for (int s = 0; s < RX_P3_MAX_SLOTS; ++s) {
+        first[s] = c < F1 && (uint32_t)s < ps.n ? ps.s[s].item_base[c] : 0u;
+        n_items[s] = c < F1 && (uint32_t)s < ps.n ? ps.s[s].item_base[c + 1] - first[s] : 0u;
+    }
+    const uint32_t rows = c < F1 ? rx_p3_rows(n_items, ps.n, ps.rows) : 0u;
+    uint32_t tot_rows;
+    const uint32_t wb = scan512_excl(rows, s_wave8, &tot_rows);
+    const bool fits = tot_rows <= row_cap;
+    if (c < F1)
+        rx.work_base[c] = wb;
+    if (c == 0) {
+        rx.work_base[F1] = fits ? tot_rows : 0u;
+        rx.ctrl[1] = fits ? tot_rows : 0u;
+    }
+    if (threadIdx.x < 256)
+        rx.queue[threadIdx.x] = 0ull;
+    for (uint32_t r = 0; fits && r < rows; ++r) {
+        RxP3RowSeg sg[RX_P3_ROW_CHUNKS];
+        uint32_t n_ch = 0;
+#pragma unroll
+        for (int k = 0; k < RX_P3_ROW_CHUNKS; ++k) {
+            const RxP3Seg w = rx_p3_row_segment(n_items, ps.n, ps.rows, r, (uint32_t)k);
+            RxP3Slot sl = ps.s[0];
+            uint32_t f0 = first[0];
+#pragma unroll
+            for (int s = 1; s < RX_P3_MAX_SLOTS; ++s) {
+                sl = w.slot == (uint32_t)s ? ps.s[s] : sl;
+                f0 = w.slot == (uint32_t)s ? first[s] : f0;
+            }
+            const uint32_t it0 = f0 + w.first;
+            sg[k].items = sl.buf2 + (size_t)it0 * RX_B;
+            sg[k].starts = sl.start2T + it0;
+            sg[k].max_items = sl.max_items;
+            sg[k].n_it = w.n;
+            sg[k].pad = 0u;
+            n_ch += w.n ? 1u : 0u;
+        }
+#pragma unroll
+        for (int k = 0; k < RX_P3_ROW_CHUNKS; ++k) {
+            sg[k].n_ch = n_ch;
+            tab[(size_t)(wb + r) * RX_P3_ROW_CHUNKS + k] = sg[k];
+        }
+    }
+}
+
 template <bool WITH_P>
 __global__ void __launch_bounds__(256) k_rx_colscan(RxView rx)
 {
@@ -1457,8 +1510,9 @@
 #define RX_P3_KEY_READ(cond)
 #endif
 template <int WMAX, int ECAP, int WPS, typename DirT, int SUBCAP = RX_SUBCAP3, bool P16 = false, bool FP = false>
-__global__ void __launch_bounds__(RX_NT, WPS) k_rx_p3(IndexView iv, RxView rx, int max_freq)
-{
+__global__ void __launch_bounds__(RX_NT, WPS) k_rx_p3(IndexView iv, RxView rx, const RxP3RowSeg *rowtab, int max_freq)
+{
+    constexpr int RC = RX_P3_ROW_CHUNKS;
     static_assert(!P16 || sizeof(DirT) == 2, "the 16-bit directory is copied as it is");
     __shared__ uint32_t sfp[FP ? (ECAP + 8) / 4 : 1];
     __shared__ __attribute__((aligned(4))) DirT sdir[WMAX + 2];
@@ -1483,12 +1537,14 @@
     const int sh = rx.w + rx.f2;
     __syncthreads();
     struct Slice {
-        uint32_t valid, g, e0, ne, it0, n_it, over, tot, fmax;
+        uint32_t valid, g, e0, ne, row, over, tot, fmax;
+        RxP3RowSeg seg0;
         uint64_t h0;
     };
     auto describe = [&](uint32_t sub, uint32_t idx) {
         Slice d;
-        d.valid = 0; d.g = 0; d.e0 = 0; d.ne = 0; d.it0 = 0; d.n_it = 0; d.h0 = 0; d.over = 0; d.tot = 0; d.fmax = 0xFFFFu;
+        d.valid = 0; d.g = 0; d.e0 = 0; d.ne = 0; d.row = 0; d.h0 = 0; d.over = 0; d.tot = 0; d.fmax = 0xFFFFu;
+        d.seg0.items = nullptr; d.seg0.starts = nullptr; d.seg0.max_items = 0; d.seg0.n_it = 0; d.seg0.n_ch = 0; d.seg0.pad = 0;
         if (idx >= limit)
             return d;
         const uint32_t row = idx / gs, g = sub * gs + idx % gs;
@@ -1504,7 +1560,6 @@
         const uint32_t f2c = rx.PF - c * F2 < F2 ? rx.PF - c * F2 : F2;
         if (g >= f2c)
             return d;
-        const uint32_t chunk = row - s_wb[c];
         d.valid = 1;
         d.g = g;
         d.h0 = (uint64_t)(c * F2 + g) << rx.w;
@@ -1520,10 +1575,18 @@
         d.tot = e1 - d.e0;
         d.ne = e1 - d.e0 < (uint32_t)ECAP ? e1 - d.e0 : (uint32_t)ECAP;
         d.over = e1 - d.e0 > (uint32_t)ECAP ? 1u : 0u;
-        d.it0 = rx.item_base[c] + chunk * RX_IC;
-        const uint32_t it_end = rx.item_base[c + 1];
-        d.n_it = it_end - d.it0 < (uint32_t)RX_IC ? it_end - d.it0 : (uint32_t)RX_IC;
+        d.row = row;
+        d.seg0 = rowtab[(size_t)row * RC];
         return d;
+    };
+    auto load_runs = [&](const RxP3RowSeg &sg, uint32_t g, uint32_t (&rf)[RX_IC / RX_NT], uint32_t (&rt)[RX_IC / RX_NT]) {
+        const auto *rfp = RX_GLOBAL_PTR(uint16_t, sg.starts + (size_t)g * sg.max_items), *rtp = rfp + sg.max_items;
+#pragma unroll
+        for (int j = 0; j < RX_IC / RX_NT; ++j) {
+            const uint32_t i = tid + j * RX_NT;
+            rf[j] = i < sg.n_it ? rfp[i] : 0u;
+            rt[j] = i < sg.n_it ? rtp[i] : 0u;
+        }
     };
     RX_PT_DECL;
     for (uint32_t turn = 0; turn < 8u; ++turn) {
@@ -1543,7 +1606,7 @@
     Slice sl = describe(sub, idx_first);
     for (;;) {
         RX_PT(0);
-        const uint32_t g = sl.g, e0 = sl.e0, ne = sl.ne, it0 = sl.it0, n_it = sl.n_it;
+        const uint32_t e0 = sl.e0, ne = sl.ne;
         const uint64_t h0 = sl.h0;
         uint32_t rf[RX_IC / RX_NT], rt[RX_IC / RX_NT];
 #pragma unroll
@@ -1579,14 +1642,7 @@
             kv[j] = i < ne ? rx.pkeys[(size_t)e0 + i] : 0ull;
             fv[j] = i < ne && need_f ? rx.pfreq[(size_t)e0 + i] : 0u;
         }
-        const uint16_t *rfp = rx.start2T + (size_t)g * rx.max_items + it0;
-        const uint16_t *rtp = rfp + rx.max_items;
-#pragma unroll
-        for (int j = 0; j < RX_IC / RX_NT; ++j) {
-            const uint32_t i = tid + j * RX_NT;
-            rf[j] = i < n_it ? rfp[i] : 0u;
-            rt[j] = i < n_it ? rtp[i] : 0u;
-        }
+        load_runs(sl.seg0, sl.g, rf, rt);
         if (P16) {
             uint32_t *sd32 = reinterpret_cast<uint32_t *>(sdir);
 #pragma unroll
@@ -1636,31 +1692,43 @@
             }
         };
         if (sl.valid) {
-        {
+        RxP3RowSeg sg = sl.seg0;
+        const uint32_t n_ch = (uint32_t)__builtin_amdgcn_readfirstlane((int)sg.n_ch);
+        for (uint32_t ck = 0; ck < n_ch; ++ck) {
             constexpr int NR = RX_IC / RX_NT;
-            uint32_t len[NR], np[NR], np_sum = 0, src[NR];
+            uint32_t rf_n[NR], rt_n[NR];
+            RxP3RowSeg sg_n = sg;
+            sg_n.n_it = 0u;
+            if (ck + 1u < n_ch)
+                sg_n = rowtab[(size_t)sl.row * RC + ck + 1u];
+            load_runs(sg_n, sl.g, rf_n, rt_n);
+            uint32_t rl[NR], np_sum = 0;
 #pragma unroll
             for (int j = 0; j < NR; ++j) {
-                len[j] = rt[j] - rf[j];
-                src[j] = (uint32_t)(tid + j * RX_NT) * (uint32_t)RX_B + rf[j];
-                np[j] = (len[j] + (uint32_t)RX_LPR_P3 - 1u) / (uint32_t)RX_LPR_P3;
-                np_sum += np[j];
-            }
-            const char *wbase = reinterpret_cast<const char *>(rx.buf2 + (size_t)__builtin_amdgcn_readfirstlane((int)it0) * RX_B);
+                const uint32_t len = rt[j] - rf[j];
+                rl[j] = rf[j] | len << 16;
+                np_sum += (len + (uint32_t)RX_LPR_P3 - 1u) / (uint32_t)RX_LPR_P3;
+            }
+            const uint64_t ib = reinterpret_cast<uint64_t>(sg.items);
+            const char *wbase = reinterpret_cast<const char *>((uint64_t)(uint32_t)__builtin_amdgcn_readfirstlane((int)(ib >> 32)) << 32 |
+                                                               (uint32_t)__builtin_amdgcn_readfirstlane((int)ib));
             uint32_t n_sub;
             const uint32_t pre = rx_scan_threads(np_sum, s_wave8, scan_flip, &n_sub);
             for (uint32_t win = 0; win < n_sub; win += SUBCAP) {
                 uint32_t first = pre;
 #pragma unroll
                 for (int j = 0; j < NR; ++j) {
+                    asm volatile("" : "+v"(rl[j]));
+                    const uint32_t len = rl[j] >> 16, np = (len + (uint32_t)RX_LPR_P3 - 1u) / (uint32_t)RX_LPR_P3;
+                    const uint32_t src = (uint32_t)(tid + j * RX_NT) * (uint32_t)RX_B + (rl[j] & 0xFFFFu);
                     const uint32_t j0 = first > win ? first : win;
-                    const uint32_t j1 = first + np[j] < win + (uint32_t)SUBCAP ? first + np[j] : win + (uint32_t)SUBCAP;
+                    const uint32_t j1 = first + np < win + (uint32_t)SUBCAP ? first + np : win + (uint32_t)SUBCAP;
                     for (uint32_t q = j0; q < j1; ++q) {
                         const uint32_t done = (q - first) * (uint32_t)RX_LPR_P3;
-                        const uint32_t n = len[j] - done < (uint32_t)RX_LPR_P3 ? len[j] - done : (uint32_t)RX_LPR_P3;
-                        sub_list[q - win] = ((src[j] + done) << 5) | n;
+                        const uint32_t n = len - done < (uint32_t)RX_LPR_P3 ? len - done : (uint32_t)RX_LPR_P3;
+                        sub_list[q - win] = ((src + done) << 5) | n;
                     }
-                    first += np[j];
+                    first += np;
                 }
                 const uint32_t nw = n_sub - win < (uint32_t)SUBCAP ? n_sub - win : (uint32_t)SUBCAP;
                 constexpr uint32_t STEP = RX_NG3 * RX_U;
@@ -1678,11 +1746,11 @@
 #pragma unroll
                     for (int u = 0; u < RX_U; ++u) {
                         const bool in = (uint32_t)lg < (e[u] & 31u);
-                        x[u] = RX_LOAD3(reinterpret_cast<const uint64_t *>(wbase + (((e[u] >> 5) + (in ? (uint32_t)lg : 0u)) << 3)));
+                        x[u] = RX_LOAD3(RX_GLOBAL_PTR(uint64_t, wbase + (((e[u] >> 5) + (in ? (uint32_t)lg : 0u)) << 3)));
                         act |= (in ? 1u : 0u) << u;
 #if RX_PROBE_P3R
                         if (u % RX_PROBE_P3R == 0) {
-                            const size_t far = ((size_t)it0 * RX_B + (e[u] >> 5) + (uint32_t)lg) % ((size_t)rx.NB * RX_B);
+                            const size_t far = ((size_t)(sg.items - rx.buf2) + (e[u] >> 5) + (uint32_t)lg) % ((size_t)rx.NB * RX_B);
                             const uint64_t z = RX_LOAD3(rx.buf1 + far);
                             asm volatile("" ::"v"(z));
                         }
@@ -1787,6 +1855,12 @@
                 __syncthreads();
                 RX_PT(3);
             }
+#pragma unroll
+            for (int j = 0; j < NR; ++j) {
+                rf[j] = rf_n[j];
+                rt[j] = rt_n[j];
+            }
+            sg = sg_n;
         }
         for (uint32_t i = tid; i < ne; i += RX_NT) {
             const uint32_t cn = scnt[i];
diff --git a/kmer_mapper_amd/csrc/kmm_radix_host.hpp b/kmer_mapper_amd/csrc/kmm_radix_host.hpp
--- a/kmer_mapper_amd/csrc/kmm_radix_host.hpp
+++ b/kmer_mapper_amd/csrc/kmm_radix_host.hpp
@@ -56,7 +56,7 @@
     return ix->rx_p3_fp && rx_p3_shape(rx_p3_variant(ix)).fingerprints;
 }
 
-RxView rx_view_of(const kmm_index *ix, const RxScratch &sc, uint32_t NB)
+RxView rx_view_of(const kmm_index *ix, const RxScratch &sc, uint32_t NB, int slot)
 {
     const RxGeometry &g = ix->rx_geo;
     RxView rx;
@@ -70,7 +70,7 @@
     rx.p2f_k = NB / 2048u < 4u ? 4u : (NB / 2048u > (uint32_t)P2F_KMAX ? (uint32_t)P2F_KMAX : NB / 2048u);
     rx.w = g.w; rx.f2 = g.f2; rx.PF = g.PF; rx.F1 = g.F1; rx.F2 = g.F2;
     rx.NB = NB; rx.max_items = (uint32_t)sc.max_items;
-    uint8_t *m = (uint8_t *)ix->rx_meta.p;
+    uint8_t *m = (uint8_t *)ix->rx_meta[slot].p;
     rx.start1 = (uint16_t *)(m + sc.start1); rx.P1T = (uint32_t *)(m + sc.P1T); rx.S1T = (uint16_t *)(m + sc.S1T);
     rx.csum = (uint32_t *)(m + sc.csum); rx.T1 = (uint32_t *)(m + sc.T1); rx.item_base = (uint32_t *)(m + sc.item_base);
     rx.work_base = (uint32_t *)(m + sc.work_base); rx.item_desc = (uint2 *)(m + sc.item_desc);
@@ -78,7 +78,7 @@
     rx.ctrl = (uint32_t *)(m + sc.ctrl);
     rx.queue = (unsigned long long *)(m + sc.queue);
     rx.buf1 = (uint64_t *)ix->rx_buf1.p;
-    rx.buf2 = (uint64_t *)ix->rx_buf2.p;
+    rx.buf2 = (uint64_t *)ix->rx_buf2[slot].p;
 #if RX_PROBE_ANY
     rx.probe = (uint64_t *)ix->rx_probe.p;
 #endif
@@ -127,11 +127,11 @@
     hipLaunchKernelGGL(kern, dim3(ix->n_cu), dim3(P2F_NT), 0, ix->stream, iv, rx);
 }
 
-void rx_launch_p3(kmm_index *ix, const IndexView &iv, const RxView &rx, int max_freq)
+void rx_launch_p3(kmm_index *ix, const IndexView &iv, const RxView &rx, const RxP3RowSeg *rowtab, int max_freq)
 {
     const RxP3Variant v = rx_p3_variant(ix);
     const dim3 grid(ix->n_cu * (rx_p3_shape(v).wg_per_cu > 1 ? ix->rx_grid_per_cu : 1));
-    auto go = [&](auto kern) { hipLaunchKernelGGL(kern, grid, dim3(RX_NT), 0, ix->stream, iv, rx, max_freq); };
+    auto go = [&](auto kern) { hipLaunchKernelGGL(kern, grid, dim3(RX_NT), 0, ix->stream, iv, rx, rowtab, max_freq); };
     static_assert(rx_p3_shape(RxP3Variant::W12_DIR16).fingerprints && rx_p3_fp_shapes() == 1,
                   "RX_P3_SHAPES promises the fingerprint form exactly where an instantiation is named below");
     switch (v) {
@@ -150,6 +150,94 @@
     }
 }
 
+constexpr size_t RX_P3_CTL_WORK = 0, RX_P3_CTL_CTRL = rx_align256((RX_MAXF + 1) * 4), RX_P3_CTL_QUEUE = RX_P3_CTL_CTRL + 256,
+                 RX_P3_CTL_BYTES = RX_P3_CTL_QUEUE + 2048;
+
+int rx_settle(kmm_index *ix)
+{
+    if (!ix->rx_n_pend)
+        return KMM_OK;
+    KMMCHK(ensure(ix->rx_p3_ctl, RX_P3_CTL_BYTES));
+    const RxScratch none = rx_scratch(0, ix->rx_geo.F1, ix->rx_geo.F2);
+    RxView rx = rx_view_of(ix, none, 0, 0);
+    uint8_t *m = (uint8_t *)ix->rx_p3_ctl.p;
+    rx.start1 = nullptr; rx.P1T = nullptr; rx.S1T = nullptr; rx.csum = nullptr; rx.T1 = nullptr; rx.item_base = nullptr;
+    rx.item_desc = nullptr; rx.start2 = nullptr; rx.start2T = nullptr; rx.buf2 = nullptr; rx.max_items = 0;
+    rx.work_base = (uint32_t *)(m + RX_P3_CTL_WORK);
+    rx.ctrl = (uint32_t *)(m + RX_P3_CTL_CTRL);
+    rx.queue = (unsigned long long *)(m + RX_P3_CTL_QUEUE);
+    RxP3Slots ps;
+    memset(&ps, 0, sizeof ps);
+    for (int i = 0; i < ix->rx_n_pend; ++i)
+        ps.s[i] = ix->rx_pend[i];
+    ps.n = (uint32_t)ix->rx_n_pend;
+    ps.rows = rx_p3_rows_of(ix->dbg_p3_chunk_items, ix->dbg_p3_row_chunks);
+    const size_t row_cap = rx_p3_row_bound(ps.s, ps.n, ix->rx_geo.F1, ps.rows);
+    KMMCHK(ensure(ix->rx_p3_rowtab, row_cap * RX_P3_ROW_CHUNKS * sizeof(RxP3RowSeg)));
+    RxP3RowSeg *rowtab = (RxP3RowSeg *)ix->rx_p3_rowtab.p;
+    ScopedTimer tm;
+    KMMCHK(tm.begin(ix, KMM_KERNEL_RX_SCAN));
+    hipLaunchKernelGGL(k_rx_p3_rows, dim3(1), dim3(512), 0, ix->stream, rx, ps, rowtab, (uint32_t)row_cap);
+    HIPCHK(hipGetLastError());
+    KMMCHK(tm.end());
+    KMMCHK(tm.begin(ix, KMM_KERNEL_RX_P3));
+    rx_launch_p3(ix, view_of(ix), rx, rowtab, ix->rx_pend_max_freq);
+    HIPCHK(hipGetLastError());
+    KMMCHK(tm.end());
+    ix->ecnt_dirty = true;
+    ix->rx_p3_launches++;
+    ix->rx_n_pend = 0;
+    return KMM_OK;
+}
+
+int rx_drop_pending(kmm_index *ix)
+{
+    if (!ix->rx_n_pend)
+        return KMM_OK;
+    ix->rx_n_pend = 0;
+    HIPCHK(hipMemsetAsync(ix->stats, 0, KMM_STAT_BYTES, ix->stream));
+    ix->rx_unchecked = false;
+    return KMM_OK;
+}
+
+int rx_alloc_buffers(kmm_index *ix, const RxScratch &sm, int want)
+{
+    const size_t lim = (size_t)ix->dbg_rx_buf_limit;
+    if (lim && sm.buf1_bytes > lim)
+        return KMM_ERR_NOMEM;
+    KMMCHK(ensure(ix->rx_buf1, sm.buf1_bytes));
+    KMMCHK(ensure(ix->rx_p3_ctl, RX_P3_CTL_BYTES));
+#if RX_PROBE_ANY
+    KMMCHK(ensure(ix->rx_probe, sm.buf2_bytes));
+#endif
+    int n = 0, rc = KMM_OK;
+    for (; n < want; ++n) {
+        rc = lim && n >= 1 && (size_t)n * sm.buf1_bytes >= lim ? (int)KMM_ERR_NOMEM : ensure(ix->rx_meta[n], sm.meta_bytes);
+        if (rc == KMM_OK)
+            rc = ensure(ix->rx_buf2[n], sm.buf2_bytes);
+        if (rc != KMM_OK)
+            break;
+    }
+    if (n >= 1) {
+        RxP3Slot full[RX_P3_MAX_SLOTS] = {};
+        for (int i = 0; i < n; ++i)
+            full[i].max_items = (uint32_t)sm.max_items;
+        const size_t rows = rx_p3_row_bound(full, (uint32_t)n, ix->rx_geo.F1, rx_p3_rows_of(RX_IC, RX_P3_ROW_CHUNKS));
+        if (ensure(ix->rx_p3_rowtab, rows * RX_P3_ROW_CHUNKS * sizeof(RxP3RowSeg)) != KMM_OK)
+            (void)hipGetLastError();
+    }
+    for (int i = n; i < RX_P3_MAX_SLOTS; ++i) {
+        (void)ix->rx_meta[i].reset();
+        (void)ix->rx_buf2[i].reset();
+    }
+    ix->rx_n_slots = n;
+    if (n >= 1 && rc == KMM_ERR_NOMEM) {
+        (void)hipGetLastError();
+        rc = KMM_OK;
+    }
+    return rc;
+}
+
 template <int MODE>
 int launch_rx(kmm_index *ix, const ReadsView &rv, const uint64_t *kmers_in, int64_t n_in, int k, int max_freq,
               int also_rc)
@@ -166,26 +254,30 @@
     if (ix->rx_sub_cap_eff > 0 && ++ix->rx_sub_cap_eff_age >= RX_SUB_CAP_AGE)
         ix->rx_sub_cap_eff = 0;
     int64_t cap = ix->rx_sub_cap_eff > 0 && ix->rx_sub_cap_eff < ix->rx_sub_cap ? ix->rx_sub_cap_eff : ix->rx_sub_cap;
+    if (ix->rx_n_pend && ix->rx_pend_max_freq != max_freq)
+        KMMCHK(rx_settle(ix));
     for (;;) {
         split = rx_split(n_src_total, X, cap);
         const RxScratch sm = rx_scratch((uint32_t)(split.max_src * X), F1, F2);
-        int rc = ix->dbg_rx_buf_limit && sm.buf1_bytes > (size_t)ix->dbg_rx_buf_limit ? (int)KMM_ERR_NOMEM
-                                                                                      : ensure(ix->rx_meta, sm.meta_bytes);
-        if (rc == KMM_OK)
-            rc = ensure(ix->rx_buf1, sm.buf1_bytes);
-        if (rc == KMM_OK)
-            rc = ensure(ix->rx_buf2, sm.buf2_bytes);
-#if RX_PROBE_ANY
-        if (rc == KMM_OK)
-            rc = ensure(ix->rx_probe, sm.buf2_bytes);
-#endif
+        bool fits = ix->rx_n_slots >= 1 && sm.buf1_bytes <= ix->rx_buf1.cap &&
+                    !(ix->dbg_rx_buf_limit && sm.buf1_bytes > (size_t)ix->dbg_rx_buf_limit);
+        for (int i = 0; i < ix->rx_n_slots; ++i)
+            fits = fits && sm.meta_bytes <= ix->rx_meta[i].cap && sm.buf2_bytes <= ix->rx_buf2[i].cap;
+        if (fits)
+            break;
+        KMMCHK(rx_settle(ix));
+        const int rc = rx_alloc_buffers(ix, sm, ix->rx_p3_defer);
         if (rc == KMM_OK)
             break;
         if (rc != KMM_ERR_NOMEM || cap <= RX_SUB_CAP_FLOOR || n_src_total <= 1)
             return rc;
         (void)hipGetLastError();
         (void)ix->rx_buf1.reset();
-        (void)ix->rx_buf2.reset();
+        for (int i = 0; i < RX_P3_MAX_SLOTS; ++i) {
+            (void)ix->rx_meta[i].reset();
+            (void)ix->rx_buf2[i].reset();
+        }
+        ix->rx_n_slots = 0;
         cap = rx_next_smaller_cap(n_src_total, X, split.n_sub);
         ix->rx_sub_cap_eff = cap;
         ix->rx_sub_cap_eff_age = 0;
@@ -197,13 +289,16 @@
         const uint32_t n_src = (uint32_t)(n_src_total - s0 < max_src ? n_src_total - s0 : max_src);
         const uint32_t NB = n_src * X;
         const RxScratch sc = rx_scratch(NB, F1, F2);
-        bool grew = sc.meta_bytes > ix->rx_meta.cap || sc.buf1_bytes > ix->rx_buf1.cap || sc.buf2_bytes > ix->rx_buf2.cap;
+        const int slot = ix->rx_n_pend;
+        if (slot >= ix->rx_n_slots)
+            return fail(KMM_ERR_INTERNAL, "radix path: %d sub-batches pending in %d slots", slot, ix->rx_n_slots);
+        bool grew = sc.meta_bytes > ix->rx_meta[slot].cap || sc.buf1_bytes > ix->rx_buf1.cap || sc.buf2_bytes > ix->rx_buf2[slot].cap;
 #if RX_PROBE_ANY
         grew = grew || sc.buf2_bytes > ix->rx_probe.cap;
 #endif
         if (grew)
             return fail(KMM_ERR_INTERNAL, "radix path: a sub-batch of %u blocks needs more scratch than the largest one was given", NB);
-        const RxView rx = rx_view_of(ix, sc, NB);
+        const RxView rx = rx_view_of(ix, sc, NB, slot);
         ix->dbg_T1 = rx.T1; ix->dbg_item_base = rx.item_base; ix->dbg_start1 = rx.start1; ix->dbg_F1 = F1; ix->dbg_NB = NB;
         HIPCHK(hipMemsetAsync(rx.ctrl, 0, sc.meta_bytes - sc.ctrl, ix->stream));
         ScopedTimer tm;
@@ -231,23 +326,24 @@
         hipLaunchKernelGGL(k_rx_tr2, dim3((unsigned)((sc.max_items + RX_TR2 - 1) / RX_TR2)), dim3(256), 0, ix->stream, rx);
         HIPCHK(hipGetLastError());
         KMMCHK(tm.end());
-        KMMCHK(tm.begin(ix, KMM_KERNEL_RX_P3));
-        rx_launch_p3(ix, iv, rx, max_freq);
-        HIPCHK(hipGetLastError());
-        KMMCHK(tm.end());
-        ix->ecnt_dirty = true;
         ix->rx_unchecked = true;
+        RxP3Slot &pd = ix->rx_pend[slot];
+        pd.buf2 = rx.buf2; pd.start2T = rx.start2T; pd.item_base = rx.item_base; pd.max_items = rx.max_items;
+        ix->rx_pend_max_freq = max_freq;
+        if (++ix->rx_n_pend >= ix->rx_n_slots)
+            KMMCHK(rx_settle(ix));
     }
     ix->n_radix_batches++;
     if (verbose && ms_since(t_0) > 20.0)
         fprintf(stderr, "libkmm: radix passes of %lld positions: %.2f ms for the batch buffers (%zu + %zu + %zu bytes), %.2f ms to issue %lld "
-                "sub-batch(es)\n", (long long)units, ms_buffers, ix->rx_meta.cap, ix->rx_buf1.cap, ix->rx_buf2.cap, ms_since(t_0) - ms_buffers,
+                "sub-batch(es)\n", (long long)units, ms_buffers, ix->rx_meta[0].cap, ix->rx_buf1.cap, ix->rx_buf2[0].cap, ms_since(t_0) - ms_buffers,
                 (long long)split.n_sub);
     return KMM_OK;
 }
 
 int rx_flush(kmm_index *ix)
 {
+    KMMCHK(rx_settle(ix));
     if (!ix->ecnt_dirty)
         return KMM_OK;
     ScopedTimer tm;
@@ -333,6 +429,12 @@
         ix->rx_filter_slots = atoi(env) != 0;
     if (const char *env = getenv("KMM_RX_P3_FP"))
         ix->rx_p3_fp = atoi(env) != 0;
+    if (const char *env = getenv("KMM_RX_P3_DEFER"))
+        if (atoi(env) >= 1 && atoi(env) <= RX_P3_MAX_SLOTS)
+            ix->rx_p3_defer = atoi(env);
+    if (const char *env = getenv("KMM_RX_P3_ROW_CHUNKS"))
+        if (atoi(env) >= 1 && atoi(env) <= RX_P3_ROW_CHUNKS)
+            ix->dbg_p3_row_chunks = (uint32_t)atoi(env);
     ix->rx_why_not = 1;
     if (M >= (1ull << 31))
         return KMM_OK;
diff --git a/kmer_mapper_amd/csrc/kmm_radix_plan.hpp b/kmer_mapper_amd/csrc/kmm_radix_plan.hpp
--- a/kmer_mapper_amd/csrc/kmm_radix_plan.hpp
+++ b/kmer_mapper_amd/csrc/kmm_radix_plan.hpp
@@ -249,6 +249,91 @@
     return RxP3Variant::W13_BIG;
 }
 
+constexpr int RX_P3_MAX_SLOTS = 8;
+constexpr int RX_P3_ROW_CHUNKS = 4;
+
+struct RxP3Seg {
+    uint32_t slot, first, n;
+};
+struct RxP3Rows {
+    uint32_t chunk_items, chunk_magic, row_chunks;
+};
+constexpr RxP3Rows rx_p3_rows_of(uint32_t chunk_items, uint32_t row_chunks)
+{
+    return RxP3Rows{chunk_items, (uint32_t)((((uint64_t)1 << 31) + chunk_items - 1u) / chunk_items), row_chunks};
+}
+RX_PLAN_HD inline uint32_t rx_p3_chunks(uint32_t n_items, const RxP3Rows &r)
+{
+    return (uint32_t)(((uint64_t)(n_items + r.chunk_items - 1u) * r.chunk_magic) >> 31);
+}
+RX_PLAN_HD inline uint32_t rx_p3_row_capacity(const uint32_t *n_items, uint32_t n_slots, const RxP3Rows &r, uint32_t *chunks)
+{
+    uint32_t n = 0, most = 0;
+    for (uint32_t s = 0; s < (uint32_t)RX_P3_MAX_SLOTS; ++s) {
+        const uint32_t ch = s < n_slots ? rx_p3_chunks(n_items[s], r) : 0u;
+        n += ch;
+        most = ch > most ? ch : most;
+    }
+    *chunks = n;
+    return most > 1u ? 1u : r.row_chunks;
+}
+RX_PLAN_HD inline uint32_t rx_p3_rows(const uint32_t *n_items, uint32_t n_slots, const RxP3Rows &r)
+{
+    uint32_t n;
+    const uint32_t cap = rx_p3_row_capacity(n_items, n_slots, r, &n);
+    return (n + cap - 1u) / cap;
+}
+RX_PLAN_HD inline RxP3Seg rx_p3_row_segment(const uint32_t *n_items, uint32_t n_slots, const RxP3Rows &r, uint32_t row, uint32_t k)
+{
+    RxP3Seg seg = {0u, 0u, 0u};
+    uint32_t n;
+    const uint32_t cap = rx_p3_row_capacity(n_items, n_slots, r, &n);
+    if (k >= cap)
+        return seg;
+    uint32_t q = row * cap + k;
+    bool found = false;
+    for (uint32_t s = 0; s < (uint32_t)RX_P3_MAX_SLOTS; ++s) {
+        const uint32_t ni = s < n_slots ? n_items[s] : 0u;
+        const uint32_t ch = rx_p3_chunks(ni, r);
+        if (!found && q < ch) {
+            found = true;
+            seg.slot = s;
+            seg.first = q * r.chunk_items;
+            seg.n = ni - seg.first < r.chunk_items ? ni - seg.first : r.chunk_items;
+        }
+        q -= found ? 0u : ch;
+    }
+    return seg;
+}
+
+struct RxP3Slot {
+    const uint64_t *buf2;
+    const uint16_t *start2T;
+    const uint32_t *item_base;
+    uint32_t max_items;
+};
+struct RxP3RowSeg {
+    const uint64_t *items;
+    const uint16_t *starts;
+    uint32_t max_items;
+    uint32_t n_it;
+    uint32_t n_ch;
+    uint32_t pad;
+};
+static_assert(sizeof(RxP3RowSeg) == 32, "one aligned 32-byte record per segment");
+inline size_t rx_p3_row_bound(const RxP3Slot *slots, uint32_t n_slots, uint32_t F1, const RxP3Rows &r)
+{
+    size_t rows = 1;
+    for (uint32_t s = 0; s < n_slots; ++s)
+        rows += slots[s].max_items / r.chunk_items + F1;
+    return rows;
+}
+struct RxP3Slots {
+    RxP3Slot s[RX_P3_MAX_SLOTS];
+    uint32_t n;
+    RxP3Rows rows;
+};
+
 struct RxViewBytes {
     enum : size_t { pstart = 4, pkeys = 8, pkeys_raw = 8, pfreq = 2, pnodes = 4, porig = 4, ecnt = 4, norder = 4, nnode = 4 };
 };
```
